# Kolkir/feature-point-cnn

Hardware: AMD Instinct MI355X
Metric: frames/sec (VGA 640x480) SuperPoint fwd+NMS+descriptors (higher is better)
Workload: dtype f32

## Files before the change

### feature-point-cnn_amd/_lib.py

```python
import ctypes
import os
import subprocess

import torch

_DIR = os.path.dirname(os.path.abspath(__file__))
LIB_PATH = os.environ.get("FPC_LIB_PATH") or os.path.join(_DIR, "lib", "libfpc.so")
CSRC = os.path.join(_DIR, "csrc")

SYMBOLS = [
    "fpc_abi_version", "fpc_build_flags", "fpc_strerror", "fpc_last_hip_error", "fpc_default_config", "fpc_create",
    "fpc_destroy", "fpc_load_weights", "fpc_packed_size", "fpc_packed_device_ptr",
    "fpc_export_packed", "fpc_import_packed", "fpc_import_packed_device", "fpc_mark_weights_loaded", "fpc_set_stream", "fpc_upload_stream",
    "fpc_get_stream", "fpc_sync", "fpc_forward", "fpc_detect", "fpc_get_points", "fpc_results",
    "fpc_get_counts", "fpc_get_keypoints", "fpc_set_timing", "fpc_get_timings", "fpc_match", "fpc_first_within",
    "fpc_detect_u8", "fpc_u8_staging", "fpc_homography_adaptation", "fpc_detect_u8_resized",
    "fpc_sample_descriptors", "fpc_plan_hash", "fpc_broadcast_weights", "fpc_read_activation",
    "fpc_pack_layout_revision", "fpc_check_guards", "fpc_stream_report", "fpc_output_range",
    "fpc_match_frames", "fpc_first_within_frames",
    "fpc_default_ransac_params", "fpc_ransac_homography", "fpc_homography_frames",
    "fpc_bank_create", "fpc_bank_destroy", "fpc_bank_get", "fpc_bank_store", "fpc_bank_store_rows", "fpc_bank_clear",
    "fpc_match_bank", "fpc_homography_bank", "fpc_bank_create_ex", "fpc_bank_format",
    "fpc_match_frames_guided", "fpc_match_bank_guided",
    "fpc_cell_order", "fpc_match_frames_guided_cells", "fpc_match_bank_guided_cells",
    "fpc_bank_topk_reserve", "fpc_match_bank_topk", "fpc_homography_bank_topk",
    "fpc_ransac_fundamental", "fpc_fundamental_frames", "fpc_fundamental_bank",
    "fpc_match_frames_guided_epipolar", "fpc_match_bank_guided_epipolar",
]

ABI_VERSION = 4
PACK_LAYOUT_REVISION = 4

PLAN_FLAGS = {
    "no_fused_blocks": 1 << 0, "no_winograd": 1 << 1, "no_winograd_detector": 1 << 2, "no_winograd_layer_in1": 1 << 3,
    "no_xcd_order": 1 << 4, "no_fused_stem_pool": 1 << 5, "split_heads": 1 << 6, "nms_in_line": 1 << 7,
    "no_persistent_grid": 1 << 8, "layer1_tile_8x16": 1 << 9, "winograd_gen1": 1 << 10, "no_latency_tiles": 1 << 11,
    "nms_one_workgroup": 1 << 12, "no_fused_softmax": 1 << 13, "winograd_gen2": 1 << 14, "guard_zones": 1 << 15, "detector_gen1": 1 << 16, "heads_in_line": 1 << 17, "w36_one_wave": 1 << 18, "convt_phases": 1 << 19, "stem_round3": 1 << 20, "conv_round1": 1 << 21,
}


class FpcConfig(ctypes.Structure):
    _fields_ = [("device", ctypes.c_int), ("height", ctypes.c_int), ("width", ctypes.c_int),
                ("max_batch", ctypes.c_int), ("cell", ctypes.c_int), ("nms_dist", ctypes.c_int),
                ("conf_thresh", ctypes.c_float), ("border_remove", ctypes.c_int),
                ("descriptor_enabled", ctypes.c_int), ("max_keypoints", ctypes.c_int),
                ("in_channels", ctypes.c_int), ("dtype", ctypes.c_int), ("arch", ctypes.c_int),
                ("num_streams", ctypes.c_int), ("plan_flags", ctypes.c_uint), ("nms_round_launches", ctypes.c_int),
                ("min_sub_batch", ctypes.c_int)]


class FpcTensor(ctypes.Structure):
    _fields_ = [("name", ctypes.c_char_p), ("data", ctypes.c_void_p), ("ndim", ctypes.c_int),
                ("shape", ctypes.c_int64 * 4)]


class FpcDeviceResults(ctypes.Structure):
    _fields_ = [("count", ctypes.c_void_p), ("n_candidates", ctypes.c_void_p), ("xy", ctypes.c_void_p),
                ("conf", ctypes.c_void_p), ("desc", ctypes.c_void_p), ("capacity", ctypes.c_int),
                ("desc_dim", ctypes.c_int)]


class FpcStreamReport(ctypes.Structure):
    _fields_ = [("n_streams", ctypes.c_int), ("slot", ctypes.c_int * 16), ("queue", ctypes.c_int * 16),
                ("probing", ctypes.c_int), ("hw_queues_found", ctypes.c_int), ("process_probe_rounds", ctypes.c_int),
                ("process_probe_launches", ctypes.c_int), ("process_inconclusive_rounds", ctypes.c_int),
                ("process_probe_ms", ctypes.c_float), ("create_probe_rounds", ctypes.c_int),
                ("create_placement_ms", ctypes.c_float), ("process_registered_streams", ctypes.c_int)]


class FpcRansacParams(ctypes.Structure):
    _fields_ = [("iterations", ctypes.c_int), ("reproj_threshold", ctypes.c_float), ("seed", ctypes.c_uint32),
                ("refits", ctypes.c_int), ("min_inliers", ctypes.c_int)]


BANK_MAX_SLOTS = 1024
BANK_TOPK_MAX = 16


class FpcBankView(ctypes.Structure):
    _fields_ = [("desc", ctypes.c_void_p), ("xy", ctypes.c_void_p), ("count", ctypes.c_void_p), ("slots", ctypes.c_int),
                ("rows", ctypes.c_int), ("desc_dim", ctypes.c_int), ("chunk", ctypes.c_int), ("bytes", ctypes.c_size_t)]


class FpcError(RuntimeError):
    def __init__(self, code, where):
        self.code = code
        l = load()
        msg = l.fpc_strerror(code).decode()
        detail = l.fpc_last_hip_error().decode()
        super().__init__("%s: %s (%d)%s" % (where, msg, code, " -- " + detail if detail else ""))


_lib = None


def build(force=False):
    args = ["make", "-s", "-C", CSRC]
    if force:
        args.append("-B")
    subprocess.check_call(args)
    return LIB_PATH


def load():
    global _lib
    if _lib is not None:
        return _lib
    if not os.path.exists(LIB_PATH):
        raise ImportError("libfpc.so is not built (%s): run `python -c 'import __graft_entry__ as g; g.build()'` "
                          "or `make -C feature-point-cnn_amd/csrc`; there is no CPU fallback" % LIB_PATH)
    l = ctypes.CDLL(LIB_PATH)
    vp, ci = ctypes.c_void_p, ctypes.c_int
    l.fpc_abi_version.restype = ci
    l.fpc_build_flags.restype = ctypes.c_char_p
    l.fpc_strerror.restype = ctypes.c_char_p
    l.fpc_strerror.argtypes = [ci]
    l.fpc_last_hip_error.restype = ctypes.c_char_p
    l.fpc_default_config.argtypes = [ctypes.POINTER(FpcConfig)]
    l.fpc_create.argtypes = [ctypes.POINTER(vp), ctypes.POINTER(FpcConfig)]
    l.fpc_destroy.argtypes = [vp]
    l.fpc_destroy.restype = None
    l.fpc_load_weights.argtypes = [vp, ctypes.POINTER(FpcTensor), ci]
    l.fpc_packed_size.argtypes = [vp]
    l.fpc_packed_size.restype = ctypes.c_size_t
    l.fpc_packed_device_ptr.argtypes = [vp]
    l.fpc_packed_device_ptr.restype = vp
    l.fpc_export_packed.argtypes = [vp, vp, ctypes.c_size_t]
    l.fpc_import_packed.argtypes = [vp, vp, ctypes.c_size_t]
    l.fpc_import_packed_device.argtypes = [vp, vp, ctypes.c_size_t]
    l.fpc_mark_weights_loaded.argtypes = [vp]
    l.fpc_set_stream.argtypes = [vp, vp]
    l.fpc_upload_stream.argtypes = [vp]
    l.fpc_upload_stream.restype = vp
    l.fpc_get_stream.argtypes = [vp]
    l.fpc_get_stream.restype = vp
    l.fpc_sync.argtypes = [vp]
    l.fpc_forward.argtypes = [vp, vp, ci, vp, vp, vp]
    l.fpc_detect.argtypes = [vp, vp, ci]
    l.fpc_get_points.argtypes = [vp, vp, vp, ci]
    l.fpc_detect_u8.argtypes = [vp, vp, ci, ci]
    l.fpc_u8_staging.argtypes = [vp]
    l.fpc_detect_u8_resized.argtypes = [vp, vp, ci, ci, ci, ci]
    l.fpc_homography_adaptation.argtypes = [vp, vp, ci, vp, vp, ci, ci, ci, vp]
    l.fpc_u8_staging.restype = vp
    l.fpc_results.argtypes = [vp, ctypes.POINTER(FpcDeviceResults)]
    l.fpc_get_counts.argtypes = [vp, ci, vp, vp]
    l.fpc_get_keypoints.argtypes = [vp, ci, ci, vp, vp, vp]
    l.fpc_output_range.argtypes = [vp, ci, vp, vp, vp]
    l.fpc_match.argtypes = [vp, vp, ci, vp, ci, ci, ctypes.c_float, vp, vp]
    l.fpc_first_within.argtypes = [vp, vp, ci, vp, ci, ctypes.c_float, vp]
    l.fpc_match_frames.argtypes = [vp, ci, ci, vp, vp, ci, ctypes.c_float, ctypes.c_float, vp, vp]
    l.fpc_first_within_frames.argtypes = [vp, ci, vp, vp, ctypes.c_float, vp]
    rp = ctypes.POINTER(FpcRansacParams)
    l.fpc_default_ransac_params.argtypes = [rp]
    l.fpc_ransac_homography.argtypes = [vp, ci, vp, vp, vp, ci, rp, vp, vp, vp]
    l.fpc_homography_frames.argtypes = [vp, ci, ci, vp, vp, vp, rp, vp, vp, vp]
    l.fpc_bank_create.argtypes = [vp, ci, ci]
    l.fpc_bank_create_ex.argtypes = [vp, ci, ci, ci]
    l.fpc_bank_format.argtypes = [vp, ctypes.POINTER(ci), ctypes.POINTER(vp)]
    l.fpc_bank_destroy.argtypes = [vp]
    l.fpc_bank_get.argtypes = [vp, ctypes.POINTER(FpcBankView)]
    l.fpc_bank_store.argtypes = [vp, ci, ci]
    l.fpc_bank_store_rows.argtypes = [vp, ci, vp, vp, vp]
    l.fpc_bank_clear.argtypes = [vp, ci]
    l.fpc_match_bank.argtypes = [vp, ci, ci, ctypes.c_float, ctypes.c_float, ci, vp, vp, vp, vp]
    l.fpc_homography_bank.argtypes = [vp, ci, vp, vp, rp, vp, vp, vp]
    l.fpc_ransac_fundamental.argtypes = [vp, ci, vp, vp, vp, ci, rp, vp, vp, vp]
    l.fpc_fundamental_frames.argtypes = [vp, ci, ci, vp, vp, vp, rp, vp, vp, vp]
    l.fpc_fundamental_bank.argtypes = [vp, ci, vp, vp, rp, vp, vp, vp]
    l.fpc_match_frames_guided.argtypes = [vp, ci, ci, vp, vp, vp, vp, ctypes.c_float, ci, ctypes.c_float, ctypes.c_float,
                                          vp, vp]
    l.fpc_match_bank_guided.argtypes = [vp, ci, vp, vp, ctypes.c_float, ci, ctypes.c_float, ctypes.c_float, vp, vp]
    l.fpc_cell_order.argtypes = [vp, vp, vp, ci, ci, vp]
    l.fpc_match_frames_guided_cells.argtypes = [vp, ci, ci, vp, vp, vp, vp, ctypes.c_float, ci, ctypes.c_float,
                                                ctypes.c_float, vp, vp, vp]
    l.fpc_match_bank_guided_cells.argtypes = [vp, ci, vp, vp, ctypes.c_float, ci, ctypes.c_float, ctypes.c_float, vp, vp,
                                              vp]
    l.fpc_match_frames_guided_epipolar.argtypes = list(l.fpc_match_frames_guided.argtypes)
    l.fpc_match_bank_guided_epipolar.argtypes = list(l.fpc_match_bank_guided.argtypes)
    l.fpc_bank_topk_reserve.argtypes = [vp, ci, ctypes.POINTER(ctypes.c_size_t)]
    l.fpc_match_bank_topk.argtypes = [vp, ci, ci, ci, ctypes.c_float, ctypes.c_float, ci, vp, vp, vp, vp, vp]
    l.fpc_homography_bank_topk.argtypes = [vp, ci, ci, vp, vp, rp, vp, vp, vp, vp, vp]
    l.fpc_sample_descriptors.argtypes = [vp, vp, vp, ci, vp]
    l.fpc_read_activation.argtypes = [vp, ctypes.c_char_p, ci, ci, vp, ctypes.POINTER(ci), ctypes.POINTER(ci), ctypes.POINTER(ci)]
    l.fpc_plan_hash.argtypes = [vp]
    l.fpc_plan_hash.restype = ctypes.c_uint64
    l.fpc_broadcast_weights.argtypes = [vp, vp, ci]
    l.fpc_pack_layout_revision.restype = ci
    l.fpc_check_guards.argtypes = [vp, ctypes.POINTER(ctypes.c_longlong)]
    l.fpc_stream_report.argtypes = [vp, ctypes.POINTER(FpcStreamReport)]
# ... 21 lines not shown
```

### feature-point-cnn_amd/csrc/fpc_api.hip

```cpp
#include <hip/hip_runtime.h>

#include <dlfcn.h>

#include <algorithm>
#include <cmath>
#include <cstdio>
#include <cstdlib>
#include <cstring>
#include <memory>
#include <mutex>
#include <chrono>
#include <string>
#include <vector>

#include "../../include/fpc.h"
#include "block_mfma.h"
#include "block_bf16.h"
#include "convt_bf16.h"
#include "block_x3.h"
#include "stem_bf16.h"
#include "wblock_mfma.h"
#include "wblock16_mfma.h"
#include "wblock36_mfma.h"
#include "wblock36p_mfma.h"
// ... 268 lines not shown
#undef X
#define X(name, TYT, TXT)                                                                                 \
  {#name, "wblock36_dust_kernel<" #TYT ", " #TXT ">", 3, 16, 2, 64,                                        \
   W36Cfg<1, TYT, TXT, true>::LDS_BYTES, 4, 4 * TYT, 4 * TXT, 256, (const void*)wblock36_dust_kernel<TYT, TXT>, launchw_##name, true},
    FPC_W36D_KINDS(X)
#undef X
#define X(name, TYT, TXT)                                                                                 \
  {#name, "wblock36p_kernel<" #TYT ", " #TXT ", 3>", 3, 16, 2, 64,                                            \
   W36PCfg<TYT, TXT>::LDS_BYTES, 4, 4 * TYT, 4 * TXT, 512, (const void*)wblock36p_kernel<TYT, TXT>, launchw_##name},
    FPC_W36P_KINDS(X)
#undef X
#define X(name, TYT, TXT)                                                                                 \
  {#name, "wblock36p_dust_kernel<" #TYT ", " #TXT ", 3>", 3, 16, 2, 64,                                    \
   W36PCfg<TYT, TXT, true>::LDS_BYTES, 4, 4 * TYT, 4 * TXT, 512, (const void*)wblock36p_dust_kernel<TYT, TXT>, launchw_##name, true},
    FPC_W36PD_KINDS(X)
#undef X
};

static size_t w1_floats(const WKindInfo& k, int nchunk) {
  if (k.gen == 3) return (size_t)k.NCG * ((size_t)nchunk * 36 + (k.NCG == 8 ? W36Cfg<2, 4, 4>::WPAD : W36Cfg<1, 4, 4>::WPAD)) * 256;
  return (size_t)k.NCG * ((size_t)nchunk * 16 + W16Cfg<8>::WPAD) * 256;
}
static double wkind_mfma_flops(const WKindInfo& k, int tiles, int nchunk, int k8_1x1) {
  const double px = (double)k.TH * k.TW, n = k.NBT * 32.0;
  if (k.gen == 3) return 2.0 * tiles * n * (36.0 * (px / 16) * nchunk * k.KC + px * k8_1x1 * 8.0);
  return 2.0 * tiles * n * (16.0 * (px / 4) * nchunk * k.KC + px * k8_1x1 * 8.0);
}
static bool w36_fits(int , int H, int W, int cs_in, int cs_out) {
  return (unsigned long long)H * W * (unsigned long long)std::max(cs_in, cs_out) * sizeof(float) < (unsigned long long)W36_MARKER;
}
static int w36_frames_per_launch(int H, int W, int cs_in, int cs_out) {
  const unsigned long long fb = (unsigned long long)H * W * (unsigned long long)std::max(cs_in, cs_out) * sizeof(float);
  return (int)std::max<unsigned long long>(1, ((unsigned long long)W36_MARKER - 1) / fb);
}
static int w36_conv_part(int cout, int tiles, int cus) {
  if (cout < 128) return 64;
  if (cout == 128) return 128;
  const double t2 = std::ceil((double)tiles * (cout / 128) / cus) * 1.0, t1 = std::ceil((double)tiles * (cout / 64) / cus) * 0.53;
  return t1 < t2 ? 64 : 128;
}
static WKind w36_kind(int cout, int H, int W, bool paired = false) {
  const int t44 = ((H + 15) / 16) * ((W + 15) / 16), t28 = ((H + 7) / 8) * ((W + 31) / 32);
  if (cout == 65 && paired) return t28 < t44 ? WK_W36PD_C65_2x8 : WK_W36PD_C65_4x4;
  if (cout == 65) return t28 < t44 ? WK_W36_C65_2x8 : WK_W36_C65_4x4;
  if (cout == 64 && paired) return t28 < t44 ? WK_W36P_C64_2x8 : WK_W36P_C64_4x4;
  if (cout == 64) return t28 < t44 ? WK_W36_C64_2x8 : WK_W36_C64_4x4;
  return t28 < t44 ? WK_W36_C128_2x8 : WK_W36_C128_4x4;
}

#define FPC_BF16_KINDS(X)                                                                   \
  X(F816_s1_K64_C64, block_bf16_one_kernel, BlockBfCfg, 1, 8, 32, 1, 3, 64, 2, 2, 4, 1, 64) \
  X(F816_s1_K64_C128, block_bf16_kernel, BlockBfCfg, 1, 8, 16, 1, 3, 64, 1, 4, 4, 1, 128)   \
  X(F816_s1_K80_C80, block_bf16_one_kernel, BlockBfCfg, 1, 8, 16, 1, 3, 80, 4, 1, 1, 3, 80) \
  X(F816_s1_K128_C128, block_bf16_one_kernel, BlockBfCfg, 1, 8, 16, 1, 3, 128, 1, 4, 4, 1, 128) \
  X(F816_s1_K128_C80w, block_bf16_one_kernel, BlockBfCfg, 1, 8, 16, 1, 3, 128, 1, 4, 4, 1, 80) \
  X(F620_s2_K64_C128, block_bf16_one_kernel, BlockBfCfg, 1, 6, 20, 2, 3, 64, 2, 2, 2, 2, 128) \
  X(F320_s2_K128_C256, block_bf16_one_kernel, BlockBfCfg, 1, 3, 20, 2, 3, 128, 1, 4, 2, 2, 256) \
  X(F416_s1_K128_C256, block_bf16_two_kernel, BlockBfCfg, 1, 4, 16, 1, 3, 128, 1, 4, 2, 2, 256) \
  X(F816_ct_K64_C128, block_bf16_kernel, BlockBfCfg, 1, 8, 16, 1, 2, 64, 1, 4, 4, 1, 128)   \
  X(F816_ctf_K64_C128, convt_bf16_kernel, ConvTBfCfg, 1, 8, 16, 1, 2, 64, 2, 2, 2, 1, 128)  \
  X(S816_s1_K64_C64, block_x3_kernel, BlockX3Cfg, 3, 8, 16, 1, 3, 64, 2, 2, 2, 1, 64)       \
  X(S620_s2_K16_C128, block_x3_kernel, BlockX3Cfg, 3, 6, 20, 2, 3, 16, 2, 2, 2, 2, 128)     \
  X(S620_s1_K64_C128, block_x3_kernel, BlockX3Cfg, 3, 6, 20, 1, 3, 64, 2, 2, 2, 2, 128)     \
  X(S620_s1_K64_C80, block_x3_kernel, BlockX3Cfg, 3, 6, 20, 1, 3, 64, 4, 1, 1, 3, 80)       \
  X(S620_s1_K16_C80, block_x3_kernel, BlockX3Cfg, 3, 6, 20, 1, 3, 16, 4, 1, 1, 3, 80)       \
  X(S320_s2_K16_C256, block_x3_kernel, BlockX3Cfg, 3, 3, 20, 2, 3, 16, 1, 4, 2, 2, 256)     \
  X(S320_s1_K64_C256, block_x3_kernel, BlockX3Cfg, 3, 3, 20, 1, 3, 64, 1, 4, 2, 2, 256)     \
  X(S620_ct_K64_C128, block_x3_kernel, BlockX3Cfg, 3, 6, 20, 1, 2, 64, 2, 2, 2, 2, 128)     \
  X(S620_1x1_K64_C80, block_x3_kernel, BlockX3Cfg, 3, 6, 20, 1, 1, 64, 4, 1, 1, 3, 80)      \
  X(S320_1x1_K64_C256, block_x3_kernel, BlockX3Cfg, 3, 3, 20, 1, 1, 64, 1, 4, 2, 2, 256)     \
  X(H816_s1_K64_C64, block_h2_kernel, BlockH2Cfg, 2, 8, 16, 1, 3, 64, 2, 2, 2, 1, 64)     \
  X(H620_s2_K16_C128, block_h2_kernel, BlockH2Cfg, 2, 6, 20, 2, 3, 16, 2, 2, 2, 2, 128)     \
  X(H620_s1_K64_C128, block_h2_kernel, BlockH2Cfg, 2, 6, 20, 1, 3, 64, 2, 2, 2, 2, 128)     \
  X(H620_s1_K64_C80, block_h2_kernel, BlockH2Cfg, 2, 6, 20, 1, 3, 64, 4, 1, 1, 3, 80)     \
  X(H620_s1_K16_C80, block_h2_kernel, BlockH2Cfg, 2, 6, 20, 1, 3, 16, 4, 1, 1, 3, 80)     \
  X(H320_s2_K16_C256, block_h2_kernel, BlockH2Cfg, 2, 3, 20, 2, 3, 16, 1, 4, 2, 2, 256)     \
  X(H320_s1_K64_C256, block_h2_kernel, BlockH2Cfg, 2, 3, 20, 1, 3, 64, 1, 4, 2, 2, 256)     \
  X(H620_ct_K64_C128, block_h2_kernel, BlockH2Cfg, 2, 6, 20, 1, 2, 64, 2, 2, 2, 2, 128)     \
  X(H620_1x1_K64_C80, block_h2_kernel, BlockH2Cfg, 2, 6, 20, 1, 1, 64, 4, 1, 1, 3, 80)     \
  X(H320_1x1_K64_C256, block_h2_kernel, BlockH2Cfg, 2, 3, 20, 1, 1, 64, 1, 4, 2, 2, 256)

enum FKind {
#define X(name, ...) FK_##name,
  FPC_BF16_KINDS(X)
#undef X
      FK_COUNT
};

struct FKindInfo {
  const char* name;
  const char* symbol;
  int planes, TH, TW, S, EXT, KC, WM, WN, MB, NB, CMIDP;
  int lds_bytes;
  const void* fn;
  void (*launch)(const BlockBfArgs&, dim3, hipStream_t);
};

#define X(name, KERN, CFG, PL, TH, TW, S, EXT, KC, WM, WN, MB, NB, CMIDP)                                  \
  static void launchf_##name(const BlockBfArgs& a, dim3 grid, hipStream_t st) {                            \
    constexpr int lds = CFG<TH, TW, S, EXT, KC, WM, WN, MB, NB, CMIDP>::LDS_BYTES;                         \
    hipLaunchKernelGGL((KERN<TH, TW, S, EXT, KC, WM, WN, MB, NB, CMIDP>), grid, dim3(WM* WN * 64), lds, st, a); \
  }
FPC_BF16_KINDS(X)
#undef X

static const FKindInfo g_fkinds[FK_COUNT] = {
#define X(name, KERN, CFG, PL, TH, TW, S, EXT, KC, WM, WN, MB, NB, CMIDP)                                   \
  {#name, #KERN "<" #TH ", " #TW ", " #S ", " #EXT ", " #KC ", " #WM ", " #WN ", " #MB ", " #NB ", " #CMIDP ">", \
   PL, TH, TW, S, EXT, KC, WM, WN, MB, NB, CMIDP, CFG<TH, TW, S, EXT, KC, WM, WN, MB, NB, CMIDP>::LDS_BYTES,   \
   (const void*)KERN<TH, TW, S, EXT, KC, WM, WN, MB, NB, CMIDP>, launchf_##name},
    FPC_BF16_KINDS(X)
#undef X
};

enum OpType { OP_STEM, OP_POOL, OP_CONV, OP_BLOCK, OP_WBLOCK, OP_BF16, OP_SOFTMAX, OP_NMS, OP_DESC,
              OP_VCONV0, OP_POOL2, OP_L2NORM };

struct Op {
  OpType type;
  std::string name;
  Kind kind = K_COUNT;
  ConvArgs args{};
  BKind bkind = BK_COUNT;
  BlockArgs bargs{};
  WKind wkind = WK_COUNT;
  WBlockArgs wargs{};
  FKind fkind = FK_COUNT;
  BlockBfArgs fargs{};
  int phase = -1;
  int when = 0;
  bool shadow = false;
  bool wconv = false;
  int n0 = 0;
  bool plain_conv = false;
  bool lean = false;
  int ksize = 0;
  const float* pin = nullptr;
  float* pout = nullptr;
  int pH = 0, pW = 0, pC = 0;
  std::string prefix;
  int cin = 0, cout = 0;
  int grid_y = 1, grid_z = 1;
  double flops_per_frame = 0;
  double mfma_flops_per_frame = 0;
  bool fused_softmax_capable = false;
  double bytes_per_frame = 0;
  bool descriptor_branch = false;
};

struct Timing {
  hipEvent_t start, stop;
  int op;
  int frames;
};

}

using namespace fpc;

struct fpc_ctx {
  fpc_config cfg{};
  int H = 0, W = 0, B = 0, Hc = 0, Wc = 0;
  bool vgg = false;
  int D = 128;
  std::vector<float*> vbuf;
  size_t vconv0_off = 0;
  bool bf16 = false;
  bool split = false;
  bool split_f16 = false;
  int lgcs = 72;
  int cin = 3;
  int cap = 0, sort_cap = 0;
  hipStream_t stream = nullptr;
  bool own_stream = false;
  hipStream_t upload = nullptr;
  bool queue_probe = true;
  int probe_rounds = 0;
  double placement_ms = 0.0;
  std::vector<std::pair<hipStream_t, int>> caller_stream_memo;
  std::vector<hipStream_t> aux;
  std::vector<hipEvent_t> ev_join;
  std::vector<hipStream_t> side;
  std::vector<hipEvent_t> ev_enc, ev_det;
  bool nms_aside = true;
  bool split_heads = false;
  hipEvent_t ev_fork = nullptr;
  int min_sub = 8;
  int num_cus = 256;
  int fkind_blocks_per_cu[64] = {};
  int persist_min_tiles = 1;
  bool xcd_order = true;
  int nms_passes = 2;
  bool fuse_softmax = true;
  bool convt_fused = true;
  bool logits_valid = false;
  bool nms_one_workgroup = false;
  int nms_g = 0;
  bool fuse_stem_pool = true;
  bool conv_lean = true;
  bool stem_lean = true;
  bool stem2 = false;
  bool layer1_t816 = false;
#ifdef FPC_DIAG
  unsigned long long* diag_stamps = nullptr;
  int diag_n = 0;
#endif
  bool winograd_in1 = true;
  bool winograd_det = true;
  int w36_cus = 0;
  bool w36_paired = true;
  bool winograd_det_gen3 = true;
  bool winograd = true;
  bool latency_tiles = true;
  int winograd_gen = 3;
  bool fuse_blocks = true;
  bool weights_loaded = false;
  bool plan_error = false;

  char* slab = nullptr;
  size_t slab_bytes = 0;
  bool guard_zones = false;
  std::vector<std::pair<size_t, size_t>> guards;
  float *stem_out, *x0, *h4, *x1, *x2, *h8, *x3, *cat, *dh, *dproj, *d0, *lg;
  float *h16, *y16a, *y16b, *lo_h, *lo0, *desc_map, *desc_in_nhwc;
  float* prob;
  uint32_t *nmsmap, *cand;
  int32_t *ncand, *count, *xy, *status;
  float* rowmax = nullptr;
  uint32_t* range = nullptr;
  float *conf, *desc_out;
  unsigned long long* sort_scratch;
  int32_t* nms_aux = nullptr;
  unsigned long long *rowbest, *colbest;
  float* mf_norms = nullptr;
  unsigned long long *mf_top2 = nullptr, *mf_colbest = nullptr;
  float4* hf_pairs = nullptr;
  int32_t *hf_row = nullptr, *hf_np = nullptr;
  unsigned long long* hf_best = nullptr;
  int32_t *mgc_perm_q = nullptr, *mgc_perm_t = nullptr;
  int4* mgc_box = nullptr;
  char* bank_slab = nullptr;
  size_t bank_bytes = 0;
  BankArgs bank{};
  int bank_format = FPC_BANK_F32;
  BankBf16Args bank16{};
  std::vector<std::pair<size_t, size_t>> bank_guards;
  char* topk_slab = nullptr;
  BankTopkArgs topk{};
  float4* topk_pairs = nullptr;
  int32_t *topk_row = nullptr, *topk_np = nullptr;
  unsigned long long* topk_best = nullptr;
  std::vector<std::pair<size_t, size_t>> topk_guards;
  int pts_n = 0;
  bool pts_desc = false;

  float* u8stage = nullptr;
  char* ha_ws = nullptr;

  float* blob = nullptr;
  size_t blob_floats = 0;
  uint32_t* bcast_tag = nullptr;
  std::vector<float> host_blob;

  std::vector<Op> ops;
  StemArgs stem{};
  size_t stem_w_off = 0, stem_b_off = 0;
  struct ConvW {
    size_t w_off[4] = {0, 0, 0, 0}, b_off = 0, b2_off = 0;
  };
  std::vector<ConvW> convw;

  bool timing = false;
  int timing_every = 0, timing_calls = 0;
  std::vector<Timing> timings;
  std::vector<hipEvent_t> event_pool;
  size_t events_used = 0;
};

namespace fpc {

static size_t align_up(size_t v, size_t a) { return (v + a - 1) / a * a; }

constexpr size_t GUARD_BYTES = 64 << 10;
constexpr size_t GUARD_TAIL = (size_t)0x80000000u + (4u << 20);
constexpr uint32_t GUARD_PATTERN = 0xA5C3F00Du;

struct Carver {
  size_t off = 0;
  size_t guard = 0;
  std::vector<std::pair<size_t, size_t>>* zones = nullptr;
  template <typename T>
  size_t take(size_t n) {
    const size_t o = off;
    off = align_up(off + n * sizeof(T), 256);
    if (guard) {
      zones->push_back({off, guard});
      off += guard;
    }
    return o;
  }
  void finish() {
    if (guard) {
      zones->push_back({off, GUARD_TAIL});
      off += GUARD_TAIL;
    }
  }
};


__global__ void guard_fill_kernel(uint32_t* p, size_t n, uint32_t v) {
  for (size_t i = (size_t)blockIdx.x * blockDim.x + threadIdx.x; i < n; i += (size_t)gridDim.x * blockDim.x) p[i] = v;
}
__global__ void guard_count_kernel(const uint32_t* p, size_t n, uint32_t v, unsigned long long* bad) {
  unsigned long long mine = 0;
  for (size_t i = (size_t)blockIdx.x * blockDim.x + threadIdx.x; i < n; i += (size_t)gridDim.x * blockDim.x) mine += p[i] != v;
  if (mine) atomicAdd(bad, mine);
}
using GuardZones = std::vector<std::pair<size_t, size_t>>;
static unsigned guard_blocks(size_t words) { return (unsigned)std::min<size_t>(4096, (words + 255) / 256); }

static void fill_zones(fpc_ctx* c, char* base, const GuardZones& zones) {
  for (const auto& z : zones) {
    const size_t n = z.second / 4;
    guard_fill_kernel<<<guard_blocks(n), 256, 0, c->stream>>>(reinterpret_cast<uint32_t*>(base + z.first), n, GUARD_PATTERN);
  }
}
static void count_zones(fpc_ctx* c, const char* base, const GuardZones& zones, unsigned long long* bad) {
  for (const auto& z : zones) {
    const size_t n = z.second / 4;
    guard_count_kernel<<<guard_blocks(n), 256, 0, c->stream>>>(reinterpret_cast<const uint32_t*>(base + z.first), n, GUARD_PATTERN, bad);
  }
}

static int fill_guards(fpc_ctx* c) {
  HIPCHECK(hipDeviceSynchronize());
  fill_zones(c, c->slab, c->guards);
  if (!c->guards.empty()) HIPCHECK(hipStreamSynchronize(c->stream));
  return FPC_OK;
}

static int alloc_side_slab(fpc_ctx* c, const Carver& cv, char** slab) {
  char* p = nullptr;
  HIPCHECK(hipMalloc((void**)&p, cv.off));
  hipError_t e = hipMemset(p, 0, cv.off);
  if (e == hipSuccess) e = hipDeviceSynchronize();
  fill_zones(c, p, *cv.zones);
  if (e == hipSuccess) e = hipStreamSynchronize(c->stream);
  if (e != hipSuccess) hipFree(p);
  HIPCHECK(e);
  *slab = p;
  return FPC_OK;
}


struct ConvSpec {
  std::string name;
  Kind kind;
  int ksize;
  int stride;
  const float* in0;
  int cs0, cin0, cin0_pad, H0, W0;
  const float* in1 = nullptr;
// ... 1548 lines not shown
        srcs.push_back({ci, a.k16_x * 16, 1, [&](int n, int c_, int) { return (double)wp[(size_t)n * ci + c_]; }, &fp.s});
      frag = pack_conv_bf16(srcs, co, nbt, 16, k.planes, &range_bad);
      memcpy(blob.data() + cw.w_off[1], frag.data(), frag.size() * sizeof(float));
      for (int n = 0; n < co; ++n) blob[cw.b2_off + n] = (float)bias[n];
      continue;
    }
    if (op.type == OP_BLOCK) {
      const BKindInfo& k = g_bkinds[op.bkind];
      const BlockArgs& a = op.bargs;
      const fpc_ctx::ConvW& cw = c->convw[i];
      const std::string& p = op.prefix;
      const int ci = op.cin, co = op.cout, nbt = k.WN * k.NB;
      const float* w1 = need(p + ".conv1.weight", {co, ci, 3, 3});
      const float* w2 = need(p + ".conv2.weight", {co, co, 1, 1});
      Fold f1, f2, fp;
      if (!w1 || !w2 || !fold_bn(m, p + ".bn1", co, &f1, missing) || !fold_bn(m, p + ".bn2", co, &f2, missing))
        return FPC_E_MISSING_KEY;
      PackSource s1{ci, a.nchunk * k.KC, 9, [&](int n, int c_, int t) { return (double)w1[((size_t)(n * ci + c_)) * 9 + t]; }, &f1.s};
      std::vector<float> frag = pack_conv({s1}, co, nbt, k.KC);
      memcpy(blob.data() + cw.w_off[0], frag.data(), frag.size() * sizeof(float));
      for (int n = 0; n < co; ++n) blob[cw.b_off + n] = (float)f1.t[n];
      std::vector<PackSource> srcs;
      srcs.push_back({co, a.k8_h * 8, 1, [&](int n, int c_, int) { return (double)w2[(size_t)n * co + c_]; }, &f2.s});
      std::vector<double> bias(f2.t);
      const float* wp = nullptr;
      if (a.k8_x > 0) {
        wp = need(p + ".identity_downsample.0.weight", {co, ci, 1, 1});
        if (!wp || !fold_bn(m, p + ".identity_downsample.1", co, &fp, missing)) return FPC_E_MISSING_KEY;
        srcs.push_back({ci, a.k8_x * 8, 1, [&](int n, int c_, int) { return (double)wp[(size_t)n * ci + c_]; }, &fp.s});
        for (int n = 0; n < co; ++n) bias[n] += fp.t[n];
      }
      frag = pack_conv(srcs, co, nbt, 8);
      memcpy(blob.data() + cw.w_off[1], frag.data(), frag.size() * sizeof(float));
      for (int n = 0; n < co; ++n) blob[cw.b2_off + n] = (float)bias[n];
      continue;
    }
    if (op.type != OP_CONV) continue;
    const KindInfo& k = g_kinds[op.kind];
    const ConvArgs& a = op.args;
    const fpc_ctx::ConvW& cw = c->convw[i];
    const std::string& nm = op.name;
    const size_t dot = nm.find(".conv1+");
    const size_t dot2 = nm.find(".conv2+");
    const int cin0p = a.nchunk0 * k.KC, cin1p = a.nchunk1 * k.KC;
    Fold f, fp;
    std::vector<double> bias(a.nbt * 32, 0.0);
    if (nm == "descriptor.up_sample+bn+relu") {
      const float* w = need("descriptor.up_sample.weight", {256, 128, 3, 3});
      const float* bct = need("descriptor.up_sample.bias", {128});
      if (!w || !bct || !fold_bn(m, "descriptor.bn", 128, &f, missing)) return FPC_E_MISSING_KEY;
      for (int ph = 0; ph < 4; ++ph) {
        const int py = ph >> 1, px = ph & 1;
        std::vector<std::pair<int, int>> taps;
        for (int iy = 0; iy < (py ? 2 : 1); ++iy)
          for (int ix = 0; ix < (px ? 2 : 1); ++ix) taps.push_back({py ? (iy == 0 ? 0 : 2) : 1, px ? (ix == 0 ? 0 : 2) : 1});
        PackSource s{256, cin0p, (int)taps.size(),
                     [&](int n, int ci, int t) { return (double)w[((ci * 128 + n) * 3 + taps[t].first) * 3 + taps[t].second]; },
                     &f.s};
        std::vector<float> frag = pack_conv({s}, 128, a.nbt, k.KC);
        memcpy(blob.data() + cw.w_off[ph], frag.data(), frag.size() * sizeof(float));
      }
      for (int n = 0; n < 128; ++n) bias[n] = (double)bct[n] * f.s[n] + f.t[n];
    } else if (nm == "detector.layer.0.identity_downsample") {
      const float* w = need("detector.layer.0.identity_downsample.0.weight", {65, 128, 1, 1});
      if (!w || !fold_bn(m, "detector.layer.0.identity_downsample.1", 65, &f, missing)) return FPC_E_MISSING_KEY;
      PackSource s{128, cin0p, 1, [&](int n, int ci, int) { return (double)w[n * 128 + ci]; }, &f.s};
      std::vector<float> frag = pack_conv({s}, 65, a.nbt, k.KC);
      memcpy(blob.data() + cw.w_off[0], frag.data(), frag.size() * sizeof(float));
      for (int n = 0; n < 65; ++n) bias[n] = f.t[n];
    } else if (dot != std::string::npos) {
      const std::string p = nm.substr(0, dot);
      auto it = m.find(p + ".conv1.weight");
      if (it == m.end() || it->second.shape.size() != 4 || it->second.shape[2] != 3) {
        if (missing->empty()) *missing = p + ".conv1.weight";
        return FPC_E_MISSING_KEY;
      }
      const int co = (int)it->second.shape[0], ci = (int)it->second.shape[1];
      const float* w = it->second.data;
      if (ci > cin0p || co > a.nbt * 32 || !w) {
        *missing = p + ".conv1.weight";
        return FPC_E_MISSING_KEY;
      }
      if (!fold_bn(m, p + ".bn1", co, &f, missing)) return FPC_E_MISSING_KEY;
      PackSource s{ci, cin0p, 9, [&](int n, int c_, int t) { return (double)w[((size_t)(n * ci + c_)) * 9 + t]; }, &f.s};
      std::vector<float> frag = pack_conv({s}, co, a.nbt, k.KC);
      memcpy(blob.data() + cw.w_off[0], frag.data(), frag.size() * sizeof(float));
      for (int n = 0; n < co; ++n) bias[n] = f.t[n];
    } else if (dot2 != std::string::npos) {
      const std::string p = nm.substr(0, dot2);
      auto it = m.find(p + ".conv2.weight");
      if (it == m.end() || it->second.shape.size() != 4 || !it->second.data) {
        if (missing->empty()) *missing = p + ".conv2.weight";
        return FPC_E_MISSING_KEY;
      }
      const int co = (int)it->second.shape[0];
      const float* w = it->second.data;
      if ((int)it->second.shape[1] != co || co > cin0p || co > a.nbt * 32) {
        *missing = p + ".conv2.weight";
        return FPC_E_MISSING_KEY;
      }
      if (!fold_bn(m, p + ".bn2", co, &f, missing)) return FPC_E_MISSING_KEY;
      std::vector<PackSource> srcs;
      srcs.push_back({co, cin0p, 1, [&, co](int n, int c_, int) { return (double)w[(size_t)n * co + c_]; }, &f.s});
      for (int n = 0; n < co; ++n) bias[n] = f.t[n];
      const float* wp = nullptr;
      int cip = 0;
      if (a.in1) {
        auto ip = m.find(p + ".identity_downsample.0.weight");
        if (ip == m.end() || ip->second.shape.size() != 4 || (int)ip->second.shape[0] != co || !ip->second.data ||
            (int)ip->second.shape[1] > cin1p) {
          if (missing->empty()) *missing = p + ".identity_downsample.0.weight";
          return FPC_E_MISSING_KEY;
        }
        wp = ip->second.data;
        cip = (int)ip->second.shape[1];
        if (!fold_bn(m, p + ".identity_downsample.1", co, &fp, missing)) return FPC_E_MISSING_KEY;
        srcs.push_back({cip, cin1p, 1, [&, cip](int n, int c_, int) { return (double)wp[(size_t)n * cip + c_]; }, &fp.s});
        for (int n = 0; n < co; ++n) bias[n] += fp.t[n];
      }
      std::vector<float> frag = pack_conv(srcs, co, a.nbt, k.KC);
      memcpy(blob.data() + cw.w_off[0], frag.data(), frag.size() * sizeof(float));
    } else {
      *missing = "internal: unknown op " + nm;
      return FPC_E_INVALID;
    }
    for (int n = 0; n < a.nbt * 32; ++n) blob[cw.b_off + n] = (float)bias[n];
  }
  return FPC_OK;
}

static hipEvent_t next_event(fpc_ctx* c) {
  if (c->events_used == c->event_pool.size()) {
    hipEvent_t e;
    hipEventCreate(&e);
    c->event_pool.push_back(e);
  }
  return c->event_pool[c->events_used++];
}

struct Sub {
  int f0, n;
  bool small = false;
  bool fuse_softmax = false;
  hipStream_t st;
  hipStream_t side = nullptr;
  hipEvent_t ev_enc = nullptr, ev_det = nullptr;
};

struct LaunchTimer {
  fpc_ctx* c;
  int op;
  hipStream_t st;
  int frames;
  hipEvent_t s{}, e{};
  LaunchTimer(fpc_ctx* c_, int op_, hipStream_t st_, int frames_) : c(c_), op(op_), st(st_), frames(frames_) {
    if (c->timing) {
      s = next_event(c);
      e = next_event(c);
      hipEventRecord(s, st);
    }
  }
  ~LaunchTimer() {
    if (c->timing) {
      hipEventRecord(e, st);
      c->timings.push_back({s, e, op, frames});
    }
  }
};

static int op_index(const fpc_ctx* c, OpType t) {
  for (size_t i = 0; i < c->ops.size(); ++i)
    if (c->ops[i].type == t) return (int)i;
  return -1;
}

static void run_network(fpc_ctx* c, const float* frames, const Sub& sb0, int which, hipStream_t st) {
  Sub sb = sb0;
  sb.st = st;
  const int H = c->H, W = c->W, n = sb.n, f0 = sb.f0;
  for (size_t i = 0; i < c->ops.size(); ++i) {
    const Op& op = c->ops[i];
    const int br = op.descriptor_branch ? 2 : (op.name.compare(0, 8, "detector") == 0 ? 1 : 0);
    if (br != which) continue;
    if (op.shadow) continue;
    if (op.when == 1 && !sb.small) continue;
    if (op.when == 2 && sb.small) continue;
    switch (op.type) {
      case OP_STEM: {
        if (c->fuse_stem_pool || c->cin == 1 || c->bf16) {
          float* x0 = c->bf16 ? reinterpret_cast<float*>(reinterpret_cast<unsigned short*>(c->x0) + (size_t)f0 * (H / 4) * (W / 4) * 64)
                              : c->x0 + (size_t)f0 * (H / 4) * (W / 4) * 64;
          if (!c->bf16) stem_border_clear_kernel<<<(n * (H / 4) + 7) / 8, 256, 0, sb.st>>>(reinterpret_cast<float4*>(x0), H / 4, W / 4, n * (H / 4));
          LaunchTimer t(c, (int)i, sb.st, n);
          StemPoolArgs a{};
          a.in = frames + (size_t)f0 * c->cin * H * W;
          a.wfrag = c->stem.wfrag;
          a.bias = c->stem.bias;
          a.out = x0;
          a.H = H; a.W = W; a.Ho = H / 2; a.Wo = W / 2; a.Hp = H / 4; a.Wp = W / 4;
          a.tiles_x = c->stem.tiles_x; a.tiles_y = c->stem.tiles_y;
          a.range = c->range + (size_t)f0 * FPC_RANGE_WORDS;
          if (c->split || c->bf16) {
            StemX3Args x{};
            x.in = a.in; x.wfrag = reinterpret_cast<const uint4*>(a.wfrag); x.bias = a.bias; x.out = a.out;
            x.H = H; x.W = W; x.Ho = a.Ho; x.Wo = a.Wo; x.Hp = a.Hp; x.Wp = a.Wp; x.tiles_x = a.tiles_x; x.tiles_y = a.tiles_y;
            x.range_flag = c->split_f16 ? c->status + 1 : nullptr;
#ifdef FPC_DIAG
            x.stamps = nullptr;
            if (const char* e = getenv("FPC_STAMP_OP"))
              if (op.name.find(e) != std::string::npos) {
                if (!c->diag_stamps) hipHostMalloc((void**)&c->diag_stamps, (size_t)65536 * 8 * sizeof(unsigned long long));
                memset(c->diag_stamps, 0, (size_t)65536 * 8 * sizeof(unsigned long long));
                x.stamps = c->diag_stamps;
                c->diag_n = a.tiles_x * a.tiles_y * n;
              }
#endif
            const dim3 grid(a.tiles_x * a.tiles_y * n);
            if (c->split_f16) {
              if (c->cin == 1) hipLaunchKernelGGL((stem_pool_x3_kernel<1, 2>), grid, dim3(256), 0, sb.st, x);
              else hipLaunchKernelGGL((stem_pool_x3_kernel<3, 2>), grid, dim3(256), 0, sb.st, x);
            } else if (c->bf16) {
              x.frames = n;
              x.tiles_x = (x.Wp + SB2_PW - 1) / SB2_PW;
              x.tiles_y = (x.Hp + SB2_PH - 1) / SB2_PH;
              const int T = x.tiles_x * x.tiles_y * n;
              const dim3 pg(std::min((T + 7) / 8 * 8, std::max(8, 2 * c->num_cus / 8 * 8)));
              if (c->cin == 1) hipLaunchKernelGGL(stem_bf16_kernel<1>, pg, dim3(SB2_THREADS), StemB2Cfg<1>::LDS_BYTES, sb.st, x);
              else hipLaunchKernelGGL(stem_bf16_kernel<3>, pg, dim3(SB2_THREADS), StemB2Cfg<3>::LDS_BYTES, sb.st, x);
            } else {
              if (c->cin == 1) hipLaunchKernelGGL((stem_pool_x3_kernel<1, 3>), grid, dim3(256), 0, sb.st, x);
              else hipLaunchKernelGGL((stem_pool_x3_kernel<3, 3>), grid, dim3(256), 0, sb.st, x);
            }
          } else if (c->stem2) {
            if (c->cin == 1) hipLaunchKernelGGL(stem_pool2_kernel<1>, dim3(a.tiles_x * a.tiles_y * n), dim3(256), 0, sb.st, a);
            else hipLaunchKernelGGL(stem_pool2_kernel<3>, dim3(a.tiles_x * a.tiles_y * n), dim3(256), 0, sb.st, a);
          } else if (c->cin == 1)
            hipLaunchKernelGGL(stem_pool_kernel<1>, dim3(a.tiles_x * a.tiles_y * n), dim3(256), 0, sb.st, a);
          else
            hipLaunchKernelGGL(stem_pool_kernel<3>, dim3(a.tiles_x * a.tiles_y * n), dim3(256), 0, sb.st, a);
          break;
        }
        LaunchTimer t(c, (int)i, sb.st, n);
        StemArgs a = c->stem;
        a.in = frames + (size_t)f0 * 3 * H * W;
        a.out = c->stem_out + (size_t)f0 * (H / 2) * (W / 2) * 64;
        hipLaunchKernelGGL(stem_kernel, dim3(a.tiles_x * a.tiles_y * n), dim3(256), 0, sb.st, a);
        break;
      }
      case OP_POOL: {
        if (c->fuse_stem_pool || c->cin == 1 || c->bf16) break;
        LaunchTimer t(c, (int)i, sb.st, n);
        const size_t total = (size_t)n * (H / 4) * (W / 4) * 16;
        hipLaunchKernelGGL(maxpool_kernel, dim3((unsigned)((total + 255) / 256)), dim3(256), 0, sb.st,
                           reinterpret_cast<const float4*>(c->stem_out + (size_t)f0 * (H / 2) * (W / 2) * 64),
                           reinterpret_cast<float4*>(c->x0 + (size_t)f0 * (H / 4) * (W / 4) * 64), n, H / 2, W / 2, H / 4,
                           W / 4);
        break;
      }
      case OP_WBLOCK: {
        LaunchTimer t(c, (int)i, sb.st, n);
        WBlockArgs a = op.wargs;
        a.frame0 = f0;
#ifdef FPC_DIAG
        a.stamps = nullptr;
        if (const char* e = getenv("FPC_STAMP_OP"))
          if (op.name.find(e) != std::string::npos) {
            if (!c->diag_stamps) hipHostMalloc((void**)&c->diag_stamps, (size_t)65536 * 8 * sizeof(unsigned long long));
            memset(c->diag_stamps, 0, (size_t)65536 * 8 * sizeof(unsigned long long));
            a.stamps = c->diag_stamps;
            c->diag_n = a.tiles_x * a.tiles_y * n;
          }
#endif
        a.total = a.tiles_x * a.tiles_y * n;
        a.xcd_order = c->xcd_order ? 1 : 0;
        {
          const unsigned long long xb = (unsigned long long)(f0 + n) * a.H * a.W * a.csx * sizeof(float);
          a.x_bytes = xb > 0xfffffff0ull ? 0xfffffff0u : (unsigned)xb;
        }
        int grid = (c->persist_min_tiles > 0 && a.total >= c->persist_min_tiles * c->num_cus) ? c->num_cus : a.total;
        if (g_wkinds[op.wkind].gen == 3) {
          const int fpl = w36_frames_per_launch(a.H, a.W, a.csx, a.cso);
          const float* x0 = a.x;
          float* o0 = a.out;
          for (int g0 = 0; g0 < n; g0 += fpl) {
            const int gn = std::min(fpl, n - g0);
            a.frame0 = 0;
            a.x = x0 + (size_t)(f0 + g0) * a.H * a.W * a.csx;
            a.out = o0 + (size_t)(f0 + g0) * a.H * a.W * a.cso;
            a.total = a.tiles_x * a.tiles_y * gn;
            a.x_bytes = (unsigned)((unsigned long long)gn * a.H * a.W * a.csx * sizeof(float));
            const int cus_cap = c->w36_cus > 0 ? std::min(c->num_cus, c->w36_cus) : c->num_cus;
            const int cus8 = std::max(1, cus_cap / 8 / std::max(1, op.grid_y)), per_xcd = (a.total + 7) / 8;
            const int rounds = (per_xcd + cus8 - 1) / cus8;
            const int grid3 = 8 * std::min(cus8, (per_xcd + rounds - 1) / rounds);
            g_wkinds[op.wkind].launch(a, dim3(std::min(a.total, grid3), op.grid_y), sb.st);
          }
          break;
        }
        g_wkinds[op.wkind].launch(a, dim3(std::min(a.total, grid), op.grid_y), sb.st);
        break;
      }
      case OP_BLOCK: {
        LaunchTimer t(c, (int)i, sb.st, n);
        BlockArgs a = op.bargs;
        a.frame0 = f0;
#ifdef FPC_DIAG
        a.stamps = nullptr;
        if (const char* e = getenv("FPC_STAMP_OP"))
          if (op.name.find(e) != std::string::npos) {
            if (!c->diag_stamps) hipHostMalloc((void**)&c->diag_stamps, (size_t)65536 * 8 * sizeof(unsigned long long));
            memset(c->diag_stamps, 0, (size_t)65536 * 8 * sizeof(unsigned long long));
            a.stamps = c->diag_stamps;
            c->diag_n = a.tiles_x * a.tiles_y * n;
          }
#endif
        g_bkinds[op.bkind].launch(a, dim3(a.tiles_x * a.tiles_y * n), sb.st);
        break;
      }
      case OP_BF16: {
        LaunchTimer t(c, (int)i, sb.st, n);
        BlockBfArgs a = op.fargs;
        a.frame0 = f0;
        a.range_flag = c->split_f16 ? c->status + 1 : nullptr;
#ifdef FPC_DIAG
        a.stamps = nullptr;
        if (const char* e = getenv("FPC_STAMP_OP"))
          if (op.name.find(e) != std::string::npos) {
            if (!c->diag_stamps) hipHostMalloc((void**)&c->diag_stamps, (size_t)65536 * 8 * sizeof(unsigned long long));
            memset(c->diag_stamps, 0, (size_t)65536 * 8 * sizeof(unsigned long long));
            a.stamps = c->diag_stamps;
            c->diag_n = a.tiles_x * a.tiles_y * n;
          }
#endif
        if (g_fkinds[op.fkind].planes == 1) {
          a.total_tiles = a.tiles_x * a.tiles_y * n;
          if (sb.fuse_softmax && op.fused_softmax_capable) {
            const size_t HW = (size_t)c->H * c->W;
            hipMemsetAsync(c->ncand + f0, 0, sizeof(int32_t) * n, sb.st);
            a.softmax = 1;
            a.thresh = c->cfg.conf_thresh;
            a.nmsmap = c->nmsmap + f0 * HW;
            a.cand = c->cand + f0 * HW;
            a.ncand = c->ncand + f0;
          }
          const int g = std::min((a.total_tiles + 7) / 8 * 8, std::max(8, c->fkind_blocks_per_cu[op.fkind] * c->num_cus / op.grid_y / 8 * 8));
          g_fkinds[op.fkind].launch(a, dim3(g, op.grid_y), sb.st);
        } else {
          g_fkinds[op.fkind].launch(a, dim3(a.tiles_x * a.tiles_y * n), sb.st);
        }
        break;
      }
      case OP_VCONV0: {
        LaunchTimer t(c, (int)i, sb.st, n);
        VggConv0Args a{};
        a.in = frames;
        a.w = c->blob + c->vconv0_off;
        a.out = op.pout;
        a.H = H; a.W = W; a.frame0 = f0;
        hipLaunchKernelGGL(vgg_conv0_kernel, dim3((unsigned)((size_t)n * H * W / 64)), dim3(256), 0, sb.st, a);
        break;
      }
      case OP_POOL2: {
        LaunchTimer t(c, (int)i, sb.st, n);
        const size_t tot = (size_t)n * (op.pH / 2) * (op.pW / 2) * (op.pC / 4);
        hipLaunchKernelGGL(maxpool2_kernel, dim3((unsigned)((tot + 255) / 256)), dim3(256), 0, sb.st,
                           reinterpret_cast<const float4*>(op.pin), reinterpret_cast<float4*>(op.pout), n, op.pH, op.pW,
                           op.pC / 4, f0);
        break;
      }
      case OP_L2NORM: {
        LaunchTimer t(c, (int)i, sb.st, n);
        const size_t npix = (size_t)n * c->Hc * c->Wc;
        hipLaunchKernelGGL(l2norm256_kernel, dim3((unsigned)((npix + 3) / 4)), dim3(256), 0, sb.st,
                           op.pout + (size_t)f0 * c->Hc * c->Wc * 256, npix);
        break;
      }
      case OP_CONV: {
        LaunchTimer t(c, (int)i, sb.st, n);
        ConvArgs a = op.args;
        a.frame0 = f0;
        if (op.lean) lean_kind(op.kind)->launch(a, dim3(a.tiles_x * a.tiles_y * n, op.grid_y, op.grid_z), sb.st);
        else g_kinds[op.kind].launch(a, dim3(a.tiles_x * a.tiles_y * n, op.grid_y, op.grid_z), sb.st);
        break;
      }
      default:
        break;
    }
  }
}

static Sub on(const Sub& sb, hipStream_t st) {
  Sub r = sb;
  r.st = st;
  return r;
}

static void run_softmax(fpc_ctx* c, const Sub& sb, bool dense_map = true) {
  const size_t HW = (size_t)c->H * c->W;
  hipMemsetAsync(c->ncand + sb.f0, 0, sizeof(int32_t) * sb.n, sb.st);
  LaunchTimer t(c, op_index(c, OP_SOFTMAX), sb.st, sb.n);
  const auto kern = c->bf16 ? softmax_d2s_kernel<true> : softmax_d2s_kernel<false>;
  hipLaunchKernelGGL(kern, dim3(sb.n * c->Hc), dim3(256), (size_t)12 * c->W * sizeof(float), sb.st,
                     c->lg + (size_t)sb.f0 * c->Hc * c->Wc * c->lgcs, c->lgcs, sb.n, c->Hc, c->Wc, c->cfg.conf_thresh,
                     dense_map ? c->prob + sb.f0 * HW : nullptr, c->nmsmap + sb.f0 * HW, c->cand + sb.f0 * HW, c->ncand + sb.f0,
                     c->rowmax + (size_t)sb.f0 * c->Hc);
}

static void run_nms(fpc_ctx* c, const Sub& sb) {
  LaunchTimer t(c, op_index(c, OP_NMS), sb.st, sb.n);
  const size_t HW = (size_t)c->H * c->W;
  const int n = sb.n, f0 = sb.f0;
  NmsArgs a{};
  a.nmsmap = c->nmsmap + f0 * HW; a.cand = c->cand + f0 * HW; a.ncand = c->ncand + f0;
  a.sort_scratch = c->sort_scratch + (size_t)f0 * c->sort_cap;
  a.sort_cap = c->sort_cap;
  const bool chunked = !c->nms_one_workgroup;
  a.aux = chunked ? c->nms_aux + (size_t)f0 * NMS_AUX_INTS : nullptr;
  a.H = c->H; a.W = c->W; a.r = c->cfg.nms_dist; a.border = c->cfg.border_remove; a.cap = c->cap;
  a.count = c->count + f0; a.xy = c->xy + (size_t)f0 * c->cap * 2; a.conf = c->conf + (size_t)f0 * c->cap;
  a.status = c->status;
  a.max_rounds = c->H * c->W;
  const int G = c->nms_g > 0 ? c->nms_g : std::max(1, std::min(16, 512 / n));
  for (int pass = 0; pass < c->nms_passes; ++pass) {
    if (c->cfg.nms_dist == 4)
      hipLaunchKernelGGL(nms_rounds_kernel<4>, dim3(G, n), dim3(NMS_ROUNDS_THREADS), 0, sb.st, a);
    else
      hipLaunchKernelGGL(nms_rounds_kernel<0>, dim3(G, n), dim3(NMS_ROUNDS_THREADS), 0, sb.st, a);
  }
  if (chunked) {
    const bool big = HW > 400000;
    const int GC = big ? 8 : 4;
    hipLaunchKernelGGL(nms_finish_kernel, dim3(n), dim3(NMS_FINISH_THREADS), 0, sb.st, a);
    if (big) {
      hipLaunchKernelGGL(nms_chunk_sort_kernel<4096>, dim3(GC, n), dim3(1024), 4096 * sizeof(unsigned long long), sb.st, a);
      hipLaunchKernelGGL(nms_merge_kernel<4096>, dim3(GC, n), dim3(1024), 4096 * sizeof(unsigned long long), sb.st, a);
    } else {
      hipLaunchKernelGGL(nms_chunk_sort_kernel<2048>, dim3(GC, n), dim3(1024), 2048 * sizeof(unsigned long long), sb.st, a);
      hipLaunchKernelGGL(nms_merge_kernel<2048>, dim3(GC, n), dim3(1024), 2048 * sizeof(unsigned long long), sb.st, a);
    }
  }
  hipLaunchKernelGGL(nms_sort_kernel, dim3(n), dim3(1024), chunked ? 0 : NMS_LDS_KEYS * sizeof(unsigned long long), sb.st, a);
}

static void run_desc(fpc_ctx* c, const Sub& sb, const float* dmap_nhwc) {
  LaunchTimer t(c, op_index(c, OP_DESC), sb.st, sb.n);
  const int by_xcd = sb.n >= 8;
  const int G = std::max(8, c->num_cus * 8 / 8 * 8);
  if (c->D == 256)
    hipLaunchKernelGGL(descriptor16_kernel<16>, dim3(G), dim3(256), 0, sb.st,
// ... 97 lines not shown
#else
         ";diag=0"
#endif
         ";ablations=none";
}

const char* fpc_strerror(int code) {
  switch (code) {
    case FPC_OK: return "ok";
    case FPC_E_INVALID: return "invalid argument or unsupported geometry";
    case FPC_E_NO_DEVICE: return "no usable HIP device (this library has no CPU fallback)";
    case FPC_E_HIP: return "HIP runtime error (see fpc_last_hip_error)";
    case FPC_E_NO_WEIGHTS: return "weights not loaded";
    case FPC_E_MISSING_KEY: return "checkpoint entry missing or of the wrong shape (see fpc_last_hip_error)";
    case FPC_E_CAPACITY: return "caller buffer too small";
    case FPC_E_NOT_CONVERGED: return "NMS round limit hit";
    case FPC_E_RANGE: return "value outside fp16's range in FPC_F32_SPLIT_F16 mode (use FPC_F32_SPLIT or FPC_F32)";
    case FPC_E_NONFINITE: return "a frame of the call holds a NaN or Inf pixel (see fpc_last_hip_error for which)";
    default: return "unknown error";
  }
}

const char* fpc_last_hip_error(void) { return g_hip_err.c_str(); }

int fpc_default_config(fpc_config* cfg) {
  if (!cfg) return FPC_E_INVALID;
  memset(cfg, 0, sizeof(*cfg));
  cfg->device = 0;
  cfg->height = 480;
  cfg->width = 640;
  cfg->max_batch = 1;
  cfg->cell = 8;
  cfg->nms_dist = 4;
  cfg->conf_thresh = 0.015f;
  cfg->border_remove = 4;
  cfg->descriptor_enabled = 1;
  cfg->max_keypoints = 0;
  return FPC_OK;
}

enum { SLOT_MAIN = 0, SLOT_AUX = 1, SLOT_SIDE = 100, SLOT_UPLOAD = 200 };

static int prepare_kernels(fpc_ctx* c, const fpc_config* cfg) {
  for (int k = 0; k < K_COUNT; ++k)
    HIPCHECK(hipFuncSetAttribute(g_kinds[k].fn, hipFuncAttributeMaxDynamicSharedMemorySize, g_kinds[k].lds_bytes));
  for (const LeanKindInfo& l : g_lean_kinds) HIPCHECK(hipFuncSetAttribute(l.fn, hipFuncAttributeMaxDynamicSharedMemorySize, l.lds_bytes));
  for (int k = 0; k < WK_COUNT; ++k)
    HIPCHECK(hipFuncSetAttribute(g_wkinds[k].fn, hipFuncAttributeMaxDynamicSharedMemorySize, g_wkinds[k].lds_bytes));
  for (int k = 0; k < BK_COUNT; ++k)
    HIPCHECK(hipFuncSetAttribute(g_bkinds[k].fn, hipFuncAttributeMaxDynamicSharedMemorySize, g_bkinds[k].lds_bytes));
  static_assert(FK_COUNT <= 64, "fpc_ctx::fkind_blocks_per_cu");
  for (int k = 0; k < FK_COUNT; ++k) {
    HIPCHECK(hipFuncSetAttribute(g_fkinds[k].fn, hipFuncAttributeMaxDynamicSharedMemorySize, g_fkinds[k].lds_bytes));
    int nb = 0;
    HIPCHECK(hipOccupancyMaxActiveBlocksPerMultiprocessor(&nb, g_fkinds[k].fn, g_fkinds[k].WM * g_fkinds[k].WN * 64, g_fkinds[k].lds_bytes));
    c->fkind_blocks_per_cu[k] = std::max(1, nb);
#ifdef FPC_DIAG
    hipFuncAttributes fa{};
    hipFuncGetAttributes(&fa, g_fkinds[k].fn);
    fprintf(stderr, "[diag] %s: lds %d B, regs %d, scratch %zu, occupancy %d blocks/CU\n", g_fkinds[k].name, g_fkinds[k].lds_bytes, fa.numRegs, fa.localSizeBytes, nb);
#endif
  }
  HIPCHECK(hipFuncSetAttribute((const void*)softmax_d2s_kernel<false>, hipFuncAttributeMaxDynamicSharedMemorySize,
                               12 * cfg->width * (int)sizeof(float)));
  HIPCHECK(hipFuncSetAttribute((const void*)softmax_d2s_kernel<true>, hipFuncAttributeMaxDynamicSharedMemorySize,
                               12 * cfg->width * (int)sizeof(float)));
  HIPCHECK(hipFuncSetAttribute((const void*)stem_bf16_kernel<1>, hipFuncAttributeMaxDynamicSharedMemorySize, StemB2Cfg<1>::LDS_BYTES));
  HIPCHECK(hipFuncSetAttribute((const void*)stem_bf16_kernel<3>, hipFuncAttributeMaxDynamicSharedMemorySize, StemB2Cfg<3>::LDS_BYTES));
  HIPCHECK(hipFuncSetAttribute((const void*)nms_sort_kernel, hipFuncAttributeMaxDynamicSharedMemorySize,
                               NMS_LDS_KEYS * (int)sizeof(unsigned long long)));
#ifdef FPC_DIAG
  for (int k = 0; k < BK_COUNT; ++k) {
    int nb = -1;
    hipOccupancyMaxActiveBlocksPerMultiprocessor(&nb, g_bkinds[k].fn, g_bkinds[k].WM * g_bkinds[k].WN * 64, g_bkinds[k].lds_bytes);
    hipFuncAttributes fa{};
    hipFuncGetAttributes(&fa, g_bkinds[k].fn);
    fprintf(stderr, "[diag] %s: lds %d B, regs %d, static lds %zu, occupancy %d blocks/CU\n", g_bkinds[k].name, g_bkinds[k].lds_bytes, fa.numRegs, fa.sharedSizeBytes, nb);
  }
  for (int k = 0; k < K_COUNT; ++k) {
    int nb = -1;
    hipOccupancyMaxActiveBlocksPerMultiprocessor(&nb, g_kinds[k].fn, g_kinds[k].threads, g_kinds[k].lds_bytes);
    fprintf(stderr, "[diag] %s: lds %d B, occupancy %d blocks/CU\n", g_kinds[k].name, g_kinds[k].lds_bytes, nb);
  }
#endif
  return FPC_OK;
}

int fpc_create(fpc_ctx** out, const fpc_config* cfg) {
  if (!out || !cfg) return FPC_E_INVALID;
  *out = nullptr;
  const int mult = (cfg->descriptor_enabled && cfg->arch != FPC_ARCH_VGG) ? 16 : 8;
  if (cfg->in_channels != 0 && cfg->in_channels != 1 && cfg->in_channels != 3) return FPC_E_INVALID;
  if (cfg->dtype < FPC_F32 || cfg->dtype > FPC_F32_SPLIT_F16) return FPC_E_INVALID;
  if (cfg->arch != FPC_ARCH_RESNET && cfg->arch != FPC_ARCH_VGG) return FPC_E_INVALID;
  if (cfg->arch == FPC_ARCH_VGG && (cfg->in_channels != 1 || cfg->dtype == FPC_BF16)) return FPC_E_INVALID;
  if (!(cfg->conf_thresh >= 0.f) || !(cfg->conf_thresh <= 3.0e38f)) return FPC_E_INVALID;
  if (cfg->cell != 8 || cfg->height < 16 || cfg->width < 16 || cfg->height % mult || cfg->width % mult ||
      cfg->max_batch < 1 || cfg->nms_dist < 0 || cfg->nms_dist > 64 || cfg->border_remove < 0 ||
      (long long)cfg->height * cfg->width >= (1ll << 30) ||
      (long long)cfg->max_batch * cfg->height * cfg->width >= (1ll << 28) ||
      cfg->width > 3328)
    return FPC_E_INVALID;
  int ndev = 0;
  if (hipGetDeviceCount(&ndev) != hipSuccess || ndev <= 0 || cfg->device < 0 || cfg->device >= ndev) {
    g_hip_err = "hipGetDeviceCount: no device";
    return FPC_E_NO_DEVICE;
  }
  HIPCHECK(hipSetDevice(cfg->device));
  std::unique_ptr<fpc_ctx> c(new fpc_ctx());
  {
    hipDeviceProp_t prop;
    HIPCHECK(hipGetDeviceProperties(&prop, cfg->device));
    c->num_cus = std::max(1, prop.multiProcessorCount);
  }
  c->cfg = *cfg;
  c->H = cfg->height;
  c->W = cfg->width;
  c->B = cfg->max_batch;
  c->Hc = c->H / 8;
  c->Wc = c->W / 8;
  c->cin = cfg->in_channels == 1 ? 1 : 3;
  c->vgg = cfg->arch == FPC_ARCH_VGG;
  c->D = c->vgg ? 256 : 128;
  c->bf16 = cfg->dtype == FPC_BF16;
  c->split = cfg->dtype == FPC_F32_SPLIT || cfg->dtype == FPC_F32_SPLIT_F16;
  c->split_f16 = cfg->dtype == FPC_F32_SPLIT_F16;
  c->lgcs = (c->bf16 || c->split) ? 80 : 72;
  const int r1 = cfg->nms_dist + 1;
  const int worst = ((c->H + r1 - 1) / r1) * ((c->W + r1 - 1) / r1);
  c->cap = cfg->max_keypoints > 0 ? cfg->max_keypoints : worst;
  c->sort_cap = 1;
  while (c->sort_cap < worst) c->sort_cap <<= 1;
  {
    const int prc = prepare_kernels(c.get(), cfg);
    if (prc != FPC_OK) return prc;
  }
  const bool qprobe = qmap::probe_mode() != 0;
  c->queue_probe = qprobe;
  const auto create_t0 = std::chrono::steady_clock::now();
  std::unique_lock<std::mutex> queue_lock(qmap::state().mu);
  const int probe_rounds0 = qmap::state().dev[cfg->device].rounds;
  c->stream = qmap::acquire(cfg->device, c.get(), SLOT_MAIN, true, qprobe, true);
  if (!c->stream) { qmap::release_owner(c.get()); g_hip_err = "hipStreamCreateWithFlags"; return FPC_E_HIP; }
  c->own_stream = true;
  {
    int nsub = cfg->num_streams > 0 ? std::min(8, cfg->num_streams) : (c->split ? 3 : 2);
    const unsigned pf = cfg->plan_flags;
    c->fuse_blocks = !(pf & FPC_PLAN_NO_FUSED_BLOCKS);
    c->guard_zones = (pf & FPC_PLAN_GUARD_ZONES) != 0;
    if (const char* e = getenv("FPC_GUARD_ZONES")) c->guard_zones = atoi(e) != 0;
    c->winograd_det_gen3 = !(pf & FPC_PLAN_DETECTOR_GEN1);
    c->w36_paired = !(pf & FPC_PLAN_W36_ONE_WAVE);
    if (const char* e = getenv("FPC_W36_PAIRED")) c->w36_paired = atoi(e) != 0;
    if (const char* e = getenv("FPC_W36_CUS")) c->w36_cus = std::max(0, atoi(e));
    if (const char* e = getenv("FPC_WINOGRAD_DET_GEN")) c->winograd_det_gen3 = atoi(e) >= 3;
    c->winograd = !(pf & FPC_PLAN_NO_WINOGRAD);
    c->winograd_det = !(pf & FPC_PLAN_NO_WINOGRAD_DETECTOR);
    c->winograd_in1 = !(pf & FPC_PLAN_NO_WINOGRAD_LAYER_IN1);
    c->xcd_order = !(pf & FPC_PLAN_NO_XCD_ORDER);
    c->fuse_stem_pool = !(pf & FPC_PLAN_NO_FUSED_STEM_POOL);
    c->stem_lean = !(pf & FPC_PLAN_STEM_ROUND3);
    c->conv_lean = !(pf & FPC_PLAN_CONV_ROUND1);
    if (const char* e = getenv("FPC_CONV_LEAN")) c->conv_lean = atoi(e) != 0;
    if (const char* e = getenv("FPC_STEM_LEAN")) c->stem_lean = atoi(e) != 0;
    c->split_heads = (pf & FPC_PLAN_SPLIT_HEADS) != 0;
    if (pf & FPC_PLAN_NO_PERSISTENT_GRID) c->persist_min_tiles = 0;
    c->layer1_t816 = (pf & FPC_PLAN_LAYER1_TILE_8x16) != 0;
    c->winograd_gen = (pf & FPC_PLAN_WINOGRAD_GEN1) ? 1 : (pf & FPC_PLAN_WINOGRAD_GEN2) ? 2 : 3;
    if (const char* e = getenv("FPC_WINOGRAD_GEN")) c->winograd_gen = std::min(3, std::max(1, atoi(e)));
    c->latency_tiles = !(pf & FPC_PLAN_NO_LATENCY_TILES);
    if (const char* e = getenv("FPC_LATENCY_TILES")) c->latency_tiles = atoi(e) != 0;
    c->fuse_softmax = !(pf & FPC_PLAN_NO_FUSED_SOFTMAX);
    c->convt_fused = !(pf & FPC_PLAN_CONVT_PHASES);
    if (const char* e = getenv("FPC_CONVT_FUSED")) c->convt_fused = atoi(e) != 0;
    if (const char* e = getenv("FPC_FUSE_SOFTMAX")) c->fuse_softmax = atoi(e) != 0;
    c->nms_one_workgroup = (pf & FPC_PLAN_NMS_ONE_WORKGROUP) != 0;
    if (const char* e = getenv("FPC_NMS_CHUNKED")) c->nms_one_workgroup = atoi(e) == 0;
    if (cfg->min_sub_batch > 0) c->min_sub = cfg->min_sub_batch;
    if (cfg->nms_round_launches > 0) c->nms_passes = std::min(64, cfg->nms_round_launches);
    else if (cfg->nms_round_launches < 0) c->nms_passes = 0;
    if (const char* e = getenv("FPC_STREAMS")) nsub = std::max(1, std::min(8, atoi(e)));
    if (!(pf & FPC_PLAN_HEADS_IN_LINE) && nsub >= 2 && !c->vgg && !c->bf16 && !c->split) c->split_heads = true;
    if (const char* e = getenv("FPC_FUSE")) c->fuse_blocks = atoi(e) != 0;
    if (const char* e = getenv("FPC_WINOGRAD")) c->winograd = atoi(e) != 0;
    if (const char* e = getenv("FPC_XCD_ORDER")) c->xcd_order = atoi(e) != 0;
    if (const char* e = getenv("FPC_MIN_SUB")) c->min_sub = std::max(1, atoi(e));
    if (const char* e = getenv("FPC_PERSIST_MIN")) c->persist_min_tiles = atoi(e);
    if (const char* e = getenv("FPC_WINOGRAD_DET")) c->winograd_det = atoi(e) != 0;
    if (const char* e = getenv("FPC_WINOGRAD_IN1")) c->winograd_in1 = atoi(e) != 0;
    if (const char* e = getenv("FPC_FUSE_STEM")) c->fuse_stem_pool = atoi(e) != 0;
    if (const char* e = getenv("FPC_NMS_PASSES")) c->nms_passes = std::max(0, std::min(64, atoi(e)));
    if (const char* e = getenv("FPC_NMS_G")) c->nms_g = std::max(0, std::min(64, atoi(e)));
    if (getenv("FPC_L1_T816")) c->layer1_t816 = true;
    auto fail = [&](const char* what) {
      g_hip_err = what;
      queue_lock.unlock();
      fpc_destroy(c.release());
      return FPC_E_HIP;
    };
    if (hipEventCreateWithFlags(&c->ev_fork, hipEventDisableTiming) != hipSuccess) return fail("hipEventCreateWithFlags");
    for (int i = 1; i < nsub; ++i) {
      hipStream_t st = qmap::acquire(cfg->device, c.get(), SLOT_AUX + (i - 1), true, qprobe, true);
      hipEvent_t ev;
      if (!st) return fail("hipStreamCreateWithFlags");
      c->aux.push_back(st);
      if (hipEventCreateWithFlags(&ev, hipEventDisableTiming) != hipSuccess) return fail("hipEventCreateWithFlags");
      c->ev_join.push_back(ev);
    }
    if (const char* e = getenv("FPC_SPLIT_HEADS")) c->split_heads = atoi(e) != 0;
    c->nms_aside = !c->split;
    if (pf & FPC_PLAN_NMS_IN_LINE) c->nms_aside = false;
    if (const char* e = getenv("FPC_NMS_ASIDE")) c->nms_aside = atoi(e) != 0;
    if (c->split_heads) c->nms_aside = false;
    const int nside = 2 * nsub <= 4 ? nsub : 1;
    for (int i = 0; i < nsub; ++i) {
      hipStream_t st = nullptr;
      hipEvent_t e1, e2;
      if (i < nside) {
        st = qmap::acquire(cfg->device, c.get(), SLOT_SIDE + i, false, qprobe, true);
        if (!st) return fail("hipStreamCreateWithFlags");
      }
      c->side.push_back(st);
      if (hipEventCreateWithFlags(&e1, hipEventDisableTiming) != hipSuccess) return fail("hipEventCreateWithFlags");
      c->ev_enc.push_back(e1);
      if (hipEventCreateWithFlags(&e2, hipEventDisableTiming) != hipSuccess) return fail("hipEventCreateWithFlags");
      c->ev_det.push_back(e2);
    }
    c->probe_rounds = qmap::state().dev[cfg->device].rounds - probe_rounds0;
    c->placement_ms = std::chrono::duration<double, std::milli>(std::chrono::steady_clock::now() - create_t0).count();
    queue_lock.unlock();
  }
  int rc = FPC_OK;
  if (rc == FPC_OK && getenv("FPC_TEST_FAIL_CREATE")) {
    g_hip_err = "FPC_TEST_FAIL_CREATE is set: fpc_create's failure path was asked for";
    rc = FPC_E_HIP;
  }
  if (rc == FPC_OK) rc = build_plan(c.get());
  if (rc == FPC_OK && c->plan_error) {
    g_hip_err = "no kernel instance for a layer of this dtype / arch combination";
    rc = FPC_E_INVALID;
  }
  if (rc != FPC_OK) {
    fpc_destroy(c.release());
    return rc;
  }
  *out = c.release();
  return FPC_OK;
}

void fpc_destroy(fpc_ctx* c) {
  if (!c) return;
  hipSetDevice(c->cfg.device);
  hipDeviceSynchronize();
  for (auto e : c->event_pool) hipEventDestroy(e);
  for (auto e : c->ev_join) hipEventDestroy(e);
  for (auto e : c->ev_enc) hipEventDestroy(e);
  for (auto e : c->ev_det) hipEventDestroy(e);
  if (c->ev_fork) hipEventDestroy(c->ev_fork);
  {
    std::lock_guard<std::mutex> queue_lock(qmap::state().mu);
    qmap::DeviceQueues& q = qmap::state().dev[c->cfg.device];
    auto give_back = [&](hipStream_t st, int slot) {
      if (!st) return;
      const qmap::Placed* p = qmap::find(c, slot);
      qmap::retire(q, st, p && p->st == st ? p->qclass : qmap::Q_UNKNOWN);
    };
    for (size_t i = 0; i < c->aux.size(); ++i) give_back(c->aux[i], SLOT_AUX + (int)i);
    for (size_t i = 0; i < c->side.size(); ++i) give_back(c->side[i], SLOT_SIDE + (int)i);
    give_back(c->upload, SLOT_UPLOAD);
    if (c->own_stream) give_back(c->stream, SLOT_MAIN);
    qmap::release_owner(c);
  }
  if (c->slab) hipFree(c->slab);
  if (c->bank_slab) hipFree(c->bank_slab);
  if (c->topk_slab) hipFree(c->topk_slab);
  if (c->blob) hipFree(c->blob);
  if (c->u8stage) hipFree(c->u8stage);
  if (c->ha_ws) hipFree(c->ha_ws);
  delete c;
}

int fpc_load_weights(fpc_ctx* c, const fpc_tensor* tensors, int n) {
  if (!c || !tensors || n <= 0) return FPC_E_INVALID;
  TensorMap m;
  for (int i = 0; i < n; ++i) {
    if (!tensors[i].name || tensors[i].ndim < 0 || tensors[i].ndim > 4) return FPC_E_INVALID;
    HostTensor t;
    t.data = tensors[i].data;
    t.shape.assign(tensors[i].shape, tensors[i].shape + tensors[i].ndim);
    m[tensors[i].name] = t;
  }
  std::string missing;
  const int rc = pack_all(c, m, &missing);
  if (rc != FPC_OK) {
    g_hip_err = "checkpoint entry: " + missing;
    return rc;
  }
  HIPCHECK(hipSetDevice(c->cfg.device));
  HIPCHECK(hipMemcpy(c->blob, c->host_blob.data(), c->blob_floats * sizeof(float), hipMemcpyHostToDevice));
  c->weights_loaded = true;
  return FPC_OK;
}

size_t fpc_packed_size(const fpc_ctx* c) { return c ? c->blob_floats * sizeof(float) : 0; }
void* fpc_packed_device_ptr(fpc_ctx* c) { return c ? c->blob : nullptr; }

// ... 1099 lines not shown
  a.cross_check = cross_check != 0;
  bank_as_train(a, c->bank, slot);
  const MatchGuidedArgs g{H, c->xy, c->bank.xy, (double)radius * (double)radius};
  return match_guided_launch(c, half ? GUIDED_BANK_BF16 : strip, a, g, n, max_dist, ratio, match, dist, stats);
}

int fpc_match_frames_guided(fpc_ctx* c, int n, int pairing, const float* key, const int32_t* nkey, const int32_t* key_xy,
                            const float* H, float radius, int cross_check, float max_dist, float ratio, int32_t* match,
                            float* dist) {
  return match_frames_guided(c, GUIDED_PLAIN, n, pairing, key, nkey, key_xy, H, radius, cross_check, max_dist, ratio, match, dist,
                             nullptr);
}

int fpc_match_frames_guided_cells(fpc_ctx* c, int n, int pairing, const float* key, const int32_t* nkey,
                                  const int32_t* key_xy, const float* H, float radius, int cross_check, float max_dist,
                                  float ratio, int32_t* match, float* dist, int32_t* stats) {
  return match_frames_guided(c, GUIDED_CELLS, n, pairing, key, nkey, key_xy, H, radius, cross_check, max_dist, ratio, match, dist,
                             stats);
}

int fpc_match_bank_guided(fpc_ctx* c, int n, const int32_t* slot, const float* H, float radius, int cross_check,
                          float max_dist, float ratio, int32_t* match, float* dist) {
  return match_bank_guided(c, GUIDED_PLAIN, n, slot, H, radius, cross_check, max_dist, ratio, match, dist, nullptr);
}

int fpc_match_bank_guided_cells(fpc_ctx* c, int n, const int32_t* slot, const float* H, float radius, int cross_check,
                                float max_dist, float ratio, int32_t* match, float* dist, int32_t* stats) {
  return match_bank_guided(c, GUIDED_CELLS, n, slot, H, radius, cross_check, max_dist, ratio, match, dist, stats);
}

int fpc_match_frames_guided_epipolar(fpc_ctx* c, int n, int pairing, const float* key, const int32_t* nkey,
                                     const int32_t* key_xy, const float* F, float radius, int cross_check, float max_dist,
                                     float ratio, int32_t* match, float* dist) {
  return match_frames_guided(c, GUIDED_EPIPOLAR, n, pairing, key, nkey, key_xy, F, radius, cross_check, max_dist, ratio, match,
                             dist, nullptr);
}

int fpc_match_bank_guided_epipolar(fpc_ctx* c, int n, const int32_t* slot, const float* F, float radius, int cross_check,
                                   float max_dist, float ratio, int32_t* match, float* dist) {
  return match_bank_guided(c, GUIDED_EPIPOLAR, n, slot, F, radius, cross_check, max_dist, ratio, match, dist, nullptr);
}

int fpc_results(fpc_ctx* c, fpc_device_results* out) {
  if (!c || !out) return FPC_E_INVALID;
  out->count = c->count;
  out->n_candidates = c->ncand;
  out->xy = c->xy;
  out->conf = c->conf;
  out->desc = c->cfg.descriptor_enabled ? c->desc_out : nullptr;
  out->capacity = c->cap;
  out->desc_dim = c->D;
  return FPC_OK;
}

int fpc_get_counts(fpc_ctx* c, int n, int32_t* count, int32_t* ncand) {
  if (!c || n < 1 || n > c->B) return FPC_E_INVALID;
  HIPCHECK(hipSetDevice(c->cfg.device));
  HIPCHECK(hipStreamSynchronize(c->stream));
  int32_t st[2] = {0, 0};
  HIPCHECK(hipMemcpy(st, c->status, sizeof(st), hipMemcpyDeviceToHost));
  if (st[0]) return FPC_E_NOT_CONVERGED;
  if (st[1]) return FPC_E_RANGE;
  if (count) HIPCHECK(hipMemcpy(count, c->count, sizeof(int32_t) * n, hipMemcpyDeviceToHost));
  if (ncand) HIPCHECK(hipMemcpy(ncand, c->ncand, sizeof(int32_t) * n, hipMemcpyDeviceToHost));
  std::vector<uint32_t> rw((size_t)n * FPC_RANGE_WORDS);
  HIPCHECK(hipMemcpy(rw.data(), c->range, rw.size() * sizeof(uint32_t), hipMemcpyDeviceToHost));
  for (int b = 0; b < n; ++b)
    if (rw[(size_t)b * FPC_RANGE_WORDS + RANGE_BAD_INPUT]) {
      g_hip_err = "frame " + std::to_string(b) + " of the last call holds a NaN or Inf pixel";
      return FPC_E_NONFINITE;
    }
  return FPC_OK;
}

int fpc_output_range(fpc_ctx* c, int n, float* max_logit, float* max_desc, int32_t* nonfinite_input) {
  if (!c || n < 1 || n > c->B) return FPC_E_INVALID;
  HIPCHECK(hipSetDevice(c->cfg.device));
  HIPCHECK(hipStreamSynchronize(c->stream));
  std::vector<uint32_t> rw((size_t)n * FPC_RANGE_WORDS);
  HIPCHECK(hipMemcpy(rw.data(), c->range, rw.size() * sizeof(uint32_t), hipMemcpyDeviceToHost));
  std::vector<float> rm((size_t)n * c->Hc);
  if (max_logit) HIPCHECK(hipMemcpy(rm.data(), c->rowmax, rm.size() * sizeof(float), hipMemcpyDeviceToHost));
  for (int b = 0; b < n; ++b) {
    const uint32_t* w = rw.data() + (size_t)b * FPC_RANGE_WORDS;
    float f;
    if (max_logit) {
      f = 0.f;
      for (int i = 0; i < c->Hc; ++i) f = std::max(f, rm[(size_t)b * c->Hc + i]);
      max_logit[b] = f;
    }
    if (max_desc) { memcpy(&f, w + RANGE_MAX_DESC, 4); max_desc[b] = f; }
    if (nonfinite_input) nonfinite_input[b] = (int32_t)w[RANGE_BAD_INPUT];
  }
  return FPC_OK;
}

int fpc_get_keypoints(fpc_ctx* c, int frame, int cap, int32_t* xy, float* conf, float* desc) {
  if (!c || frame < 0 || frame >= c->B || cap < 0) return FPC_E_INVALID;
  HIPCHECK(hipSetDevice(c->cfg.device));
  HIPCHECK(hipStreamSynchronize(c->stream));
  int32_t k = 0;
  HIPCHECK(hipMemcpy(&k, c->count + frame, sizeof(k), hipMemcpyDeviceToHost));
  if (k > cap || k > c->cap) return FPC_E_CAPACITY;
  if (k == 0) return 0;
  if (xy) HIPCHECK(hipMemcpy(xy, c->xy + (size_t)frame * c->cap * 2, sizeof(int32_t) * 2 * k, hipMemcpyDeviceToHost));
  if (conf) HIPCHECK(hipMemcpy(conf, c->conf + (size_t)frame * c->cap, sizeof(float) * k, hipMemcpyDeviceToHost));
  if (desc) {
    if (!c->cfg.descriptor_enabled) return FPC_E_INVALID;
    HIPCHECK(hipMemcpy(desc, c->desc_out + (size_t)frame * c->cap * c->D, sizeof(float) * c->D * k, hipMemcpyDeviceToHost));
  }
  return k;
}

int fpc_set_timing(fpc_ctx* c, int enable) {
  if (!c) return FPC_E_INVALID;
  c->timing_every = enable > 0 ? enable : 0;
  c->timing_calls = 0;
  c->timing = enable != 0;
  c->timings.clear();
  c->events_used = 0;
  return FPC_OK;
}

int fpc_get_timings(fpc_ctx* c, int cap, const char** names, const char** kernels, float* ms, double* flops,
                    double* mfma_flops, double* bytes) {
  if (!c) return FPC_E_INVALID;
  const int n = (int)c->timings.size();
  for (int i = 0; i < n && i < cap; ++i) {
    const Timing& t = c->timings[i];
    float v = 0.f;
    if (hipEventElapsedTime(&v, t.start, t.stop) != hipSuccess) v = -1.f;
    const Op* op = t.op >= 0 ? &c->ops[t.op] : nullptr;
    if (names) names[i] = op ? op->name.c_str() : "?";
    if (kernels) {
      const char* k = "?";
      if (op) switch (op->type) {
          case OP_STEM: k = c->bf16 ? "stem_bf16_kernel" : c->split ? "stem_pool_x3_kernel" : c->stem2 ? "stem_pool2_kernel" : c->fuse_stem_pool ? "stem_pool_kernel" : "stem_kernel"; break;
          case OP_POOL: k = "maxpool_kernel"; break;
          case OP_CONV: k = op->lean ? lean_kind(op->kind)->symbol : g_kinds[op->kind].symbol; break;
          case OP_BLOCK: k = g_bkinds[op->bkind].symbol; break;
          case OP_WBLOCK: k = g_wkinds[op->wkind].symbol; break;
          case OP_BF16: k = g_fkinds[op->fkind].symbol; break;
          case OP_SOFTMAX: k = "softmax_d2s_kernel"; break;
          case OP_NMS: k = c->nms_one_workgroup ? "nms_rounds_kernel+nms_sort_kernel" : "nms_rounds_kernel+nms_finish_kernel+nms_chunk_sort_kernel+nms_merge_kernel"; break;
          case OP_DESC: k = "descriptor16_kernel"; break;
          case OP_VCONV0: k = "vgg_conv0_kernel"; break;
          case OP_POOL2: k = "maxpool2_kernel"; break;
          case OP_L2NORM: k = "l2norm256_kernel"; break;
        }
      kernels[i] = k;
    }
    if (ms) ms[i] = v;
    if (flops) flops[i] = op ? op->flops_per_frame * t.frames : 0.0;
    if (mfma_flops) mfma_flops[i] = op ? op->mfma_flops_per_frame * t.frames : 0.0;
    if (bytes) bytes[i] = op ? op->bytes_per_frame * t.frames : 0.0;
  }
  return n;
}

}
```

### feature-point-cnn_amd/csrc/wblock36_mfma.h

```cpp
#pragma once
#include <type_traits>
#include <utility>

#include "wblock16_mfma.h"

namespace fpc {

template <int... I, class F>
__device__ __forceinline__ void fpc_static_for_impl(std::integer_sequence<int, I...>, F&& f) {
  (f(std::integral_constant<int, I>{}), ...);
}
template <int N, class F>
__device__ __forceinline__ void fpc_static_for(F&& f) {
  fpc_static_for_impl(std::make_integer_sequence<int, N>{}, f);
}

struct W36Dust {
  static constexpr int W2ROW = 0, W2COL = 64, WPCOL = 144, B1 = 400, B2 = 401, UIN64 = 404, UIN = 448, UOUT = 448 + 4 * 36 * 16;
  static constexpr int floats(int nchunk) { return UOUT + nchunk * 36 * 16; }
};

template <int NB_, int TYT_, int TXT_, bool DUST_ = false>
struct W36Cfg {
  static constexpr int NB = NB_, TYT = TYT_, TXT = TXT_;
  static constexpr bool DUST = DUST_;
  static_assert(!DUST || NB == 1, "the dust channel rides on the 64-channel instance");
  static_assert(TYT * TXT == 16 && (TYT == 4 || TYT == 2), "16 Winograd tiles per workgroup tile: 4 x 4 or 2 x 8");
  static_assert(NB == 1 || NB == 2, "a wave owns 16 or 32 output channels");
  static constexpr int NT = 256, NPOS = 36, KC = 16;
  static constexpr int TH = 4 * TYT, TW = 4 * TXT, HH = TH + 2, HW = TW + 2, NHALO = HH * HW;
  static constexpr int N = 64 * NB;
  static constexpr int HROW = 20;
  static constexpr int HIT = (NHALO * 5 + NT - 1) / NT;
  static constexpr int HALO_FLOATS = HIT * NT * 4;
  static constexpr int V_FLOATS = NPOS * 16 * 16;
  static constexpr int OFF_V0 = 0, OFF_H1 = V_FLOATS, OFF_H0 = OFF_H1 + HALO_FLOATS, OFF_V1 = OFF_H0 + HALO_FLOATS;
  static constexpr int RH = N + 8;
  static constexpr int RX = 128 + 8;
  static constexpr int HPX = 128;
  static constexpr int T_FLOATS = HPX * (RH > RX ? RH : RX);
  static constexpr int BASE_FLOATS = (OFF_V1 + V_FLOATS) > (OFF_H0 + T_FLOATS) ? (OFF_V1 + V_FLOATS) : (OFF_H0 + T_FLOATS);
  static constexpr int HIT64 = (NHALO + NT - 1) / NT;
  static constexpr int D_HEAD = BASE_FLOATS, D_COL = D_HEAD + 64, D_UIN = D_HEAD + 448, D_V64 = D_UIN + 2304, D_M64 = D_V64 + 576, D_H64 = D_M64 + 576;
  static constexpr int LDS_FLOATS = DUST ? D_H64 + HIT64 * NT * 4 : BASE_FLOATS;
  static constexpr int LDS_BYTES = LDS_FLOATS * 4;
  static_assert(LDS_BYTES <= 160 * 1024, "LDS");
  static constexpr int STEPS = 18;
  static constexpr int RING = NB == 2 ? 6 : 9;
  static_assert(STEPS % RING == 0, "ring slots must line up across chunks");
  static constexpr int PAG = NB == 2 ? 30 : 36;
  static constexpr int WPAD = 36;
  static constexpr int WPAD2 = 16;
};

template <bool AG0, bool AG1, bool LAST_IN_ASM = false>
__device__ __forceinline__ void fpc_mfma_step(f32x4& c0, f32x4& c1, const f32x4& a0, const f32x4& a1, const f32x4& b0, const f32x4& b1) {
#define FPC_MFMA7                                                                                                      \
  "v_mfma_f32_16x16x4_f32 %0, %2, %10, %0\n\tv_mfma_f32_16x16x4_f32 %1, %6, %14, %1\n\t"                                \
  "v_mfma_f32_16x16x4_f32 %0, %3, %11, %0\n\tv_mfma_f32_16x16x4_f32 %1, %7, %15, %1\n\t"                                \
  "v_mfma_f32_16x16x4_f32 %0, %4, %12, %0\n\tv_mfma_f32_16x16x4_f32 %1, %8, %16, %1\n\t"                                \
  "v_mfma_f32_16x16x4_f32 %0, %5, %13, %0\n\t"
#define FPC_MFMA8 FPC_MFMA7 "v_mfma_f32_16x16x4_f32 %1, %9, %17, %1"
#define FPC_MFMA8_IN                                                                                                   \
  "v"(a0[0]), "v"(a0[1]), "v"(a0[2]), "v"(a0[3]), "v"(a1[0]), "v"(a1[1]), "v"(a1[2]), "v"(a1[3]), "v"(b0[0]), "v"(b0[1]), \
      "v"(b0[2]), "v"(b0[3]), "v"(b1[0]), "v"(b1[1]), "v"(b1[2]), "v"(b1[3])
  if constexpr (LAST_IN_ASM) {
    if constexpr (AG0 && AG1) asm volatile(FPC_MFMA8 : "+a"(c0), "+a"(c1) : FPC_MFMA8_IN);
    else if constexpr (AG0) asm volatile(FPC_MFMA8 : "+a"(c0), "+v"(c1) : FPC_MFMA8_IN);
    else if constexpr (AG1) asm volatile(FPC_MFMA8 : "+v"(c0), "+a"(c1) : FPC_MFMA8_IN);
    else asm volatile(FPC_MFMA8 : "+v"(c0), "+v"(c1) : FPC_MFMA8_IN);
  } else {
    if constexpr (AG0 && AG1) asm volatile(FPC_MFMA7 "s_nop 1" : "+a"(c0), "+a"(c1) : FPC_MFMA8_IN);
    else if constexpr (AG0) asm volatile(FPC_MFMA7 "s_nop 1" : "+a"(c0), "+v"(c1) : FPC_MFMA8_IN);
    else if constexpr (AG1) asm volatile(FPC_MFMA7 "s_nop 1" : "+v"(c0), "+a"(c1) : FPC_MFMA8_IN);
    else asm volatile(FPC_MFMA7 "s_nop 1" : "+v"(c0), "+v"(c1) : FPC_MFMA8_IN);
    c1 = __builtin_amdgcn_mfma_f32_16x16x4f32(a1[3], b1[3], c1, 0, 0, 0);
  }
#undef FPC_MFMA7
#undef FPC_MFMA8
#undef FPC_MFMA8_IN
}

#define W36_MARKER 0x7fffff00

template <bool AG>
__device__ __forceinline__ void fpc_mfma_step16(f32x4& c00, f32x4& c01, f32x4& c10, f32x4& c11, const f32x4& a0, const f32x4& a1,
                                                const f32x4& b00, const f32x4& b01, const f32x4& b10, const f32x4& b11) {
#define FPC_MFMA16                                                                                                      \
  "v_mfma_f32_16x16x4_f32 %0, %4, %12, %0\n\tv_mfma_f32_16x16x4_f32 %1, %4, %16, %1\n\t"                               \
  "v_mfma_f32_16x16x4_f32 %2, %8, %20, %2\n\tv_mfma_f32_16x16x4_f32 %3, %8, %24, %3\n\t"                               \
  "v_mfma_f32_16x16x4_f32 %0, %5, %13, %0\n\tv_mfma_f32_16x16x4_f32 %1, %5, %17, %1\n\t"                               \
  "v_mfma_f32_16x16x4_f32 %2, %9, %21, %2\n\tv_mfma_f32_16x16x4_f32 %3, %9, %25, %3\n\t"                               \
  "v_mfma_f32_16x16x4_f32 %0, %6, %14, %0\n\tv_mfma_f32_16x16x4_f32 %1, %6, %18, %1\n\t"                               \
  "v_mfma_f32_16x16x4_f32 %2, %10, %22, %2\n\tv_mfma_f32_16x16x4_f32 %3, %10, %26, %3\n\t"                             \
  "v_mfma_f32_16x16x4_f32 %0, %7, %15, %0\n\tv_mfma_f32_16x16x4_f32 %1, %7, %19, %1\n\t"                               \
  "v_mfma_f32_16x16x4_f32 %2, %11, %23, %2\n\tv_mfma_f32_16x16x4_f32 %3, %11, %27, %3"
#define FPC_MFMA16_IN                                                                                                   \
  "v"(a0[0]), "v"(a0[1]), "v"(a0[2]), "v"(a0[3]), "v"(a1[0]), "v"(a1[1]), "v"(a1[2]), "v"(a1[3]), "v"(b00[0]), "v"(b00[1]), \
      "v"(b00[2]), "v"(b00[3]), "v"(b01[0]), "v"(b01[1]), "v"(b01[2]), "v"(b01[3]), "v"(b10[0]), "v"(b10[1]), "v"(b10[2]),  \
      "v"(b10[3]), "v"(b11[0]), "v"(b11[1]), "v"(b11[2]), "v"(b11[3])
  if constexpr (AG) asm volatile(FPC_MFMA16 : "+a"(c00), "+a"(c01), "+a"(c10), "+a"(c11) : FPC_MFMA16_IN);
  else asm volatile(FPC_MFMA16 : "+v"(c00), "+v"(c01), "+v"(c10), "+v"(c11) : FPC_MFMA16_IN);
#undef FPC_MFMA16
#undef FPC_MFMA16_IN
}

template <int NB, int TYT, int TXT, bool DUST>
__device__ __forceinline__ void wblock36_body(const WBlockArgs& a) {
  using C = W36Cfg<NB, TYT, TXT, DUST>;
  constexpr int NT = C::NT, TH = C::TH, TW = C::TW, HW = C::HW, HH = C::HH, HROW = C::HROW, HIT = C::HIT;
  constexpr int N = C::N, RH = C::RH, RX = C::RX, RING = C::RING, STEPS = C::STEPS, HPX = C::HPX;
  extern __shared__ __attribute__((aligned(16))) float lds[];
  f32x4* const lds4 = reinterpret_cast<f32x4*>(lds);
  constexpr int TL4 = C::OFF_H0 / 4;

  const int tid = threadIdx.x, lane = tid & 63;
  const unsigned lane16 = (unsigned)lane * 16u;
  const int wave = __builtin_amdgcn_readfirstlane(tid >> 6);
  const int tiles = a.tiles_x * a.tiles_y;
  const int nchunk = a.nchunk;
  const float4* const w1h = a.w1 + (size_t)blockIdx.y * (a.ysplit_floats / 4);
  const float* const b1h = a.b1 + (size_t)blockIdx.y * a.ysplit_floats;

  const bool xcd_order = a.xcd_order && (gridDim.x & 7) == 0;
  const int wg_step = xcd_order ? (int)(gridDim.x >> 3) : (int)gridDim.x;
  const int xchunk = (a.total + 7) >> 3;
  const int wg_first = xcd_order ? (int)(blockIdx.x & 7) * xchunk + (int)(blockIdx.x >> 3) : (int)blockIdx.x;
  const int wg_end = xcd_order ? min(a.total, ((int)(blockIdx.x & 7) + 1) * xchunk) : a.total;
  if (wg_first >= wg_end) return;

  const __amdgpu_buffer_rsrc_t xrsrc = __builtin_amdgcn_make_buffer_rsrc(const_cast<float*>(a.x), 0, (int)a.x_bytes, 0x00020000);
  int okoff[HIT];
  int okoff64[DUST ? C::HIT64 : 1];
  struct TilePos { int b, ty, tx, live; };
  auto tile_pos = [&](int wg) {
    TilePos q;
    q.live = wg < wg_end;
    const int wgc = q.live ? wg : wg_first;
    const int bl = wgc / tiles;
    const int t = wgc - bl * tiles;
    q.b = a.frame0 + bl;
    q.ty = t / a.tiles_x;
    q.tx = t - q.ty * a.tiles_x;
    return q;
  };
  auto halo_base = [&](const TilePos& q) {
    return __builtin_amdgcn_readfirstlane(((q.b * a.H + q.ty * TH) * a.W + q.tx * TW) * a.csx * 4);
  };
  auto halo_tile = [&](const TilePos& q) {
    int tl = tid;
    asm volatile("" : "+v"(tl));
    const int iy0 = q.ty * TH - 1, ix0 = q.tx * TW - 1;
    const int hlim = q.live ? a.H : 0;
#pragma unroll
    for (int i = 0; i < HIT; ++i) {
      const int e = tl + i * NT;
      const int pix = (e * 13108) >> 16, c4 = e - pix * 5;
      const int hy = HW == 18 ? (pix * 3641) >> 16 : (pix * 1928) >> 16;
      const int hx = pix - hy * HW;
      const bool ok = ((unsigned)(iy0 + hy) < (unsigned)hlim) & ((unsigned)(ix0 + hx) < (unsigned)a.W) & (hy < HH) & (c4 < 4);
      const int off = (((hy - 1) * a.W + (hx - 1)) * a.csx + c4 * 4) * 4;
      okoff[i] = ok ? off : W36_MARKER;
    }
    if constexpr (DUST) {
#pragma unroll
      for (int i = 0; i < C::HIT64; ++i) {
        const int pix = tl + i * NT;
        const int hy = HW == 18 ? (pix * 3641) >> 16 : (pix * 1928) >> 16;
        const int hx = pix - hy * HW;
        const bool ok = ((unsigned)(iy0 + hy) < (unsigned)hlim) & ((unsigned)(ix0 + hx) < (unsigned)a.W) & (hy < HH) & (a.dust_in != 0);
        okoff64[i] = ok ? (((hy - 1) * a.W + (hx - 1)) * a.csx + 64) * 4 : W36_MARKER;
      }
    }
  };
  auto load_halo = [&](int base, int hoff) {
#pragma unroll
    for (int i = 0; i < HIT; ++i) {
      int voff;
      asm("v_add_i32 %0, %1, %2 clamp" : "=v"(voff) : "v"(okoff[i]), "s"(base));
      __builtin_amdgcn_raw_ptr_buffer_load_lds(xrsrc, (__attribute__((address_space(3))) void*)(lds + hoff + (i * NT + wave * 64) * 4), 16, voff, 0, 0, 0);
    }
  };
  auto load_halo64 = [&](int base) {
    if constexpr (DUST) {
#pragma unroll
      for (int i = 0; i < C::HIT64; ++i) {
        int voff;
        asm("v_add_i32 %0, %1, %2 clamp" : "=v"(voff) : "v"(okoff64[i]), "s"(base));
        __builtin_amdgcn_raw_ptr_buffer_load_lds(xrsrc, (__attribute__((address_space(3))) void*)(lds + C::D_H64 + (i * NT + wave * 64) * 4), 16, voff, 0, 0, 0);
      }
    }
  };
  const int wt_t = tid >> 4, ch_t = tid & 15;
  const int m_t = ((wt_t & 7) >> 1) * 4 + (wt_t >> 3) * 2 + (wt_t & 1);
  const int trd = ((4 * (wt_t / TXT)) * HW + 4 * (wt_t % TXT)) * HROW + ch_t;
  const int twr = m_t * 16 + ((((ch_t >> 2) ^ (2 * ((m_t >> 3) & 1))) << 2) | (ch_t & 3));
  typedef float f32x2 __attribute__((ext_vector_type(2)));
  f32x2 tp[6][3];
  auto t_read = [&](int rd, int i, int j) { tp[i][j >> 1][j & 1] = lds[rd + (i * HW + j) * HROW]; };
  auto bt6 = [&](f32x2& x0, f32x2& x1, f32x2& x2, f32x2& x3, f32x2& x4, f32x2& x5) {
    const f32x2 k4 = {4.f, 4.f}, km4 = {-4.f, -4.f}, k5 = {-5.f, -5.f}, k2 = {2.f, 2.f}, km2 = {-2.f, -2.f};
    const f32x2 p = __builtin_elementwise_fma(km4, x2, x4), q = __builtin_elementwise_fma(km4, x1, x3);
    const f32x2 r = x4 - x2, s = x3 - x1;
    const f32x2 y0 = __builtin_elementwise_fma(k4, x0, __builtin_elementwise_fma(k5, x2, x4));
    const f32x2 y5 = __builtin_elementwise_fma(k4, x1, __builtin_elementwise_fma(k5, x3, x5));
    x0 = y0;
    x1 = p + q;
    x2 = p - q;
    x3 = __builtin_elementwise_fma(k2, s, r);
    x4 = __builtin_elementwise_fma(km2, s, r);
    x5 = y5;
  };
  auto t_burst = [&]() {
#pragma unroll
    for (int jj = 0; jj < 3; ++jj) bt6(tp[0][jj], tp[1][jj], tp[2][jj], tp[3][jj], tp[4][jj], tp[5][jj]);
#pragma unroll
    for (int ii = 0; ii < 3; ++ii)
#pragma unroll
      for (int jj = 0; jj < 3; ++jj) {
        const f32x2 ra = tp[2 * ii][jj], rb = tp[2 * ii + 1][jj];
        tp[2 * ii][jj] = __builtin_shufflevector(ra, rb, 0, 2);
        tp[2 * ii + 1][jj] = __builtin_shufflevector(ra, rb, 1, 3);
      }
#pragma unroll
    for (int ii = 0; ii < 3; ++ii) bt6(tp[2 * ii][0], tp[2 * ii + 1][0], tp[2 * ii][1], tp[2 * ii + 1][1], tp[2 * ii][2], tp[2 * ii + 1][2]);
  };
  auto t_write = [&](int wr, int i, int j) { lds[wr + (i * 6 + j) * 256] = tp[2 * (i >> 1) + (j & 1)][j >> 1][i & 1]; };
  auto transform_all = [&](int hoff, int voff) {
#pragma unroll
    for (int i = 0; i < 6; ++i)
#pragma unroll
      for (int j = 0; j < 6; ++j) t_read(trd + hoff, i, j);
    t_burst();
#pragma unroll
    for (int i = 0; i < 6; ++i)
#pragma unroll
      for (int j = 0; j < 6; ++j) t_write(twr + voff, i, j);
  };

  const int aoff4 = (lane & 15) * 4 + ((lane >> 4) ^ (2 * ((lane & 15) >> 3)));
  const unsigned gstride = ((unsigned)nchunk * 36u + (unsigned)C::WPAD) * 1024u;
  const __amdgpu_buffer_rsrc_t wrsrc = __builtin_amdgcn_make_buffer_rsrc(const_cast<float4*>(w1h), 0, (int)(4u * (unsigned)NB * gstride), 0x00020000);
  const unsigned wlane = (unsigned)(wave * NB) * gstride + lane16;
  const int gs_s = __builtin_amdgcn_readfirstlane((int)gstride);
  struct BF { f32x4 v[2][NB]; };
  auto ldb = [&](int s) {
    BF r;
#pragma unroll
    for (int q = 0; q < 2; ++q)
#pragma unroll
      for (int nb = 0; nb < NB; ++nb)
        r.v[q][nb] = __builtin_bit_cast(f32x4, __builtin_amdgcn_raw_buffer_load_b128(wrsrc, (int)wlane, (2 * s + q) * 1024 + nb * gs_s, 0));
    return r;
  };

  [[maybe_unused]] int d_va = 0, d_ua = 0;
  [[maybe_unused]] const __amdgpu_buffer_rsrc_t drsrc =
      DUST ? __builtin_amdgcn_make_buffer_rsrc(const_cast<float*>(a.dust + W36Dust::UOUT), 0, nchunk * 36 * 16 * 4, 0x00020000) : xrsrc;
  [[maybe_unused]] f32x4 du[9];
  [[maybe_unused]] float dacc[9];
  if constexpr (DUST) {
    d_va = wave * 64 + lane;
    d_ua = wave * 64 + 16 * ((lane & 3) ^ (2 * (lane >> 5)));
    for (int i = tid; i < 448 / 4; i += NT) lds4[C::D_HEAD / 4 + i] = reinterpret_cast<const f32x4*>(a.dust)[i];
    for (int i = tid; i < 2304 / 4; i += NT) lds4[C::D_UIN / 4 + i] = reinterpret_cast<const f32x4*>(a.dust + W36Dust::UIN)[i];
  }

  TilePos pos_cur = tile_pos(wg_first);
  int base_cur = halo_base(pos_cur);
  halo_tile(pos_cur);
  load_halo64(base_cur);
  load_halo(base_cur, C::OFF_H0);
  load_halo(base_cur + 64, C::OFF_H1);
  asm volatile("s_waitcnt vmcnt(%0)" ::"n"(HIT) : "memory");
  FPC_LDS_BARRIER();
  transform_all(C::OFF_H0, C::OFF_V0);
  FPC_LDS_BARRIER();

  constexpr int C4 = N / 4, EIT = HPX * C4 / NT, PPI = NT / C4;
  constexpr int CPR = TW / PPI;
  const __amdgpu_buffer_rsrc_t orsrc = __builtin_amdgcn_make_buffer_rsrc(a.out + blockIdx.y * N, 0, W36_MARKER, 0x00020000);

  const int g2s = __builtin_amdgcn_readfirstlane(((a.k8_h + a.k8_x) / 2 + C::WPAD2) * 64);
  const __amdgpu_buffer_rsrc_t w2rsrc = __builtin_amdgcn_make_buffer_rsrc(const_cast<float4*>(a.w2), 0, a.conv_only ? 0 : 4 * NB * g2s * 16, 0x00020000);
  const unsigned w2lane = (unsigned)(wave * NB * g2s) * 16u + lane16;

  const int wg_stamp = wg_first + 2 * wg_step < wg_end ? wg_first + 2 * wg_step : wg_first;
  for (int wg = wg_first; wg < wg_end; wg += wg_step) {
    const int b = pos_cur.b, ty = pos_cur.ty, tx = pos_cur.tx;
    const TilePos pos_next = tile_pos(wg + wg_step);
    const int base_next = halo_base(pos_next);
    if (wg == wg_stamp) { FPC_STAMP(0) FPC_RSTAMP(6) }

    f32x4 acc[36][NB];
    {
      float zf = 0.f;
      asm volatile("" : "+v"(zf));
#pragma unroll
      for (int p = 0; p < 36; ++p)
#pragma unroll
        for (int nb = 0; nb < NB; ++nb) acc[p][nb] = f32x4{zf, zf, zf, zf};
    }

    BF bq[RING];
#pragma unroll
    for (int i = 0; i < RING - 1; ++i) bq[i] = ldb(i);
    if constexpr (DUST) {
      float zf = 0.f;
      asm volatile("" : "+v"(zf));
#pragma unroll
      for (int i = 0; i < 9; ++i) dacc[i] = zf;
    }

    auto chunk_body = [&](auto PAR, const int c) {
      constexpr int par = decltype(PAR)::value;
      constexpr int VB_OFF = par ? C::OFF_V1 : C::OFF_V0, VN_OFF = par ? C::OFF_V0 : C::OFF_V1;
      constexpr int HS_OFF = par ? C::OFF_H1 : C::OFF_H0;
      constexpr int HN_OFF = par ? C::OFF_H0 : C::OFF_H1;
      const int c3 = c + 2;
      const bool nxt = c3 >= nchunk;
      const int l_base = (nxt ? base_next : base_cur) + (nxt ? c3 - nchunk : c3) * 64;
      int ao = aoff4 + VB_OFF / 4, trd_c = trd + HN_OFF, twr_c = twr + VN_OFF;
      asm volatile("" : "+v"(ao), "+v"(trd_c), "+v"(twr_c));
      [[maybe_unused]] int dva = d_va + VB_OFF / 4;
      [[maybe_unused]] f32x4 dv[3];
      if constexpr (DUST) asm volatile("" : "+v"(dva));
      constexpr int AQ = 2;
      f32x4 ac[2][AQ];
#pragma unroll
      for (int q = 0; q < AQ; ++q) ac[0][q] = lds4[ao + q * 64];
#ifdef FPC_DIAG_STEPS
      unsigned long long tq[11] = {0, 0, 0, 0, 0, 0, 0, 0, 0, 0, 0};
#define FPC_TQ(i) asm volatile("s_memtime %0" : "=s"(tq[i]));
#else
#define FPC_TQ(i)
#endif
      fpc_static_for<STEPS>([&](auto S) __attribute__((always_inline)) {
        constexpr int s = decltype(S)::value;
        if constexpr (s % 2 == 0) { FPC_TQ(s / 2) }
        bq[(s + RING - 1) % RING] = ldb(c * STEPS + s + RING - 1);
        if (s + 1 < STEPS) {
#pragma unroll
          for (int q = 0; q < AQ; ++q) ac[(s + 1) & 1][q] = lds4[ao + ((s + 1) * AQ + q) * 64];
        }
        constexpr int SPS = 36 / STEPS;
#pragma unroll
        for (int u = 0; u < SPS; ++u) {
          const int slot = s * SPS + u;
          if (slot == 1) {
            if (c3 == nchunk) halo_tile(pos_next);
            load_halo(l_base, HS_OFF);
          } else if (slot >= 2 && slot < 14) {
#pragma unroll
            for (int k = 0; k < 3; ++k) { const int e = (slot - 2) * 3 + k; t_read(trd_c, e / 6, e % 6); }
          } else if (slot == 14) {
            t_burst();
          } else if (slot >= 15 && slot < 33) {
#pragma unroll
            for (int k = 0; k < 2; ++k) { const int e = (slot - 15) * 2 + k; t_write(twr_c, e / 6, e % 6); }
          }
          if constexpr (DUST) {
            auto dread = [&](int i0) {
#pragma unroll
              for (int k = 0; k < 3; ++k) dv[k] = lds4[dva + (i0 + k) * 256];
            };
            auto dfma = [&](int i0) {
#pragma unroll
              for (int k = 0; k < 3; ++k)
#pragma unroll
                for (int e = 0; e < 4; ++e) dacc[i0 + k] = __builtin_fmaf(dv[k][e], du[i0 + k][e], dacc[i0 + k]);
            };
            if (slot == 3) {
#pragma unroll
              for (int i = 0; i < 9; ++i)
                du[i] = __builtin_bit_cast(f32x4, __builtin_amdgcn_raw_buffer_load_b128(drsrc, d_ua + i * 256, c * (36 * 16 * 4), 0));
            } else if (slot == 23) {
              dread(0);
            } else if (slot == 25) {
              dfma(0);
              dread(3);
            } else if (slot == 27) {
              dfma(3);
              dread(6);
            } else if (slot == 29) {
              dfma(6);
            }
          }
        }
        __builtin_amdgcn_sched_barrier(0);
        {
          const BF& bv = bq[s % RING];
          constexpr int p0 = 2 * s, p1 = 2 * s + 1;
          if constexpr (NB == 2)
            fpc_mfma_step16<(p0 < C::PAG)>(acc[p0][0], acc[p0][1], acc[p1][0], acc[p1][1], ac[s & 1][0], ac[s & 1][1], bv.v[0][0], bv.v[0][1],
                                           bv.v[1][0], bv.v[1][NB - 1]);
          else
            fpc_mfma_step<true, true>(acc[p0][0], acc[p1][0], ac[s & 1][0], ac[s & 1][1], bv.v[0][0], bv.v[1][0]);
        }
        __builtin_amdgcn_sched_barrier(0);
      });
      FPC_TQ(9)
      asm volatile("s_waitcnt vmcnt(%0)" ::"n"(2 * NB * (RING - 1)) : "memory");
      FPC_LDS_BARRIER();
      FPC_TQ(10)
#ifdef FPC_DIAG_STEPS
      if (a.stamps && wg == wg_stamp && c == 2 && (threadIdx.x & 63) == 0) {
        asm volatile("s_waitcnt lgkmcnt(0)" ::: "memory");
        unsigned long long* q = a.stamps + 1024 * 8 + ((size_t)blockIdx.x * 4 + (threadIdx.x >> 6)) * 16;
        for (int i = 0; i < 11; ++i) q[i] = tq[i];
      }
#endif
    };
    __builtin_amdgcn_s_waitcnt(0x0F70);
    {
      int c = 0;
      do {
        chunk_body(std::integral_constant<int, 0>{}, c);
        chunk_body(std::integral_constant<int, 1>{}, c + 1);
        c += 2;
      } while (c < nchunk);
    }
    if (wg == wg_stamp) { FPC_STAMP(1) }
    asm volatile("s_nop 15\n\ts_nop 7" ::: "memory");

    if constexpr (DUST) {
      int tid_d = tid;
      asm volatile("" : "+v"(tid_d));
      const int lane_d = tid_d & 63;
      if (a.dust_in) {
        if (tid_d < 16) {
          const int rd = C::D_H64 + ((4 * (tid_d / TXT)) * HW + 4 * (tid_d % TXT)) * 4;
#pragma unroll
          for (int i = 0; i < 6; ++i)
#pragma unroll
            for (int j = 0; j < 6; ++j) tp[i][j >> 1][j & 1] = lds[rd + (i * HW + j) * 4];
          t_burst();
          const int mrow = ((tid_d & 7) >> 1) * 4 + (tid_d >> 3) * 2 + (tid_d & 1);
#pragma unroll
          for (int i = 0; i < 6; ++i)
#pragma unroll
            for (int j = 0; j < 6; ++j) lds[C::D_V64 + (i * 6 + j) * 16 + mrow] = tp[2 * (i >> 1) + (j & 1)][j >> 1][i & 1];
        }
        FPC_LDS_BARRIER();
        {
          const int va = C::D_V64 + (lane_d & 15), ub = C::D_UIN + wave * 576 + (lane_d & 15);
          float av[36], bv[36];
#pragma unroll
          for (int p = 0; p < 36; ++p) {
            av[p] = lds[va + p * 16];
            bv[p] = lds[ub + p * 16];
          }
          __builtin_amdgcn_sched_barrier(0);
#pragma unroll
          for (int p = 0; p < 36; ++p) {
            const float x = lane_d < 16 ? av[p] : 0.f;
            acc[p][0] = __builtin_amdgcn_mfma_f32_16x16x4f32(x, bv[p], acc[p][0], 0, 0, 0);
          }
        }
      }
      {
        const int m_d = lane_d >> 2;
#pragma unroll
        for (int i = 0; i < 9; ++i) {
          float v = dacc[i];
          v += __shfl_xor(v, 1);
          v += __shfl_xor(v, 2);
          const int pos = wave + 4 * i;
          if (a.dust_in) v = __builtin_fmaf(lds[C::D_V64 + pos * 16 + m_d], lds[C::D_HEAD + W36Dust::UIN64 + pos], v);
          if ((lane_d & 3) == 0) lds[C::D_M64 + pos * 16 + m_d] = v;
        }
      }
      FPC_LDS_BARRIER();
      load_halo64(base_next);
      if (tid_d < 16) {
        float mm[36];
#pragma unroll
        for (int p = 0; p < 36; ++p) mm[p] = lds[C::D_M64 + p * 16 + tid_d];
        const float bias1 = lds[C::D_HEAD + W36Dust::B1];
        float tt[4][6];
#pragma unroll
        for (int j = 0; j < 6; ++j) {
          const float m0 = mm[0 * 6 + j], m1 = mm[1 * 6 + j], m2 = mm[2 * 6 + j], m3 = mm[3 * 6 + j], m4 = mm[4 * 6 + j], m5 = mm[5 * 6 + j];
          const float s12 = m1 + m2, d12 = m1 - m2, s34 = m3 + m4, d34 = m3 - m4;
          tt[0][j] = m0 + s12 + s34;
          tt[1][j] = __builtin_fmaf(2.f, d34, d12);
          tt[2][j] = __builtin_fmaf(4.f, s34, s12);
          tt[3][j] = __builtin_fmaf(8.f, d34, d12) + m5;
        }
        const int T = 8 * ((tid_d >> 1) & 1) + 2 * (tid_d >> 2) + (tid_d & 1), th = T & 7;
        const int hb = C::OFF_H0 + ((4 * (th / TXT)) * TW + 4 * (th % TXT)) * RH + 64;
#pragma unroll
        for (int i = 0; i < 4; ++i) {
          const float m0 = tt[i][0], m1 = tt[i][1], m2 = tt[i][2], m3 = tt[i][3], m4 = tt[i][4], m5 = tt[i][5];
          const float s12 = m1 + m2, d12 = m1 - m2, s34 = m3 + m4, d34 = m3 - m4;
          float yv[4];
          yv[0] = m0 + s12 + s34 + bias1;
          yv[1] = __builtin_fmaf(2.f, d34, d12) + bias1;
          yv[2] = __builtin_fmaf(4.f, s34, s12) + bias1;
          yv[3] = __builtin_fmaf(8.f, d34, d12) + m5 + bias1;
#pragma unroll
          for (int jj = 0; jj < 4; ++jj) {
            const float v = yv[jj] > 0.f ? yv[jj] : 0.f;
            lds[T < 8 ? hb + (i * TW + jj) * RH : C::D_V64 + tid_d * 16 + i * 4 + jj] = v;
          }
        }
      }
    }

    int tid_t = tid;
    asm volatile("" : "+v"(tid_t));
    const int lane_t = tid_t & 63, n16 = lane_t & 15, kq = lane_t >> 4;
    const bool proj = a.k8_x > 0;
    float yh1[NB][2][16];
    int hw_base[2];
#pragma unroll
    for (int rr = 0; rr < 2; ++rr) {
      const int th = 2 * kq + rr;
      hw_base[rr] = C::OFF_H0 + ((4 * (th / TXT)) * TW + 4 * (th % TXT)) * RH + 16 * (wave * NB) + n16;
    }
#pragma unroll
    for (int nb = 0; nb < NB; ++nb) {
      const float bias1 = b1h[16 * (wave * NB + nb) + n16];
      if constexpr (NB == 1) {
#pragma unroll
      for (int rp = 0; rp < 2; ++rp) {
        __builtin_amdgcn_sched_barrier(0);
        f32x2 tt[4][6];
#pragma unroll
        for (int j = 0; j < 6; ++j) {
          auto pr = [&](int pos) { return f32x2{acc[pos][nb][2 * rp], acc[pos][nb][2 * rp + 1]}; };
          const f32x2 m0 = pr(0 * 6 + j), m1 = pr(1 * 6 + j), m2 = pr(2 * 6 + j), m3 = pr(3 * 6 + j), m4 = pr(4 * 6 + j), m5 = pr(5 * 6 + j);
          const f32x2 s12 = m1 + m2, d12 = m1 - m2, s34 = m3 + m4, d34 = m3 - m4;
          tt[0][j] = m0 + s12 + s34;
          tt[1][j] = __builtin_elementwise_fma(f32x2{2.f, 2.f}, d34, d12);
          tt[2][j] = __builtin_elementwise_fma(f32x2{4.f, 4.f}, s34, s12);
          tt[3][j] = __builtin_elementwise_fma(f32x2{8.f, 8.f}, d34, d12) + m5;
        }
        const f32x2 bias2 = {bias1, bias1}, zero2 = {0.f, 0.f};
#pragma unroll
        for (int i = 0; i < 4; ++i) {
          const f32x2 m0 = tt[i][0], m1 = tt[i][1], m2 = tt[i][2], m3 = tt[i][3], m4 = tt[i][4], m5 = tt[i][5];
          const f32x2 s12 = m1 + m2, d12 = m1 - m2, s34 = m3 + m4, d34 = m3 - m4;
          f32x2 yv[4];
          yv[0] = m0 + s12 + s34 + bias2;
          yv[1] = __builtin_elementwise_fma(f32x2{2.f, 2.f}, d34, d12) + bias2;
          yv[2] = __builtin_elementwise_fma(f32x2{4.f, 4.f}, s34, s12) + bias2;
          yv[3] = __builtin_elementwise_fma(f32x2{8.f, 8.f}, d34, d12) + m5 + bias2;
#pragma unroll
          for (int jj = 0; jj < 4; ++jj) {
            const f32x2 v = __builtin_elementwise_max(yv[jj], zero2);
#pragma unroll
            for (int e = 0; e < 2; ++e) {
              if (rp == 0) lds[hw_base[e] + 16 * nb + (i * TW + jj) * RH] = v[e];
              else yh1[nb][e][i * 4 + jj] = v[e];
            }
          }
        }
      }
      } else {
#pragma unroll
      for (int r = 0; r < 4; ++r) {
        __builtin_amdgcn_sched_barrier(0);
        float tt[4][6];
#pragma unroll
        for (int j = 0; j < 6; ++j) {
          const float m0 = acc[0 * 6 + j][nb][r], m1 = acc[1 * 6 + j][nb][r], m2 = acc[2 * 6 + j][nb][r];
          const float m3 = acc[3 * 6 + j][nb][r], m4 = acc[4 * 6 + j][nb][r], m5 = acc[5 * 6 + j][nb][r];
          const float s12 = m1 + m2, d12 = m1 - m2, s34 = m3 + m4, d34 = m3 - m4;
          tt[0][j] = m0 + s12 + s34;
          tt[1][j] = __builtin_fmaf(2.f, d34, d12);
          tt[2][j] = __builtin_fmaf(4.f, s34, s12);
          tt[3][j] = __builtin_fmaf(8.f, d34, d12) + m5;
        }
#pragma unroll
        for (int i = 0; i < 4; ++i) {
          const float m0 = tt[i][0], m1 = tt[i][1], m2 = tt[i][2], m3 = tt[i][3], m4 = tt[i][4], m5 = tt[i][5];
          const float s12 = m1 + m2, d12 = m1 - m2, s34 = m3 + m4, d34 = m3 - m4;
          float yv[4];
          yv[0] = m0 + s12 + s34 + bias1;
          yv[1] = __builtin_fmaf(2.f, d34, d12) + bias1;
          yv[2] = __builtin_fmaf(4.f, s34, s12) + bias1;
          yv[3] = __builtin_fmaf(8.f, d34, d12) + m5 + bias1;
#pragma unroll
          for (int jj = 0; jj < 4; ++jj) {
            const float v = yv[jj] > 0.f ? yv[jj] : 0.f;
            if (r < 2) lds[hw_base[r & 1] + 16 * nb + (i * TW + jj) * RH] = v;
            else yh1[nb][r - 2][i * 4 + jj] = v;
          }
        }
      }
      }
    }
    __builtin_amdgcn_sched_barrier(0);

    const int m0 = tid_t / C4, c4t = tid_t - m0 * C4;
    const int opart = (m0 * a.cso + c4t * 4) * 4;
    int ocol[CPR];
#pragma unroll
    for (int k = 0; k < CPR; ++k) ocol[k] = (tx * TW + m0 + k * PPI < a.W) ? opart + k * PPI * a.cso * 4 : W36_MARKER;

#pragma unroll
    for (int half = 0; half < 2; ++half) {
      const int y0 = ty * TH + half * (TH / 2), x0 = tx * TW;
      const int rows_valid = min(TH / 2, a.H - y0);
      const int xbase = __builtin_amdgcn_readfirstlane(((b * a.H + y0) * a.W + x0) * a.csx * 4);
      const int obase = __builtin_amdgcn_readfirstlane(((b * a.H + y0) * a.W + x0) * a.cso * 4);
      if (half == 1) {
#pragma unroll
        for (int nb = 0; nb < NB; ++nb)
#pragma unroll
          for (int rr = 0; rr < 2; ++rr)
#pragma unroll
            for (int i = 0; i < 4; ++i)
#pragma unroll
              for (int jj = 0; jj < 4; ++jj) lds[hw_base[rr] + 16 * nb + (i * TW + jj) * RH] = yh1[nb][rr][i * 4 + jj];
        if constexpr (DUST) {
          const int T = 8 * ((tid_t >> 1) & 1) + 2 * (tid_t >> 2) + (tid_t & 1), th = T & 7;
          if (tid_t < 16 && T >= 8) {
            const int hb = C::OFF_H0 + ((4 * (th / TXT)) * TW + 4 * (th % TXT)) * RH + 64;
#pragma unroll
            for (int i = 0; i < 4; ++i)
#pragma unroll
              for (int jj = 0; jj < 4; ++jj) lds[hb + (i * TW + jj) * RH] = lds[C::D_V64 + tid_t * 16 + i * 4 + jj];
          }
        }
      }
      FPC_LDS_BARRIER();
      if (wg == wg_stamp && half == 0) { FPC_STAMP(2) }
      [[maybe_unused]] float dpart[8];
      [[maybe_unused]] float dw2r = 0.f;
      [[maybe_unused]] float dhv[8][4];
      [[maybe_unused]] const int dq = lane_t & 15, dpxl = lane_t >> 4;
      [[maybe_unused]] float dx64 = 0.f;
      if constexpr (DUST) {
        if (!proj) {
          const int px = 32 * wave + 4 * (dq >> 1) + dpxl;
          dx64 = __builtin_bit_cast(float, __builtin_amdgcn_raw_buffer_load_b32(xrsrc, (((px / TW) * a.W + px % TW) * a.csx + 64) * 4, xbase, 0));
        }
        const f32x4 wq = lds4[C::D_COL / 4 + dq];
        const float w64 = dq == 0 ? lds[C::D_COL + 64] : 0.f;
#pragma unroll
        for (int it = 0; it < 8; ++it) {
          const int px = 32 * wave + 4 * it + dpxl;
          const f32x4 hq = lds4[TL4 + px * (RH / 4) + dq];
          const float h64 = lds[C::OFF_H0 + px * RH + 64];
          float v = h64 * w64;
#pragma unroll
          for (int e = 0; e < 4; ++e) v = __builtin_fmaf(hq[e], wq[e], v);
          dpart[it] = v;
        }
        dw2r = lds[C::D_HEAD + W36Dust::W2ROW + 16 * wave + (lane_t & 15)];
#pragma unroll
        for (int mb = 0; mb < 8; ++mb)
#pragma unroll
          for (int r = 0; r < 4; ++r) dhv[mb][r] = lds[C::OFF_H0 + (16 * mb + 4 * (lane_t >> 4) + r) * RH + 64];
      }
      int erd = TL4 + m0 * (RH / 4) + c4t;
      asm volatile("" : "+v"(erd));
      auto store_out = [&]() {
#pragma unroll
        for (int i = 0; i < EIT; ++i) {
          if (i / CPR < rows_valid) {
            f32x4 v = lds4[erd + i * PPI * (RH / 4)];
            if (!a.conv_only) {
              v.x = v.x > 0.f ? v.x : 0.f;
              v.y = v.y > 0.f ? v.y : 0.f;
              v.z = v.z > 0.f ? v.z : 0.f;
              v.w = v.w > 0.f ? v.w : 0.f;
            }
            int voff;
            const int so = obase + (i / CPR) * a.W * a.cso * 4;
            asm("v_add_i32 %0, %1, %2 clamp" : "=v"(voff) : "v"(ocol[i % CPR]), "s"(so));
            __builtin_amdgcn_raw_buffer_store_b128(__builtin_bit_cast(__attribute__((__vector_size__(4 * sizeof(unsigned)))) unsigned, v), orsrc, voff, 0, 0);
          }
        }
      };

      if (a.conv_only) {
        store_out();
        FPC_LDS_BARRIER();
        continue;
      }

      f32x4 acc2[8][NB];
      auto ldb2 = [&](int s, int nb) {
        return __builtin_bit_cast(f32x4, __builtin_amdgcn_raw_buffer_load_b128(w2rsrc, (int)w2lane, (nb * g2s + s * 64) * 16, 0));
      };
      constexpr int KH = N / 16;
      constexpr int NBLK = NB == 2 ? 8 : 4, APB = NB == 2 ? 1 : 2;
      auto gemm_over = [&](int row_pitch4, int ksteps, int s_first) {
        int ar = TL4 + n16 * row_pitch4 + kq;
        asm volatile("" : "+v"(ar));
        f32x4 cb[4][NB];
#pragma unroll
        for (int i = 0; i < 3; ++i)
#pragma unroll
          for (int nb = 0; nb < NB; ++nb) cb[i][nb] = ldb2(s_first + i, nb);
        f32x4 af[2][APB];
#pragma unroll
        for (int q = 0; q < APB; ++q) af[0][q] = lds4[ar + q * 16 * row_pitch4];
        for (int g = 0; g < ksteps; g += 4) {
#pragma unroll
          for (int u = 0; u < 4; ++u) {
#pragma unroll
            for (int nb = 0; nb < NB; ++nb) cb[(u + 3) & 3][nb] = ldb2(s_first + g + u + 3, nb);
            fpc_static_for<NBLK>([&](auto B_) __attribute__((always_inline)) {
              constexpr int blk = decltype(B_)::value;
              if (blk + 1 < NBLK) {
#pragma unroll
                for (int q = 0; q < APB; ++q) af[(blk + 1) & 1][q] = lds4[ar + (g + u) * 4 + ((blk + 1) * APB + q) * 16 * row_pitch4];
              } else {
#pragma unroll
                for (int q = 0; q < APB; ++q) af[(blk + 1) & 1][q] = lds4[ar + (g + u + 1) * 4 + q * 16 * row_pitch4];
              }
              __builtin_amdgcn_sched_barrier(0);
              if constexpr (NB == 2) fpc_mfma_step<true, true, true>(acc2[blk][0], acc2[blk][1], af[blk & 1][0], af[blk & 1][0], cb[u][0], cb[u][NB - 1]);
              else fpc_mfma_step<true, true>(acc2[2 * blk][0], acc2[2 * blk + 1][0], af[blk & 1][0], af[blk & 1][APB - 1], cb[u][0], cb[u][0]);
              __builtin_amdgcn_sched_barrier(0);
            });
          }
        }
      };
      if (proj) {
        constexpr int XIT = HPX * 32 / NT;
        f32x4 xst[XIT];
        auto load_x = [&](int pass) {
          const int kx4 = min(32, a.k8_x * 2 - pass * 32);
          const int xp = ((tid_t >> 5) * a.csx + ((tid_t & 31) < kx4 ? pass * 128 + (tid_t & 31) * 4 : 0)) * 4;
#pragma unroll
          for (int i = 0; i < XIT; ++i) {
            constexpr int XCPR = TW / 8;
            const int so = xbase + ((i / XCPR) * a.W + (i % XCPR) * 8) * a.csx * 4;
            xst[i] = __builtin_bit_cast(f32x4, __builtin_amdgcn_raw_buffer_load_b128(xrsrc, xp + so, 0, 0));
          }
        };
        load_x(0);
        {
          float zf = 0.f;
          asm volatile("" : "+v"(zf));
#pragma unroll
          for (int mb = 0; mb < 8; ++mb)
#pragma unroll
            for (int nb = 0; nb < NB; ++nb) acc2[mb][nb] = f32x4{zf, zf, zf, zf};
          if constexpr (DUST) {
#pragma unroll
            for (int mb = 0; mb < 8; ++mb)
#pragma unroll
              for (int r = 0; r < 4; ++r) acc2[mb][0][r] = dhv[mb][r] * dw2r;
          }
        }
        gemm_over(RH / 4, KH, 0);
        if (wg == wg_stamp && half == 0) { FPC_STAMP(3) }
        const int npass = (a.k8_x + 15) >> 4;
        for (int pass = 0; pass < npass; ++pass) {
          FPC_LDS_BARRIER();
          {
            int xw = TL4 + (tid_t >> 5) * (RX / 4) + (tid_t & 31);
            asm volatile("" : "+v"(xw));
#pragma unroll
            for (int i = 0; i < XIT; ++i) lds4[xw + i * 8 * (RX / 4)] = xst[i];
          }
          FPC_LDS_BARRIER();
          if (pass + 1 < npass) load_x(pass + 1);
          if constexpr (DUST) {
            const f32x4 wa = lds4[C::D_COL / 4 + 20 + pass * 32 + dq], wb = lds4[C::D_COL / 4 + 20 + pass * 32 + 16 + dq];
#pragma unroll
            for (int it = 0; it < 8; ++it) {
              const int px = 32 * wave + 4 * it + dpxl;
              const f32x4 xa = lds4[TL4 + px * (RX / 4) + dq], xb = lds4[TL4 + px * (RX / 4) + 16 + dq];
              float v = dpart[it];
#pragma unroll
              for (int e = 0; e < 4; ++e) v = __builtin_fmaf(xb[e], wb[e], __builtin_fmaf(xa[e], wa[e], v));
              dpart[it] = v;
            }
          }
          const int steps = min(8, a.k8_x / 2 - pass * 8);
          gemm_over(RX / 4, steps, KH + pass * 8);
        }
      } else {
        int xl = (4 * kq * a.csx + 16 * (wave * NB) + n16) * 4;
        asm volatile("" : "+v"(xl));
#pragma unroll
        for (int mb = 0; mb < 8; ++mb)
#pragma unroll
          for (int r = 0; r < 4; ++r) {
            constexpr int BPR = TW / 16;
            const int so = xbase + ((mb / BPR) * a.W + (mb % BPR) * 16 + r) * a.csx * 4;
#pragma unroll
            for (int nb = 0; nb < NB; ++nb)
              acc2[mb][nb][r] = __builtin_bit_cast(float, __builtin_amdgcn_raw_buffer_load_b32(xrsrc, xl + so + 64 * nb, 0, 0));
          }
        if constexpr (DUST) {
#pragma unroll
          for (int mb = 0; mb < 8; ++mb)
#pragma unroll
            for (int r = 0; r < 4; ++r) acc2[mb][0][r] = __builtin_fmaf(dhv[mb][r], dw2r, acc2[mb][0][r]);
        }
        gemm_over(RH / 4, KH, 0);
        if (wg == wg_stamp && half == 0) { FPC_STAMP(3) }
      }

      if (wg == wg_stamp && half == 0) { FPC_STAMP(4) }
      asm volatile("s_nop 15\n\ts_nop 7" ::: "memory");
      FPC_LDS_BARRIER();
      {
        int ew = C::OFF_H0 + (4 * kq) * RH + 16 * (wave * NB) + n16;
        asm volatile("" : "+v"(ew));
#pragma unroll
        for (int nb = 0; nb < NB; ++nb) {
          const float bias = a.b2[16 * (wave * NB + nb) + n16];
#pragma unroll
          for (int mb = 0; mb < 8; ++mb)
#pragma unroll
            for (int r = 0; r < 4; ++r) lds[ew + 16 * nb + (16 * mb + r) * RH] = acc2[mb][nb][r] + bias;
        }
      }
      FPC_LDS_BARRIER();
      store_out();
      if constexpr (DUST) {
        const bool b3 = (dq & 8) != 0, b2 = (dq & 4) != 0, b1 = (dq & 2) != 0;
        float r1[4], r2[2];
#pragma unroll
        for (int k = 0; k < 4; ++k) r1[k] = (b3 ? dpart[4 + k] : dpart[k]) + __shfl_xor(b3 ? dpart[k] : dpart[4 + k], 8);
#pragma unroll
        for (int k = 0; k < 2; ++k) r2[k] = (b2 ? r1[2 + k] : r1[k]) + __shfl_xor(b2 ? r1[k] : r1[2 + k], 4);
        float tot = (b1 ? r2[1] : r2[0]) + __shfl_xor(b1 ? r2[0] : r2[1], 2);
        tot += __shfl_xor(tot, 1);
        const int dpx = 32 * wave + 4 * (dq >> 1) + dpxl, dhf = dq & 1, drow = dpx / TW, dcol = dpx % TW;
        tot += dx64 + lds[C::D_HEAD + W36Dust::B2];
        tot = tot > 0.f ? tot : 0.f;
        const bool ok = (drow < rows_valid) & (x0 + dcol < a.W);
        const int doff = ok ? ((drow * a.W + dcol) * a.cso + 64 + 4 * dhf) * 4 : W36_MARKER;
        int voff;
        asm("v_add_i32 %0, %1, %2 clamp" : "=v"(voff) : "v"(doff), "s"(obase));
        const f32x4 v = {dhf ? 0.f : tot, 0.f, 0.f, 0.f};
        __builtin_amdgcn_raw_buffer_store_b128(__builtin_bit_cast(__attribute__((__vector_size__(4 * sizeof(unsigned)))) unsigned, v), orsrc, voff, 0, 0);
      }
      if (wg == wg_stamp && half == 0) { FPC_STAMP(5) FPC_RSTAMP(7) }
      FPC_LDS_BARRIER();
    }
    pos_cur = pos_next;
    base_cur = base_next;
  }
}

template <int NB, int TYT, int TXT>
__global__ __launch_bounds__(256, 1) void wblock36_kernel(const WBlockArgs a) {
  wblock36_body<NB, TYT, TXT, false>(a);
}

template <int TYT, int TXT>
__global__ __launch_bounds__(256, 1) void wblock36_dust_kernel(const WBlockArgs a) {
  wblock36_body<1, TYT, TXT, true>(a);
}

}
```

### feature-point-cnn_amd/csrc/wblock36p_mfma.h

```cpp
#pragma once
#include "wblock36_mfma.h"

namespace fpc {

template <int TYT_, int TXT_, bool DUST_ = false>
struct W36PCfg {
  static constexpr int TYT = TYT_, TXT = TXT_;
  static constexpr bool DUST = DUST_;
  static_assert(TYT * TXT == 16 && (TYT == 4 || TYT == 2), "16 Winograd tiles per workgroup tile: 4 x 4 or 2 x 8");
  static constexpr int NT = 512, NTH = 256, NPOS = 36, KC = 16, N = 64;
  static constexpr int TH = 4 * TYT, TW = 4 * TXT, HH = TH + 2, HW = TW + 2, NHALO = HH * HW;
  static constexpr int HROW = 20;
  static constexpr int HIT = (NHALO * 5 + NTH - 1) / NTH;
  static constexpr int HALO_FLOATS = HIT * NTH * 4;
  static constexpr int V_FLOATS = NPOS * 16 * 16;
  static constexpr int OFF_V0 = 0, OFF_H1 = V_FLOATS, OFF_H0 = OFF_H1 + HALO_FLOATS, OFF_V1 = OFF_H0 + HALO_FLOATS;
  static constexpr int RH = N + 8;
  static constexpr int PX = TH * TW;
  static constexpr int T_FLOATS = PX * RH;
  static constexpr int BASE_FLOATS = (OFF_V1 + V_FLOATS) > (OFF_H0 + T_FLOATS) ? (OFF_V1 + V_FLOATS) : (OFF_H0 + T_FLOATS);
  static constexpr int HIT64 = (NHALO + NTH - 1) / NTH;
  static constexpr int D_HEAD = BASE_FLOATS, D_COL = D_HEAD + 64, D_UIN = D_HEAD + 448, D_V64 = D_UIN + 2304, D_M64 = D_V64 + 576, D_H64 = D_M64 + 576;
  static constexpr int LDS_FLOATS = DUST ? D_H64 + HIT64 * NTH * 4 : BASE_FLOATS;
  static constexpr int LDS_BYTES = LDS_FLOATS * 4;
  static_assert(LDS_BYTES <= 160 * 1024, "LDS");
  static constexpr int STEPS = 9;
  static constexpr int WPAD = W36Cfg<1, TYT, TXT>::WPAD, WPAD2 = W36Cfg<1, TYT, TXT>::WPAD2;
  static_assert(WPAD >= 36, "a wave prefetches up to one chunk past its stream's end");
};

template <int TYT, int TXT, int RING, bool DUST>
__device__ __forceinline__ void wblock36p_body(const WBlockArgs& a) {
  using C = W36PCfg<TYT, TXT, DUST>;
  constexpr int TH = C::TH, TW = C::TW, HW = C::HW, HH = C::HH, HROW = C::HROW, HIT = C::HIT, NTH = C::NTH;
  constexpr int N = C::N, RH = C::RH, STEPS = C::STEPS, PX = C::PX;
  static_assert(STEPS % RING == 0 && RING >= 2, "ring slots must line up across chunks");
  extern __shared__ __attribute__((aligned(16))) float lds[];
  f32x4* const lds4 = reinterpret_cast<f32x4*>(lds);
  constexpr int TL4 = C::OFF_H0 / 4;

  const int tid = threadIdx.x, lane = tid & 63;
  const unsigned lane16 = (unsigned)lane * 16u;
  const int wave = __builtin_amdgcn_readfirstlane(tid >> 6);
  const int grp = wave & 3;
  const int hs = wave >> 2;
  const int tiles = a.tiles_x * a.tiles_y;
  const int nchunk = a.nchunk;
  const float4* const w1h = a.w1 + (size_t)blockIdx.y * (a.ysplit_floats / 4);
  const float* const b1h = a.b1 + (size_t)blockIdx.y * a.ysplit_floats;

  const bool xcd_order = a.xcd_order && (gridDim.x & 7) == 0;
  const int wg_step = xcd_order ? (int)(gridDim.x >> 3) : (int)gridDim.x;
  const int xchunk = (a.total + 7) >> 3;
  const int wg_first = xcd_order ? (int)(blockIdx.x & 7) * xchunk + (int)(blockIdx.x >> 3) : (int)blockIdx.x;
  const int wg_end = xcd_order ? min(a.total, ((int)(blockIdx.x & 7) + 1) * xchunk) : a.total;
  if (wg_first >= wg_end) return;

  const __amdgpu_buffer_rsrc_t xrsrc = __builtin_amdgcn_make_buffer_rsrc(const_cast<float*>(a.x), 0, (int)a.x_bytes, 0x00020000);
  struct TilePos { int b, ty, tx, live; };
  auto tile_pos = [&](int wg) {
    TilePos q;
    q.live = wg < wg_end;
    const int wgc = q.live ? wg : wg_first;
    const int bl = wgc / tiles;
    const int t = wgc - bl * tiles;
    q.b = a.frame0 + bl;
    q.ty = t / a.tiles_x;
    q.tx = t - q.ty * a.tiles_x;
    return q;
  };
  auto halo_base = [&](const TilePos& q) {
    return __builtin_amdgcn_readfirstlane(((q.b * a.H + q.ty * TH) * a.W + q.tx * TW) * a.csx * 4);
  };
  constexpr bool KEEP_HYX = !DUST;
  auto slot_hyx = [&](int tl, int i) {
    const int e = tl + i * NTH;
    const int pix = (e * 13108) >> 16, c4 = e - pix * 5;
    const int hy = HW == 18 ? (pix * 3641) >> 16 : (pix * 1928) >> 16;
    const int hx = pix - hy * HW;
    const bool slot_ok = (hy < HH) & (c4 < 4);
    return slot_ok ? (hy << 16) | (c4 << 8) | hx : 0x7fff0000;
  };
  int okoff[HIT];
  [[maybe_unused]] int hyx[KEEP_HYX ? HIT : 1];
  if (hs == 1) {
    const int tl = tid & (NTH - 1);
#pragma unroll
    for (int i = 0; i < HIT; ++i) {
      if constexpr (KEEP_HYX) hyx[i] = slot_hyx(tl, i);
      okoff[i] = W36_MARKER;
    }
  }
  [[maybe_unused]] int okoff64[C::HIT64];
  auto slot_hyx64 = [&](int tl, int i) {
    const int pix = tl + i * NTH;
    const int hy = HW == 18 ? (pix * 3641) >> 16 : (pix * 1928) >> 16;
    const int hx = pix - hy * HW;
    return (hy < HH && a.dust_in) ? (hy << 16) | hx : 0x7fff0000;
  };
  if constexpr (DUST) {
    if (hs == 1) {
#pragma unroll
      for (int i = 0; i < C::HIT64; ++i) okoff64[i] = W36_MARKER;
    }
  }
  auto halo_tile = [&](const TilePos& q) {
    const int iy0 = q.ty * TH - 1, ix0 = q.tx * TW - 1;
    const int hlim = q.live ? a.H : 0;
    int tlq = tid & (NTH - 1);
    asm volatile("" : "+v"(tlq));
#pragma unroll
    for (int i = 0; i < HIT; ++i) {
      int hv = KEEP_HYX ? hyx[KEEP_HYX ? i : 0] : slot_hyx(tlq, i);
      asm volatile("" : "+v"(hv));
      const int hy = hv >> 16, hx = hv & 0xff, c4 = (hv >> 8) & 0xff;
      const bool ok = ((unsigned)(iy0 + hy) < (unsigned)hlim) & ((unsigned)(ix0 + hx) < (unsigned)a.W);
      okoff[i] = ok ? (((hy - 1) * a.W + (hx - 1)) * a.csx + c4 * 4) * 4 : W36_MARKER;
    }
    if constexpr (DUST) {
#pragma unroll
      for (int i = 0; i < C::HIT64; ++i) {
        int hv = slot_hyx64(tlq, i);
        asm volatile("" : "+v"(hv));
        const int hy = hv >> 16, hx = hv & 0xffff;
        const bool ok = ((unsigned)(iy0 + hy) < (unsigned)hlim) & ((unsigned)(ix0 + hx) < (unsigned)a.W);
        okoff64[i] = ok ? (((hy - 1) * a.W + (hx - 1)) * a.csx + 64) * 4 : W36_MARKER;
      }
    }
  };
  auto load_halo64 = [&](int base) {
    if constexpr (DUST) {
#pragma unroll
      for (int i = 0; i < C::HIT64; ++i) {
        int voff;
        asm("v_add_i32 %0, %1, %2 clamp" : "=v"(voff) : "v"(okoff64[i]), "s"(base));
        __builtin_amdgcn_raw_ptr_buffer_load_lds(xrsrc, (__attribute__((address_space(3))) void*)(lds + C::D_H64 + (i * NTH + grp * 64) * 4), 16, voff, 0, 0, 0);
      }
    }
  };
  auto load_halo = [&](int base, int hoff_f) {
#pragma unroll
    for (int i = 0; i < HIT; ++i) {
      int voff;
      asm("v_add_i32 %0, %1, %2 clamp" : "=v"(voff) : "v"(okoff[i]), "s"(base));
      __builtin_amdgcn_raw_ptr_buffer_load_lds(xrsrc, (__attribute__((address_space(3))) void*)(lds + hoff_f + (i * NTH + grp * 64) * 4), 16, voff, 0, 0, 0);
    }
  };
  const int tq = tid & (NTH - 1);
  const int wt_t = tq >> 4, ch_t = tq & 15;
  const int m_t = ((wt_t & 7) >> 1) * 4 + (wt_t >> 3) * 2 + (wt_t & 1);
  const int trd = ((4 * (wt_t / TXT)) * HW + 4 * (wt_t % TXT)) * HROW + ch_t;
  const int twr = m_t * 16 + ((((ch_t >> 2) ^ (2 * ((m_t >> 3) & 1))) << 2) | (ch_t & 3));
  typedef float f32x2 __attribute__((ext_vector_type(2)));
  f32x2 tp[6][3];
  auto t_read = [&](int rd, int i, int j) { tp[i][j >> 1][j & 1] = lds[rd + (i * HW + j) * HROW]; };
  auto bt6 = [&](f32x2& x0, f32x2& x1, f32x2& x2, f32x2& x3, f32x2& x4, f32x2& x5) {
    const f32x2 k4 = {4.f, 4.f}, km4 = {-4.f, -4.f}, k5 = {-5.f, -5.f}, k2 = {2.f, 2.f}, km2 = {-2.f, -2.f};
    const f32x2 p = __builtin_elementwise_fma(km4, x2, x4), q = __builtin_elementwise_fma(km4, x1, x3);
    const f32x2 r = x4 - x2, s = x3 - x1;
    const f32x2 y0 = __builtin_elementwise_fma(k4, x0, __builtin_elementwise_fma(k5, x2, x4));
    const f32x2 y5 = __builtin_elementwise_fma(k4, x1, __builtin_elementwise_fma(k5, x3, x5));
    x0 = y0;
    x1 = p + q;
    x2 = p - q;
    x3 = __builtin_elementwise_fma(k2, s, r);
    x4 = __builtin_elementwise_fma(km2, s, r);
    x5 = y5;
  };
  auto t_burst = [&]() {
#pragma unroll
    for (int jj = 0; jj < 3; ++jj) bt6(tp[0][jj], tp[1][jj], tp[2][jj], tp[3][jj], tp[4][jj], tp[5][jj]);
#pragma unroll
    for (int ii = 0; ii < 3; ++ii)
#pragma unroll
      for (int jj = 0; jj < 3; ++jj) {
        const f32x2 ra = tp[2 * ii][jj], rb = tp[2 * ii + 1][jj];
        tp[2 * ii][jj] = __builtin_shufflevector(ra, rb, 0, 2);
        tp[2 * ii + 1][jj] = __builtin_shufflevector(ra, rb, 1, 3);
      }
#pragma unroll
    for (int ii = 0; ii < 3; ++ii) bt6(tp[2 * ii][0], tp[2 * ii + 1][0], tp[2 * ii][1], tp[2 * ii + 1][1], tp[2 * ii][2], tp[2 * ii + 1][2]);
  };
  auto t_write = [&](int wr, int i, int j) { lds[wr + (i * 6 + j) * 256] = tp[2 * (i >> 1) + (j & 1)][j >> 1][i & 1]; };

  const int aoff4 = (lane & 15) * 4 + ((lane >> 4) ^ (2 * ((lane & 15) >> 3))) + hs * 18 * 64;
  const unsigned gstride = ((unsigned)nchunk * 36u + (unsigned)C::WPAD) * 1024u;
  const __amdgpu_buffer_rsrc_t wrsrc = __builtin_amdgcn_make_buffer_rsrc(const_cast<float4*>(w1h), 0, (int)(4u * gstride), 0x00020000);
  const unsigned wlane = (unsigned)grp * gstride + (unsigned)hs * (18u * 1024u) + lane16;
  struct BF { f32x4 v[2]; };
  auto ldb = [&](int cc, int s) {
    BF r;
#pragma unroll
    for (int q = 0; q < 2; ++q)
      r.v[q] = __builtin_bit_cast(f32x4, __builtin_amdgcn_raw_buffer_load_b128(wrsrc, (int)wlane, cc * (36 * 1024) + (2 * s + q) * 1024, 0));
    return r;
  };

  [[maybe_unused]] int d_va = 0, d_ua = 0;
  [[maybe_unused]] const __amdgpu_buffer_rsrc_t drsrc =
      DUST ? __builtin_amdgcn_make_buffer_rsrc(const_cast<float*>(a.dust + W36Dust::UOUT), 0, nchunk * 36 * 16 * 4, 0x00020000) : xrsrc;
  [[maybe_unused]] f32x4 du[6];
  [[maybe_unused]] float dacc[9];
  if constexpr (DUST) {
    d_va = grp * 64 + lane;
    d_ua = grp * 64 + 16 * ((lane & 3) ^ (2 * (lane >> 5)));
    for (int i = tid; i < 448 / 4; i += C::NT) lds4[C::D_HEAD / 4 + i] = reinterpret_cast<const f32x4*>(a.dust)[i];
    for (int i = tid; i < 2304 / 4; i += C::NT) lds4[C::D_UIN / 4 + i] = reinterpret_cast<const f32x4*>(a.dust + W36Dust::UIN)[i];
  }

  TilePos pos_cur = tile_pos(wg_first);
  int base_cur = halo_base(pos_cur);
  if (hs == 1) {
    halo_tile(pos_cur);
    load_halo64(base_cur);
    load_halo(base_cur, C::OFF_H0);
    load_halo(base_cur + 64, C::OFF_H1);
    asm volatile("s_waitcnt vmcnt(%0)" ::"n"(HIT) : "memory");
  }
  FPC_LDS_BARRIER();
  if (hs == 0) {
#pragma unroll
    for (int i = 0; i < 6; ++i)
#pragma unroll
      for (int j = 0; j < 6; ++j) t_read(trd + C::OFF_H0, i, j);
    t_burst();
#pragma unroll
    for (int i = 0; i < 6; ++i)
#pragma unroll
      for (int j = 0; j < 6; ++j) t_write(twr + C::OFF_V0, i, j);
  }
  FPC_LDS_BARRIER();

  constexpr int C4 = N / 4, EIT = PX * C4 / C::NT, PPI = C::NT / C4;
  constexpr int RPI = PPI / TW > 0 ? PPI / TW : 1;
  const __amdgpu_buffer_rsrc_t orsrc = __builtin_amdgcn_make_buffer_rsrc(a.out + blockIdx.y * N, 0, W36_MARKER, 0x00020000);
  const int g2s = __builtin_amdgcn_readfirstlane(((a.k8_h + a.k8_x) / 2 + C::WPAD2) * 64);
  const __amdgpu_buffer_rsrc_t w2rsrc = __builtin_amdgcn_make_buffer_rsrc(const_cast<float4*>(a.w2), 0, a.conv_only ? 0 : 4 * g2s * 16, 0x00020000);
  const unsigned w2lane = (unsigned)(grp * g2s) * 16u + lane16;

  const int wg_stamp = wg_first + 2 * wg_step < wg_end ? wg_first + 2 * wg_step : wg_first;
  for (int wg = wg_first; wg < wg_end; wg += wg_step) {
    const int b = pos_cur.b, ty = pos_cur.ty, tx = pos_cur.tx;
    const TilePos pos_next = tile_pos(wg + wg_step);
    const int base_next = halo_base(pos_next);
    if (wg == wg_stamp) { FPC_STAMP(0) FPC_RSTAMP(6) }

    f32x4 acc[18];
    {
      float zf = 0.f;
      asm volatile("" : "+v"(zf));
#pragma unroll
      for (int p = 0; p < 18; ++p) acc[p] = f32x4{zf, zf, zf, zf};
    }
    if constexpr (DUST) {
      float zf = 0.f;
      asm volatile("" : "+v"(zf));
#pragma unroll
      for (int i = 0; i < 9; ++i) dacc[i] = zf;
    }
    BF bq[RING];
#pragma unroll
    for (int i = 0; i < RING - 1; ++i) bq[i] = ldb(0, i);

    auto chunk_body = [&](auto ROLE, auto PAR, const int c) {
      constexpr int role = decltype(ROLE)::value, par = decltype(PAR)::value;
      constexpr int VB_OFF = par ? C::OFF_V1 : C::OFF_V0, VN_OFF = par ? C::OFF_V0 : C::OFF_V1;
      constexpr int HS_OFF = par ? C::OFF_H1 : C::OFF_H0;
      constexpr int HN_OFF = par ? C::OFF_H0 : C::OFF_H1;
      const int c3 = c + 2;
      const bool nxt = c3 >= nchunk;
      const int l_base = (nxt ? base_next : base_cur) + (nxt ? c3 - nchunk : c3) * 64;
      int ao = aoff4 + VB_OFF / 4, trd_c = trd + HN_OFF, twr_c = twr + VN_OFF;
      asm volatile("" : "+v"(ao), "+v"(trd_c), "+v"(twr_c));
      [[maybe_unused]] int dva = d_va + VB_OFF / 4;
      [[maybe_unused]] f32x4 dv[3];
      if constexpr (DUST) asm volatile("" : "+v"(dva));
      f32x4 ac[2][2];
#pragma unroll
      for (int q = 0; q < 2; ++q) ac[0][q] = lds4[ao + q * 64];
      fpc_static_for<STEPS>([&](auto S) __attribute__((always_inline)) {
        constexpr int s = decltype(S)::value;
        {
          constexpr int t = s + RING - 1;
          if constexpr (t < STEPS) bq[t % RING] = ldb(c, t);
          else bq[t % RING] = ldb(c + 1, t - STEPS);
        }
        if (s + 1 < STEPS) {
#pragma unroll
          for (int q = 0; q < 2; ++q) ac[(s + 1) & 1][q] = lds4[ao + ((s + 1) * 2 + q) * 64];
        }
        constexpr int SPS = 4;
#pragma unroll
        for (int u = 0; u < SPS; ++u) {
          const int slot = s * SPS + u;
          if constexpr (role == 1) {
            if (slot == 1) {
              if (c3 == nchunk) halo_tile(pos_next);
              load_halo(l_base, HS_OFF);
            }
            if constexpr (DUST) {
              auto dread = [&](int i0) {
#pragma unroll
                for (int k = 0; k < 3; ++k) dv[k] = lds4[dva + (i0 + k) * 256];
              };
              auto dfma = [&](int i0) {
#pragma unroll
                for (int k = 0; k < 3; ++k)
#pragma unroll
                  for (int e = 0; e < 4; ++e) dacc[i0 + k] = __builtin_fmaf(dv[k][e], du[(i0 / 3 % 2) * 3 + k][e], dacc[i0 + k]);
              };
              auto dload = [&](int i0) {
#pragma unroll
                for (int k = 0; k < 3; ++k)
                  du[(i0 / 3 % 2) * 3 + k] = __builtin_bit_cast(f32x4, __builtin_amdgcn_raw_buffer_load_b128(drsrc, d_ua + (i0 + k) * 256, c * (36 * 16 * 4), 0));
              };
              if (slot == 3) dload(0);
              else if (slot == 11) dread(0);
              else if (slot == 13) { dfma(0); dload(3); }
              else if (slot == 21) dread(3);
              else if (slot == 23) { dfma(3); dload(6); }
              else if (slot == 31) dread(6);
              else if (slot == 33) dfma(6);
            }
          } else {
            if (slot >= 2 && slot < 14) {
#pragma unroll
              for (int k = 0; k < 3; ++k) { const int e = (slot - 2) * 3 + k; t_read(trd_c, e / 6, e % 6); }
            } else if (slot == 14) {
              t_burst();
            } else if (slot >= 15 && slot < 33) {
#pragma unroll
              for (int k = 0; k < 2; ++k) { const int e = (slot - 15) * 2 + k; t_write(twr_c, e / 6, e % 6); }
            }
          }
        }
        __builtin_amdgcn_sched_barrier(0);
        fpc_mfma_step<false, false>(acc[2 * s], acc[2 * s + 1], ac[s & 1][0], ac[s & 1][1], bq[s % RING].v[0], bq[s % RING].v[1]);
        __builtin_amdgcn_sched_barrier(0);
      });
      asm volatile("s_waitcnt vmcnt(%0)" ::"n"(2 * (STEPS - 1)) : "memory");
      FPC_LDS_BARRIER();
    };
    __builtin_amdgcn_s_waitcnt(0x0F70);
    if (hs == 0) {
      int c = 0;
      do {
        chunk_body(std::integral_constant<int, 0>{}, std::integral_constant<int, 0>{}, c);
        chunk_body(std::integral_constant<int, 0>{}, std::integral_constant<int, 1>{}, c + 1);
        c += 2;
      } while (c < nchunk);
    } else {
      int c = 0;
      do {
        chunk_body(std::integral_constant<int, 1>{}, std::integral_constant<int, 0>{}, c);
        chunk_body(std::integral_constant<int, 1>{}, std::integral_constant<int, 1>{}, c + 1);
        c += 2;
      } while (c < nchunk);
    }
    if (wg == wg_stamp) { FPC_STAMP(1) }
    asm volatile("s_nop 15\n\ts_nop 7" ::: "memory");

    int tid_t = tid;
    asm volatile("" : "+v"(tid_t));
    const int lane_t = tid_t & 63, n16 = lane_t & 15, kq = lane_t >> 4;
    const bool proj = a.k8_x > 0;
    if constexpr (DUST) {
      if (a.dust_in) {
        if (tid_t < 16) {
          const int rd = C::D_H64 + ((4 * (tid_t / TXT)) * HW + 4 * (tid_t % TXT)) * 4;
#pragma unroll
          for (int i = 0; i < 6; ++i)
#pragma unroll
            for (int j = 0; j < 6; ++j) tp[i][j >> 1][j & 1] = lds[rd + (i * HW + j) * 4];
          t_burst();
          const int mrow = ((tid_t & 7) >> 1) * 4 + (tid_t >> 3) * 2 + (tid_t & 1);
#pragma unroll
          for (int i = 0; i < 6; ++i)
#pragma unroll
            for (int j = 0; j < 6; ++j) lds[C::D_V64 + (i * 6 + j) * 16 + mrow] = tp[2 * (i >> 1) + (j & 1)][j >> 1][i & 1];
        }
        FPC_LDS_BARRIER();
        {
          const int va = C::D_V64 + hs * 18 * 16 + (lane_t & 15), ub = C::D_UIN + grp * 576 + hs * 18 * 16 + (lane_t & 15);
          float av[18], bv[18];
#pragma unroll
          for (int p = 0; p < 18; ++p) {
            av[p] = lds[va + p * 16];
            bv[p] = lds[ub + p * 16];
          }
          __builtin_amdgcn_sched_barrier(0);
#pragma unroll
          for (int p = 0; p < 18; ++p) {
            const float x = lane_t < 16 ? av[p] : 0.f;
            acc[p] = __builtin_amdgcn_mfma_f32_16x16x4f32(x, bv[p], acc[p], 0, 0, 0);
          }
        }
      }
      if (hs == 1) {
        const int m_d = lane_t >> 2;
#pragma unroll
        for (int i = 0; i < 9; ++i) {
          float v = dacc[i];
          v += __shfl_xor(v, 1);
          v += __shfl_xor(v, 2);
          const int pos = grp + 4 * i;
          if (a.dust_in) v = __builtin_fmaf(lds[C::D_V64 + pos * 16 + m_d], lds[C::D_HEAD + W36Dust::UIN64 + pos], v);
          if ((lane_t & 3) == 0) lds[C::D_M64 + pos * 16 + m_d] = v;
        }
      }
      FPC_LDS_BARRIER();
      if (hs == 1) load_halo64(base_next);
    }

    int hw_base[4];
#pragma unroll
    for (int r = 0; r < 4; ++r) {
      const int T = 8 * (r >> 1) + 2 * kq + (r & 1);
      hw_base[r] = C::OFF_H0 + ((4 * (T / TXT)) * TW + 4 * (T % TXT)) * RH + 16 * grp + n16;
    }
    auto out_transform = [&](auto ROLE) __attribute__((always_inline)) {
      constexpr int role = decltype(ROLE)::value;
      auto partial = [&](int rp, f32x2 (&yv)[4][4]) {
        f32x2 tt[4][6];
#pragma unroll
        for (int j = 0; j < 6; ++j) {
          auto pr = [&](int pos) { return f32x2{acc[pos][2 * rp], acc[pos][2 * rp + 1]}; };
          const f32x2 ma = pr(0 * 6 + j), mb = pr(1 * 6 + j), mc = pr(2 * 6 + j);
          if constexpr (role == 0) {
            const f32x2 s12 = mb + mc, d12 = mb - mc;
            tt[0][j] = ma + s12;
            tt[1][j] = d12;
            tt[2][j] = s12;
            tt[3][j] = d12;
          } else {
            const f32x2 s34 = ma + mb, d34 = ma - mb;
            tt[0][j] = s34;
            tt[1][j] = f32x2{2.f, 2.f} * d34;
            tt[2][j] = f32x2{4.f, 4.f} * s34;
            tt[3][j] = __builtin_elementwise_fma(f32x2{8.f, 8.f}, d34, mc);
          }
        }
#pragma unroll
        for (int i = 0; i < 4; ++i) {
          const f32x2 m0 = tt[i][0], m1 = tt[i][1], m2 = tt[i][2], m3 = tt[i][3], m4 = tt[i][4], m5 = tt[i][5];
          const f32x2 s12 = m1 + m2, d12 = m1 - m2, s34 = m3 + m4, d34 = m3 - m4;
          yv[i][0] = m0 + s12 + s34;
          yv[i][1] = __builtin_elementwise_fma(f32x2{2.f, 2.f}, d34, d12);
          yv[i][2] = __builtin_elementwise_fma(f32x2{4.f, 4.f}, s34, s12);
          yv[i][3] = __builtin_elementwise_fma(f32x2{8.f, 8.f}, d34, d12) + m5;
        }
      };
      {
        f32x2 yv[4][4];
        partial(1 - role, yv);
#pragma unroll
        for (int e = 0; e < 2; ++e)
#pragma unroll
          for (int i = 0; i < 4; ++i) lds4[TL4 + (e * 4 + i) * C::NT + tid_t] = f32x4{yv[i][0][e], yv[i][1][e], yv[i][2][e], yv[i][3][e]};
      }
      FPC_LDS_BARRIER();
      {
        f32x4 other[2][4];
#pragma unroll
        for (int e = 0; e < 2; ++e)
#pragma unroll
          for (int i = 0; i < 4; ++i) other[e][i] = lds4[TL4 + (e * 4 + i) * C::NT + (tid_t ^ NTH)];
        f32x2 yv[4][4];
        partial(role, yv);
        const float bias1 = b1h[16 * grp + n16];
        float hv[2][16];
#pragma unroll
        for (int i = 0; i < 4; ++i)
#pragma unroll
          for (int jj = 0; jj < 4; ++jj)
#pragma unroll
            for (int e = 0; e < 2; ++e) {
              const float v = (yv[i][jj][e] + other[e][i][jj]) + bias1;
              hv[e][i * 4 + jj] = v > 0.f ? v : 0.f;
            }
        FPC_LDS_BARRIER();
#pragma unroll
        for (int e = 0; e < 2; ++e)
#pragma unroll
          for (int i = 0; i < 4; ++i)
#pragma unroll
            for (int jj = 0; jj < 4; ++jj) lds[hw_base[2 * role + e] + (i * TW + jj) * RH] = hv[e][i * 4 + jj];
        if constexpr (DUST && role == 0) {
          if (tid_t < 16) {
            float mm[36];
#pragma unroll
            for (int p = 0; p < 36; ++p) mm[p] = lds[C::D_M64 + p * 16 + tid_t];
            const float bias64 = lds[C::D_HEAD + W36Dust::B1];
            float tt[4][6];
#pragma unroll
            for (int j = 0; j < 6; ++j) {
              const float m0 = mm[0 * 6 + j], m1 = mm[1 * 6 + j], m2 = mm[2 * 6 + j], m3 = mm[3 * 6 + j], m4 = mm[4 * 6 + j], m5 = mm[5 * 6 + j];
              const float s12 = m1 + m2, d12 = m1 - m2, s34 = m3 + m4, d34 = m3 - m4;
              tt[0][j] = m0 + s12 + s34;
              tt[1][j] = __builtin_fmaf(2.f, d34, d12);
              tt[2][j] = __builtin_fmaf(4.f, s34, s12);
              tt[3][j] = __builtin_fmaf(8.f, d34, d12) + m5;
            }
            const int T = 8 * ((tid_t >> 1) & 1) + 2 * (tid_t >> 2) + (tid_t & 1);
            const int hb = C::OFF_H0 + ((4 * (T / TXT)) * TW + 4 * (T % TXT)) * RH + 64;
#pragma unroll
            for (int i = 0; i < 4; ++i) {
              const float m0 = tt[i][0], m1 = tt[i][1], m2 = tt[i][2], m3 = tt[i][3], m4 = tt[i][4], m5 = tt[i][5];
              const float s12 = m1 + m2, d12 = m1 - m2, s34 = m3 + m4, d34 = m3 - m4;
              float yv64[4];
              yv64[0] = m0 + s12 + s34 + bias64;
              yv64[1] = __builtin_fmaf(2.f, d34, d12) + bias64;
              yv64[2] = __builtin_fmaf(4.f, s34, s12) + bias64;
              yv64[3] = __builtin_fmaf(8.f, d34, d12) + m5 + bias64;
#pragma unroll
              for (int jj = 0; jj < 4; ++jj) lds[hb + (i * TW + jj) * RH] = yv64[jj] > 0.f ? yv64[jj] : 0.f;
            }
          }
        }
      }
      FPC_LDS_BARRIER();
    };
    if (hs == 0) out_transform(std::integral_constant<int, 0>{});
    else out_transform(std::integral_constant<int, 1>{});
    if (wg == wg_stamp) { FPC_STAMP(2) }

    const int y0 = ty * TH, x0 = tx * TW;
    const int rows_valid = min(TH, a.H - y0);
    const int xbase = __builtin_amdgcn_readfirstlane(((b * a.H + y0) * a.W + x0) * a.csx * 4);
    const int obase = __builtin_amdgcn_readfirstlane(((b * a.H + y0) * a.W + x0) * a.cso * 4);
    const int m0 = tid_t / C4, c4t = tid_t - m0 * C4;
    const int rsub = __builtin_amdgcn_readfirstlane(m0 / TW), pcol = m0 % TW;
    const int ocol = (x0 + pcol < a.W) ? (pcol * a.cso + c4t * 4) * 4 : W36_MARKER;
    int erd = TL4 + m0 * (RH / 4) + c4t;
    asm volatile("" : "+v"(erd));
    auto store_out = [&]() {
#pragma unroll
      for (int i = 0; i < EIT; ++i) {
        const int prow = i * RPI + rsub;
        if (prow < rows_valid) {
          f32x4 v = lds4[erd + i * PPI * (RH / 4)];
          if (!a.conv_only) {
            v.x = v.x > 0.f ? v.x : 0.f;
            v.y = v.y > 0.f ? v.y : 0.f;
            v.z = v.z > 0.f ? v.z : 0.f;
            v.w = v.w > 0.f ? v.w : 0.f;
          }
          int voff;
          const int so = obase + prow * a.W * a.cso * 4;
          asm("v_add_i32 %0, %1, %2 clamp" : "=v"(voff) : "v"(ocol), "s"(so));
          __builtin_amdgcn_raw_buffer_store_b128(__builtin_bit_cast(__attribute__((__vector_size__(4 * sizeof(unsigned)))) unsigned, v), orsrc, voff, 0, 0);
        }
      }
    };

    if (a.conv_only) {
      store_out();
      FPC_LDS_BARRIER();
    } else {
      f32x4 acc2[8];
      const int pb = hs;
      [[maybe_unused]] float dpart[8];
      [[maybe_unused]] float dw2r = 0.f;
      [[maybe_unused]] float dhv[8][4];
      [[maybe_unused]] const int dq = lane_t & 15, dpxl = lane_t >> 4;
// ... 186 lines not shown
```

### feature-point-cnn_amd/csrc/wblock_mfma.h

```cpp
#pragma once
#include "block_mfma.h"

namespace fpc {

struct WBlockArgs {
  const float* x;
  int csx, nchunk;
  int H, W;
  const float4* w1;
  const float* b1;
  const float4* w2;
  const float* b2;
  int k8_h, k8_x;
  float* out;
  int cso, tiles_x, tiles_y, frame0;
  int total;
  int xcd_order;
  int ysplit_floats;
  unsigned x_bytes;
  int conv_only;
  const float* dust;
  int dust_in;
#ifdef FPC_DIAG
  unsigned long long* stamps;
#endif
};

template <int KC, int NBT, int CMID_>
struct WBlockCfg {
  static constexpr int TH = 8, TW = 16, NT = 512;
  static constexpr int HW = TW + 2, HH = TH + 2;
  static constexpr int ROW4 = KC / 4 + 1;
  static constexpr int CMID = CMID_;
  static constexpr int ROWH4 = CMID / 4 + 1;
  static constexpr int HALO_BYTES = HH * HW * ROW4 * 16;
  static constexpr int V_BYTES = 16 * 32 * ROW4 * 16;
  static constexpr int M_BYTES = 16 * 32 * 36 * 4;
  static constexpr int H_BYTES = 128 * ROWH4 * 16;
  static constexpr int LDS_BYTES = (HALO_BYTES + V_BYTES) > (M_BYTES + H_BYTES) ? (HALO_BYTES + V_BYTES) : (M_BYTES + H_BYTES);
  static constexpr int GN = NBT >= 4 ? 2 : 1;
  static constexpr int GX = 8 / GN;
  static constexpr int PX = 16 / GX;
  static constexpr int NBW = NBT / GN;
};

__device__ __forceinline__ float4 fpc_ldg_su(const float4* ubase, unsigned lane_bytes) {
  typedef const char __attribute__((address_space(1))) * gptr;
  typedef float f4v __attribute__((ext_vector_type(4)));
  gptr b = (gptr) reinterpret_cast<const char*>(ubase);
  asm("" : "+s"(b));
  const f4v v = *reinterpret_cast<const f4v __attribute__((address_space(1)))*>(b + lane_bytes);
  return make_float4(v.x, v.y, v.z, v.w);
}

template <int KC, int NBT, int CMID_>
__global__ __launch_bounds__(512, 2) void wblock_mfma_kernel(const WBlockArgs a) {
  using C = WBlockCfg<KC, NBT, CMID_>;
  constexpr int NT = C::NT, TH = C::TH, TW = C::TW, HW = C::HW, HH = C::HH, ROW4 = C::ROW4, K8 = KC / 8, KC4 = KC / 4;
  constexpr int NV = HH * HW * KC4, ITER = (NV + NT - 1) / NT, ROWH4 = C::ROWH4, CMID = C::CMID;
  constexpr int GN = C::GN, PX = C::PX, NBW = C::NBW;
  extern __shared__ float4 lds4[];
  float4* halo4 = lds4;
  float4* v4 = lds4 + C::HALO_BYTES / 16;

  const int tid = threadIdx.x, lane = tid & 63;
  const unsigned lane16 = (unsigned)lane * 16u;
  const int wave = __builtin_amdgcn_readfirstlane(tid >> 6);
  const int gx = wave / GN, gn = wave % GN;
  const int half = lane >> 5, l31 = lane & 31;
  const int tiles = a.tiles_x * a.tiles_y;
  FPC_STAMP(0)

  float4 stage[ITER];
  auto load_chunk = [&](int wg, int chunk) {
    const int bl = wg / tiles;
    const int bb = a.frame0 + bl;
    const int t = wg - bl * tiles;
    const int tyy = t / a.tiles_x, txx = t - tyy * a.tiles_x;
    const int iy0 = tyy * TH - 1, ix0 = txx * TW - 1;
#pragma unroll
    for (int i = 0; i < ITER; ++i) {
      const int e = tid + i * NT;
      const int pix = e / KC4, c4 = e - pix * KC4;
      const int hy = pix / HW, hx = pix - hy * HW;
      const int iy = iy0 + hy, ix = ix0 + hx;
      const bool ok = (NV % NT == 0 || e < NV) && iy >= 0 && iy < a.H && ix >= 0 && ix < a.W;
      const size_t off = ok ? ((size_t)(bb * a.H + iy) * a.W + ix) * a.csx + chunk * KC + c4 * 4 : 0;
      float4 v = *reinterpret_cast<const float4*>(a.x + off);
      if (!ok) v = make_float4(0.f, 0.f, 0.f, 0.f);
      stage[i] = v;
    }
  };
  auto store_chunk = [&]() {
#pragma unroll
    for (int i = 0; i < ITER; ++i) {
      const int e = tid + i * NT;
      const int pix = e / KC4, c4 = e - pix * KC4;
      if (NV % NT == 0 || e < NV) halo4[pix * ROW4 + c4] = stage[i];
    }
  };

  constexpr int STEPS = PX * K8;
  constexpr int stepstride = NBT * 64;
  constexpr bool PIN = NBT != 3;
  const float4* wbase = a.w1 + (size_t)(gx * PX * K8 * NBT + gn * NBW) * 64 + (PIN ? 0 : lane);
  auto ldw = [&](const float4* pw) { return PIN ? fpc_ldg_su(pw, lane16) : *pw; };
  auto wptr = [&](int s) {
    const int chunk = s / STEPS, ls = s - chunk * STEPS;
    return wbase + (size_t)(chunk * 16 * K8 + ls) * stepstride;
  };

  const bool xcd_order = a.xcd_order && (gridDim.x & 7) == 0;
  const int wg_step = xcd_order ? (int)(gridDim.x >> 3) : (int)gridDim.x;
  const int xchunk = (a.total + 7) >> 3;
  const int wg_first = xcd_order ? (int)(blockIdx.x & 7) * xchunk + (int)(blockIdx.x >> 3) : (int)blockIdx.x;
  const int wg_end = xcd_order ? min(a.total, ((int)(blockIdx.x & 7) + 1) * xchunk) : a.total;
  if (wg_first < wg_end) load_chunk(wg_first, 0);
  const int wg_stamp = wg_first + 2 * wg_step < wg_end ? wg_first + 2 * wg_step : wg_first;
  for (int wg = wg_first; wg < wg_end; wg += wg_step) {
  const int bl = wg / tiles;
  const int b = a.frame0 + bl;
  const int t = wg - bl * tiles;
  const int ty = t / a.tiles_x, tx = t - ty * a.tiles_x;
  if (wg == wg_stamp && wg != wg_first) { FPC_STAMP(0) }
  int tid_t = tid;
  asm volatile("" : "+v"(tid_t));

  f32x16 acc[PX][NBW];
#pragma unroll
  for (int p = 0; p < PX; ++p)
#pragma unroll
    for (int nb = 0; nb < NBW; ++nb)
#pragma unroll
      for (int r = 0; r < 16; ++r) acc[p][nb][r] = 0.f;

  float4 b0[NBW], b1[NBW];
  {
    const float4* p0 = wptr(0);
    const float4* p1 = wptr(1);
#pragma unroll
    for (int nb = 0; nb < NBW; ++nb) {
      b0[nb] = ldw(p0 + nb * 64);
      b1[nb] = ldw(p1 + nb * 64);
    }
  }
  int gs = 0;
  for (int chunk = 0; chunk < a.nchunk; ++chunk) {
    FPC_LDS_BARRIER();
    store_chunk();
    FPC_LDS_BARRIER();
    if (chunk == 0 && wg == wg_stamp) { FPC_STAMP(6) }
    if (chunk + 1 < a.nchunk) load_chunk(wg, chunk + 1);
    else if (wg + wg_step < wg_end) load_chunk(wg + wg_step, 0);
    {
      const float2* halo2 = reinterpret_cast<const float2*>(halo4);
      float2* v2 = reinterpret_cast<float2*>(v4);
      for (int item = tid_t; item < 32 * (KC / 2); item += NT) {
        const int c2 = item % (KC / 2), wt = item / (KC / 2);
        const int ty2 = wt >> 3, tx2 = wt & 7;
        const int base = ((2 * ty2) * HW + 2 * tx2) * (ROW4 * 2) + c2;
        float2 d[4][4];
#pragma unroll
        for (int i = 0; i < 4; ++i)
#pragma unroll
          for (int j = 0; j < 4; ++j) d[i][j] = halo2[base + (i * HW + j) * (ROW4 * 2)];
        float2 r[4][4];
#pragma unroll
        for (int j = 0; j < 4; ++j) {
          r[0][j] = make_float2(d[0][j].x - d[2][j].x, d[0][j].y - d[2][j].y);
          r[1][j] = make_float2(d[1][j].x + d[2][j].x, d[1][j].y + d[2][j].y);
          r[2][j] = make_float2(d[2][j].x - d[1][j].x, d[2][j].y - d[1][j].y);
          r[3][j] = make_float2(d[1][j].x - d[3][j].x, d[1][j].y - d[3][j].y);
        }
#pragma unroll
        for (int i = 0; i < 4; ++i) {
// ... 270 lines not shown
```

### include/fpc.h

```cpp
#ifndef FPC_H
#define FPC_H

#include <stddef.h>
#include <stdint.h>

#ifdef __cplusplus
extern "C" {
#endif

#define FPC_ABI_VERSION 4
#define FPC_PACK_LAYOUT_REVISION 4

enum {
  FPC_OK = 0,
  FPC_E_INVALID = -1,
  FPC_E_NO_DEVICE = -2,
  FPC_E_HIP = -3,
  FPC_E_NO_WEIGHTS = -4,
  FPC_E_MISSING_KEY = -5,
  FPC_E_CAPACITY = -6,
  FPC_E_NOT_CONVERGED = -7,
  FPC_E_RANGE = -8,
  FPC_E_NONFINITE = -9
};


enum { FPC_F32 = 0, FPC_BF16 = 1, FPC_F32_SPLIT = 2, FPC_F32_SPLIT_F16 = 3 };
enum { FPC_ARCH_RESNET = 0, FPC_ARCH_VGG = 1 };

typedef struct fpc_config {
  int device;
  int height, width;
  int max_batch;
  int cell;
  int nms_dist;
  float conf_thresh;
  int border_remove;
  int descriptor_enabled;
  int max_keypoints;
  int in_channels;
  int dtype;
  int arch;
  int num_streams;
  unsigned plan_flags;
  int nms_round_launches;
  int min_sub_batch;
} fpc_config;

enum {
  FPC_PLAN_NO_FUSED_BLOCKS = 1 << 0,
  FPC_PLAN_NO_WINOGRAD = 1 << 1,
  FPC_PLAN_NO_WINOGRAD_DETECTOR = 1 << 2,
  FPC_PLAN_NO_WINOGRAD_LAYER_IN1 = 1 << 3,
  FPC_PLAN_NO_XCD_ORDER = 1 << 4,
  FPC_PLAN_NO_FUSED_STEM_POOL = 1 << 5,
  FPC_PLAN_SPLIT_HEADS = 1 << 6,
  FPC_PLAN_NMS_IN_LINE = 1 << 7,
  FPC_PLAN_NO_PERSISTENT_GRID = 1 << 8,
  FPC_PLAN_LAYER1_TILE_8x16 = 1 << 9,
  FPC_PLAN_WINOGRAD_GEN1 = 1 << 10,
  FPC_PLAN_NO_LATENCY_TILES = 1 << 11,
  FPC_PLAN_NMS_ONE_WORKGROUP = 1 << 12,
  FPC_PLAN_NO_FUSED_SOFTMAX = 1 << 13,
  FPC_PLAN_WINOGRAD_GEN2 = 1 << 14,
  FPC_PLAN_HEADS_IN_LINE = 1 << 17,
  FPC_PLAN_DETECTOR_GEN1 = 1 << 16,
  FPC_PLAN_W36_ONE_WAVE = 1 << 18,
  FPC_PLAN_STEM_ROUND3 = 1 << 20,
  FPC_PLAN_CONV_ROUND1 = 1 << 21,
  FPC_PLAN_CONVT_PHASES = 1 << 19,
  FPC_PLAN_GUARD_ZONES = 1 << 15
};

typedef struct fpc_tensor {
  const char* name;
  const float* data;
  int ndim;
  int64_t shape[4];
} fpc_tensor;

typedef struct fpc_device_results {
  const int32_t* count;
  const int32_t* n_candidates;
  const int32_t* xy;
  const float* conf;
  const float* desc;
  int capacity;
  int desc_dim;
} fpc_device_results;

typedef struct fpc_ctx fpc_ctx;

int fpc_abi_version(void);
const char* fpc_build_flags(void);
const char* fpc_strerror(int code);
const char* fpc_last_hip_error(void);

int fpc_default_config(fpc_config* cfg);

int fpc_create(fpc_ctx** out, const fpc_config* cfg);
void fpc_destroy(fpc_ctx* ctx);

int fpc_load_weights(fpc_ctx* ctx, const fpc_tensor* tensors, int n);

size_t fpc_packed_size(const fpc_ctx* ctx);
void* fpc_packed_device_ptr(fpc_ctx* ctx);
int fpc_export_packed(fpc_ctx* ctx, void* host_dst, size_t cap);
int fpc_import_packed(fpc_ctx* ctx, const void* host_src, size_t n);
int fpc_import_packed_device(fpc_ctx* ctx, const void* dev_src, size_t n);
int fpc_mark_weights_loaded(fpc_ctx* ctx);
uint64_t fpc_plan_hash(const fpc_ctx* ctx);
int fpc_pack_layout_revision(void);

int fpc_check_guards(fpc_ctx* ctx, long long* bad_words);

int fpc_broadcast_weights(fpc_ctx* ctx, void* nccl_comm, int root);

int fpc_set_stream(fpc_ctx* ctx, void* hip_stream);
void* fpc_get_stream(fpc_ctx* ctx);
void* fpc_upload_stream(fpc_ctx* ctx);
typedef struct fpc_stream_report_t {
  int n_streams;
  int slot[16], queue[16];
  int probing;
  int hw_queues_found;
  int process_probe_rounds, process_probe_launches, process_inconclusive_rounds;
  float process_probe_ms;
  int create_probe_rounds;
  float create_placement_ms;
  int process_registered_streams;
} fpc_stream_report_t;
int fpc_stream_report(fpc_ctx* ctx, fpc_stream_report_t* out);
int fpc_sync(fpc_ctx* ctx);

int fpc_forward(fpc_ctx* ctx, const float* frames_dev, int n, float* prob_map_dev,
                float* desc_dev, float* logits_dev);

int fpc_read_activation(fpc_ctx* ctx, const char* name, int frame0, int n, float* out_dev, int* channels, int* height,
                        int* width);

int fpc_detect(fpc_ctx* ctx, const float* frames_dev, int n);

enum { FPC_U8_GRAY = 0, FPC_U8_RGB_HWC = 1, FPC_U8_BGR_HWC = 2, FPC_U8_BGR_HWC_GRAY = 3 };
int fpc_detect_u8(fpc_ctx* ctx, const uint8_t* frames_dev, int n, int layout);
int fpc_detect_u8_resized(fpc_ctx* ctx, const uint8_t* frames_dev, int n, int src_h, int src_w, int layout);
const float* fpc_u8_staging(fpc_ctx* ctx);

int fpc_homography_adaptation(fpc_ctx* ctx, const float* frames_dev, int n, const float* homographies_host,
                              const float* inverses_host, int num, int erosion_radius, int aggregation,
                              float* prob_out_dev);

int fpc_get_points(fpc_ctx* ctx, const float* prob_map_dev, const float* desc_nchw_dev, int n);

int fpc_sample_descriptors(fpc_ctx* ctx, const float* desc_nchw_dev, const double* xy_dev, int k, float* out_dev);

int fpc_match(fpc_ctx* ctx, const float* q_dev, int nq, const float* t_dev, int nt, int cross_check,
              float max_dist, int32_t* match_dev, float* dist_dev);
int fpc_first_within(fpc_ctx* ctx, const float* key_dev, int nk, const float* cur_dev, int nc,
                     float tolerance, int32_t* first_dev);

enum { FPC_PAIR_KEY = 0, FPC_PAIR_PREVIOUS = 1 };
int fpc_match_frames(fpc_ctx* ctx, int n, int pairing, const float* key_dev, const int32_t* nkey_dev,
                     int cross_check, float max_dist, float ratio, int32_t* match_dev, float* dist_dev);
int fpc_first_within_frames(fpc_ctx* ctx, int n, const float* key_dev, const int32_t* nkey_dev,
                            float tolerance, int32_t* first_dev);

typedef struct fpc_ransac_params {
  int      iterations;
  float    reproj_threshold;
  uint32_t seed;
  int      refits;
  int      min_inliers;
} fpc_ransac_params;
int fpc_default_ransac_params(fpc_ransac_params* params);
int fpc_ransac_homography(fpc_ctx* ctx, int n, const float* src_xy_dev, const float* dst_xy_dev, const int32_t* npairs_dev,
                          int stride, const fpc_ransac_params* params, float* H_dev, int32_t* ninliers_dev,
                          uint8_t* inlier_dev);
int fpc_homography_frames(fpc_ctx* ctx, int n, int pairing, const int32_t* key_xy_dev, const int32_t* nkey_dev,
                          const int32_t* match_dev, const fpc_ransac_params* params, float* H_dev, int32_t* ninliers_dev,
                          uint8_t* inlier_dev);

#define FPC_BANK_MAX_SLOTS 1024
typedef struct fpc_bank_view {
  const float*   desc;
  const int32_t* xy;
  const int32_t* count;
  int slots, rows, desc_dim;
  int chunk;
  size_t bytes;
} fpc_bank_view;
int fpc_bank_create(fpc_ctx* ctx, int slots, int rows);
int fpc_bank_destroy(fpc_ctx* ctx);
int fpc_bank_get(fpc_ctx* ctx, fpc_bank_view* out);
int fpc_bank_store(fpc_ctx* ctx, int frame, int slot);
int fpc_bank_store_rows(fpc_ctx* ctx, int slot, const float* desc_dev, const int32_t* xy_dev, const int32_t* n_dev);
int fpc_bank_clear(fpc_ctx* ctx, int slot);
int fpc_match_bank(fpc_ctx* ctx, int n, int cross_check, float max_dist, float ratio, int min_score, int32_t* score_dev,
                   int32_t* best_dev, int32_t* match_dev, float* dist_dev);
int fpc_homography_bank(fpc_ctx* ctx, int n, const int32_t* slot_dev, const int32_t* match_dev,
                        const fpc_ransac_params* params, float* H_dev, int32_t* ninliers_dev, uint8_t* inlier_dev);

int fpc_ransac_fundamental(fpc_ctx* ctx, int n, const float* src_xy_dev, const float* dst_xy_dev, const int32_t* npairs_dev,
                           int stride, const fpc_ransac_params* params, float* F_dev, int32_t* ninliers_dev,
                           uint8_t* inlier_dev);
int fpc_fundamental_frames(fpc_ctx* ctx, int n, int pairing, const int32_t* key_xy_dev, const int32_t* nkey_dev,
                           const int32_t* match_dev, const fpc_ransac_params* params, float* F_dev, int32_t* ninliers_dev,
                           uint8_t* inlier_dev);
int fpc_fundamental_bank(fpc_ctx* ctx, int n, const int32_t* slot_dev, const int32_t* match_dev,
                         const fpc_ransac_params* params, float* F_dev, int32_t* ninliers_dev, uint8_t* inlier_dev);

#define FPC_BANK_F32  0
#define FPC_BANK_BF16 1
int fpc_bank_create_ex(fpc_ctx* ctx, int slots, int rows, int format);
int fpc_bank_format(fpc_ctx* ctx, int* format, const void** desc);

int fpc_match_frames_guided(fpc_ctx* ctx, int n, int pairing, const float* key_dev, const int32_t* nkey_dev,
                            const int32_t* key_xy_dev, const float* H_dev, float radius, int cross_check, float max_dist,
                            float ratio, int32_t* match_dev, float* dist_dev);
int fpc_match_bank_guided(fpc_ctx* ctx, int n, const int32_t* slot_dev, const float* H_dev, float radius, int cross_check,
                          float max_dist, float ratio, int32_t* match_dev, float* dist_dev);

int fpc_cell_order(fpc_ctx* ctx, const int32_t* xy_dev, const int32_t* n_dev, int sets, int stride, int32_t* perm_dev);
// ... 36 lines not shown
```

Baseline: 12050.

## Stack frames vertically in w36 Winograd blocks to remove partial-tile waste

When the frame height is not a multiple of the 16-row Winograd tile, batched frames are launched as one tall stacked image. Tiles that straddle a frame boundary insert a zero halo row at the seam, so each frame keeps its own padding. This reduces the idle partial tiles at the bottom of each frame. The cost is extra index logic in the halo loaders, a seam word stored in LDS, and per-tile shifted read offsets. The MFMA FLOP accounting is rescaled to match the tiles actually run.

```diff
diff --git a/feature-point-cnn_amd/_lib.py b/feature-point-cnn_amd/_lib.py
--- a/feature-point-cnn_amd/_lib.py
+++ b/feature-point-cnn_amd/_lib.py
@@ -36,6 +36,7 @@
     "no_xcd_order": 1 << 4, "no_fused_stem_pool": 1 << 5, "split_heads": 1 << 6, "nms_in_line": 1 << 7,
     "no_persistent_grid": 1 << 8, "layer1_tile_8x16": 1 << 9, "winograd_gen1": 1 << 10, "no_latency_tiles": 1 << 11,
     "nms_one_workgroup": 1 << 12, "no_fused_softmax": 1 << 13, "winograd_gen2": 1 << 14, "guard_zones": 1 << 15, "detector_gen1": 1 << 16, "heads_in_line": 1 << 17, "w36_one_wave": 1 << 18, "convt_phases": 1 << 19, "stem_round3": 1 << 20, "conv_round1": 1 << 21,
+    "no_stacked_tiles": 1 << 22,
 }
 
 
diff --git a/feature-point-cnn_amd/csrc/fpc_api.hip b/feature-point-cnn_amd/csrc/fpc_api.hip
--- a/feature-point-cnn_amd/csrc/fpc_api.hip
+++ b/feature-point-cnn_amd/csrc/fpc_api.hip
@@ -444,6 +444,7 @@
   hipEvent_t start, stop;
   int op;
   int frames;
+  double mfma_scale;
 };
 
 }
@@ -500,6 +501,7 @@
   bool winograd_in1 = true;
   bool winograd_det = true;
   int w36_cus = 0;
+  bool w36_stacked = true;
   bool w36_paired = true;
   bool winograd_det_gen3 = true;
   bool winograd = true;
@@ -2354,6 +2356,7 @@
   int op;
   hipStream_t st;
   int frames;
+  double mfma_scale = 1.0;
   hipEvent_t s{}, e{};
   LaunchTimer(fpc_ctx* c_, int op_, hipStream_t st_, int frames_) : c(c_), op(op_), st(st_), frames(frames_) {
     if (c->timing) {
@@ -2365,7 +2368,7 @@
   ~LaunchTimer() {
     if (c->timing) {
       hipEventRecord(e, st);
-      c->timings.push_back({s, e, op, frames});
+      c->timings.push_back({s, e, op, frames, mfma_scale});
     }
   }
 };
@@ -2484,19 +2487,28 @@
           const int fpl = w36_frames_per_launch(a.H, a.W, a.csx, a.cso);
           const float* x0 = a.x;
           float* o0 = a.out;
+          const int H1 = a.H, tiles_y1 = a.tiles_y, TH = g_wkinds[op.wkind].TH;
+          const bool stackable = c->w36_stacked && TH == 16 && H1 % TH != 0 && H1 % 4 == 0 && H1 >= 20;
+          long long tiles_run = 0;
           for (int g0 = 0; g0 < n; g0 += fpl) {
             const int gn = std::min(fpl, n - g0);
+            const bool stacked = stackable && gn > 1;
             a.frame0 = 0;
-            a.x = x0 + (size_t)(f0 + g0) * a.H * a.W * a.csx;
-            a.out = o0 + (size_t)(f0 + g0) * a.H * a.W * a.cso;
-            a.total = a.tiles_x * a.tiles_y * gn;
-            a.x_bytes = (unsigned)((unsigned long long)gn * a.H * a.W * a.csx * sizeof(float));
+            a.x = x0 + (size_t)(f0 + g0) * H1 * a.W * a.csx;
+            a.out = o0 + (size_t)(f0 + g0) * H1 * a.W * a.cso;
+            a.H = stacked ? gn * H1 : H1;
+            a.frame_rows = stacked ? H1 : 0;
+            a.tiles_y = stacked ? (gn * H1 + TH - 1) / TH : tiles_y1;
+            a.total = a.tiles_x * a.tiles_y * (stacked ? 1 : gn);
+            tiles_run += a.total;
+            a.x_bytes = (unsigned)((unsigned long long)gn * H1 * a.W * a.csx * sizeof(float));
             const int cus_cap = c->w36_cus > 0 ? std::min(c->num_cus, c->w36_cus) : c->num_cus;
             const int cus8 = std::max(1, cus_cap / 8 / std::max(1, op.grid_y)), per_xcd = (a.total + 7) / 8;
             const int rounds = (per_xcd + cus8 - 1) / cus8;
             const int grid3 = 8 * std::min(cus8, (per_xcd + rounds - 1) / rounds);
             g_wkinds[op.wkind].launch(a, dim3(std::min(a.total, grid3), op.grid_y), sb.st);
           }
+          t.mfma_scale = (double)tiles_run / ((double)a.tiles_x * tiles_y1 * n);
           break;
         }
         g_wkinds[op.wkind].launch(a, dim3(std::min(a.total, grid), op.grid_y), sb.st);
@@ -2900,6 +2912,8 @@
     c->winograd_det_gen3 = !(pf & FPC_PLAN_DETECTOR_GEN1);
     c->w36_paired = !(pf & FPC_PLAN_W36_ONE_WAVE);
     if (const char* e = getenv("FPC_W36_PAIRED")) c->w36_paired = atoi(e) != 0;
+    c->w36_stacked = !(pf & FPC_PLAN_NO_STACKED_TILES);
+    if (const char* e = getenv("FPC_STACKED_TILES")) c->w36_stacked = atoi(e) != 0;
     if (const char* e = getenv("FPC_W36_CUS")) c->w36_cus = std::max(0, atoi(e));
     if (const char* e = getenv("FPC_WINOGRAD_DET_GEN")) c->winograd_det_gen3 = atoi(e) >= 3;
     c->winograd = !(pf & FPC_PLAN_NO_WINOGRAD);
@@ -4305,7 +4319,7 @@
     }
     if (ms) ms[i] = v;
     if (flops) flops[i] = op ? op->flops_per_frame * t.frames : 0.0;
-    if (mfma_flops) mfma_flops[i] = op ? op->mfma_flops_per_frame * t.frames : 0.0;
+    if (mfma_flops) mfma_flops[i] = op ? op->mfma_flops_per_frame * t.frames * t.mfma_scale : 0.0;
     if (bytes) bytes[i] = op ? op->bytes_per_frame * t.frames : 0.0;
   }
   return n;
diff --git a/feature-point-cnn_amd/csrc/w36_seam.h b/feature-point-cnn_amd/csrc/w36_seam.h
--- /dev/null
+++ b/feature-point-cnn_amd/csrc/w36_seam.h
@@ -0,0 +1,33 @@
+#pragma once
+
+#define FPC_SEAM_FN __host__ __device__ inline
+
+namespace fpc {
+
+constexpr int W36_SEAM_NONE = 0xff;
+constexpr int W36_SEAM_ZERO = -0x40000000;
+
+FPC_SEAM_FN int w36_seam(int y0, int frame_rows, int th) {
+  if (frame_rows <= 0) return W36_SEAM_NONE;
+  const int r = (y0 + frame_rows - 1) / frame_rows * frame_rows - y0;
+  if (r > th) return W36_SEAM_NONE;
+  if (r == 0) return 0;
+  return r < th ? (r + 1) | (1 << 8) : th + 1;
+}
+FPC_SEAM_FN int w36_seam_zero_row(int seam) { return seam & 0xff; }
+FPC_SEAM_FN int w36_seam_inserted(int seam) { return seam >> 8; }
+FPC_SEAM_FN int w36_seam_rows(int seam, int th) { return th + 2 + w36_seam_inserted(seam); }
+FPC_SEAM_FN int w36_seam_tile_row(int seam, int hy) {
+  const int z = w36_seam_zero_row(seam);
+  if (hy == z) return W36_SEAM_ZERO;
+  return hy - 1 - (w36_seam_inserted(seam) && hy > z ? 1 : 0);
+}
+FPC_SEAM_FN int w36_seam_patch_shift(int seam, int wr) {
+  return w36_seam_inserted(seam) && 4 * wr + 1 >= w36_seam_zero_row(seam) ? 1 : 0;
+}
+FPC_SEAM_FN int w36_seam_source_row(int y0, int frame_rows, int th, int hy) {
+  const int t = w36_seam_tile_row(w36_seam(y0, frame_rows, th), hy);
+  return t == W36_SEAM_ZERO ? W36_SEAM_ZERO : y0 + t;
+}
+
+}
diff --git a/feature-point-cnn_amd/csrc/wblock36_mfma.h b/feature-point-cnn_amd/csrc/wblock36_mfma.h
--- a/feature-point-cnn_amd/csrc/wblock36_mfma.h
+++ b/feature-point-cnn_amd/csrc/wblock36_mfma.h
@@ -2,6 +2,7 @@
 #include <type_traits>
 #include <utility>
 
+#include "w36_seam.h"
 #include "wblock16_mfma.h"
 
 namespace fpc {
@@ -42,6 +43,7 @@
   static constexpr int BASE_FLOATS = (OFF_V1 + V_FLOATS) > (OFF_H0 + T_FLOATS) ? (OFF_V1 + V_FLOATS) : (OFF_H0 + T_FLOATS);
   static constexpr int HIT64 = (NHALO + NT - 1) / NT;
   static constexpr int D_HEAD = BASE_FLOATS, D_COL = D_HEAD + 64, D_UIN = D_HEAD + 448, D_V64 = D_UIN + 2304, D_M64 = D_V64 + 576, D_H64 = D_M64 + 576;
+  static constexpr int D_SEAM = D_HEAD + 402;
   static constexpr int LDS_FLOATS = DUST ? D_H64 + HIT64 * NT * 4 : BASE_FLOATS;
   static constexpr int LDS_BYTES = LDS_FLOATS * 4;
   static_assert(LDS_BYTES <= 160 * 1024, "LDS");
@@ -110,6 +112,8 @@
   using C = W36Cfg<NB, TYT, TXT, DUST>;
   constexpr int NT = C::NT, TH = C::TH, TW = C::TW, HW = C::HW, HH = C::HH, HROW = C::HROW, HIT = C::HIT;
   constexpr int N = C::N, RH = C::RH, RX = C::RX, RING = C::RING, STEPS = C::STEPS, HPX = C::HPX;
+  constexpr bool SEAM = TYT == 4;
+  static_assert(!SEAM || ((HH + 1) * HW * 5 <= HIT * NT && (HH + 1) * HW <= (DUST ? C::HIT64 : 2) * NT), "an inserted halo row must fit the requests");
   extern __shared__ __attribute__((aligned(16))) float lds[];
   f32x4* const lds4 = reinterpret_cast<f32x4*>(lds);
   constexpr int TL4 = C::OFF_H0 / 4;
@@ -135,13 +139,14 @@
   struct TilePos { int b, ty, tx, live; };
   auto tile_pos = [&](int wg) {
     TilePos q;
-    q.live = wg < wg_end;
-    const int wgc = q.live ? wg : wg_first;
+    const bool live = wg < wg_end;
+    const int wgc = live ? wg : wg_first;
     const int bl = wgc / tiles;
     const int t = wgc - bl * tiles;
     q.b = a.frame0 + bl;
     q.ty = t / a.tiles_x;
     q.tx = t - q.ty * a.tiles_x;
+    q.live = (int)live | (SEAM ? w36_seam(q.ty * TH, a.frame_rows, TH) : W36_SEAM_NONE) << 1;
     return q;
   };
   auto halo_base = [&](const TilePos& q) {
@@ -151,25 +156,56 @@
     int tl = tid;
     asm volatile("" : "+v"(tl));
     const int iy0 = q.ty * TH - 1, ix0 = q.tx * TW - 1;
-    const int hlim = q.live ? a.H : 0;
-#pragma unroll
-    for (int i = 0; i < HIT; ++i) {
-      const int e = tl + i * NT;
-      const int pix = (e * 13108) >> 16, c4 = e - pix * 5;
-      const int hy = HW == 18 ? (pix * 3641) >> 16 : (pix * 1928) >> 16;
-      const int hx = pix - hy * HW;
-      const bool ok = ((unsigned)(iy0 + hy) < (unsigned)hlim) & ((unsigned)(ix0 + hx) < (unsigned)a.W) & (hy < HH) & (c4 < 4);
-      const int off = (((hy - 1) * a.W + (hx - 1)) * a.csx + c4 * 4) * 4;
-      okoff[i] = ok ? off : W36_MARKER;
-    }
-    if constexpr (DUST) {
-#pragma unroll
-      for (int i = 0; i < C::HIT64; ++i) {
-        const int pix = tl + i * NT;
+    const int hlim = (q.live & 1) ? a.H : 0;
+    if constexpr (!SEAM) {
+#pragma unroll
+      for (int i = 0; i < HIT; ++i) {
+        const int e = tl + i * NT;
+        const int pix = (e * 13108) >> 16, c4 = e - pix * 5;
         const int hy = HW == 18 ? (pix * 3641) >> 16 : (pix * 1928) >> 16;
         const int hx = pix - hy * HW;
-        const bool ok = ((unsigned)(iy0 + hy) < (unsigned)hlim) & ((unsigned)(ix0 + hx) < (unsigned)a.W) & (hy < HH) & (a.dust_in != 0);
-        okoff64[i] = ok ? (((hy - 1) * a.W + (hx - 1)) * a.csx + 64) * 4 : W36_MARKER;
+        const bool ok = ((unsigned)(iy0 + hy) < (unsigned)hlim) & ((unsigned)(ix0 + hx) < (unsigned)a.W) & (hy < HH) & (c4 < 4);
+        const int off = (((hy - 1) * a.W + (hx - 1)) * a.csx + c4 * 4) * 4;
+        okoff[i] = ok ? off : W36_MARKER;
+      }
+      if constexpr (DUST) {
+#pragma unroll
+        for (int i = 0; i < C::HIT64; ++i) {
+          const int pix = tl + i * NT;
+          const int hy = HW == 18 ? (pix * 3641) >> 16 : (pix * 1928) >> 16;
+          const int hx = pix - hy * HW;
+          const bool ok = ((unsigned)(iy0 + hy) < (unsigned)hlim) & ((unsigned)(ix0 + hx) < (unsigned)a.W) & (hy < HH) & (a.dust_in != 0);
+          okoff64[i] = ok ? (((hy - 1) * a.W + (hx - 1)) * a.csx + 64) * 4 : W36_MARKER;
+        }
+      }
+    } else {
+      const int zrow = w36_seam_zero_row(q.live >> 1), ins = w36_seam_inserted(q.live >> 1), hrows = HH + ins;
+      auto slot_row = [&](int hy, int& sy) {
+        sy = hy - (((zrow - hy) >> 31) & ins);
+        const int dz = hy - zrow, iy = iy0 + sy;
+        return iy | (hlim - 1 - iy) | ~((dz | -dz) >> 31) | (hrows - 1 - hy);
+      };
+      const int wlim = a.W - 1;
+#pragma unroll
+      for (int i = 0; i < HIT; ++i) {
+        const int e = tl + i * NT;
+        const int pix = (e * 13108) >> 16, c4 = e - pix * 5;
+        const int hy = (pix * 3641) >> 16, hx = pix - hy * HW;
+        int sy;
+        const int ix = ix0 + hx, bad = slot_row(hy, sy) | ix | (wlim - ix) | (3 - c4);
+        const int off = (((sy - 1) * a.W + (hx - 1)) * a.csx + c4 * 4) * 4;
+        okoff[i] = bad < 0 ? W36_MARKER : off;
+      }
+      if constexpr (DUST) {
+        const int nodust = a.dust_in ? 0 : -1;
+#pragma unroll
+        for (int i = 0; i < C::HIT64; ++i) {
+          const int pix = tl + i * NT;
+          const int hy = (pix * 3641) >> 16, hx = pix - hy * HW;
+          int sy;
+          const int ix = ix0 + hx, bad = slot_row(hy, sy) | ix | (wlim - ix) | nodust;
+          okoff64[i] = bad < 0 ? W36_MARKER : (((sy - 1) * a.W + (hx - 1)) * a.csx + 64) * 4;
+        }
       }
     }
   };
@@ -193,7 +229,13 @@
   };
   const int wt_t = tid >> 4, ch_t = tid & 15;
   const int m_t = ((wt_t & 7) >> 1) * 4 + (wt_t >> 3) * 2 + (wt_t & 1);
-  const int trd = ((4 * (wt_t / TXT)) * HW + 4 * (wt_t % TXT)) * HROW + ch_t;
+  int trd = ((4 * (wt_t / TXT)) * HW + 4 * (wt_t % TXT)) * HROW + ch_t;
+  auto trd_tile = [&](const TilePos& q) {
+    int tl = tid;
+    asm volatile("" : "+v"(tl));
+    const int wt = tl >> 4, wr = wt / TXT;
+    return ((4 * wr + w36_seam_patch_shift(q.live >> 1, wr)) * HW + 4 * (wt % TXT)) * HROW + (tl & 15);
+  };
   const int twr = m_t * 16 + ((((ch_t >> 2) ^ (2 * ((m_t >> 3) & 1))) << 2) | (ch_t & 3));
   typedef float f32x2 __attribute__((ext_vector_type(2)));
   f32x2 tp[6][3];
@@ -269,6 +311,7 @@
   TilePos pos_cur = tile_pos(wg_first);
   int base_cur = halo_base(pos_cur);
   halo_tile(pos_cur);
+  if constexpr (SEAM) trd = trd_tile(pos_cur);
   load_halo64(base_cur);
   load_halo(base_cur, C::OFF_H0);
   load_halo(base_cur + 64, C::OFF_H1);
@@ -276,6 +319,9 @@
   FPC_LDS_BARRIER();
   transform_all(C::OFF_H0, C::OFF_V0);
   FPC_LDS_BARRIER();
+  if constexpr (DUST && SEAM) {
+    if (tid == 0) lds[C::D_SEAM] = __int_as_float(pos_cur.live >> 1);
+  }
 
   constexpr int C4 = N / 4, EIT = HPX * C4 / NT, PPI = NT / C4;
   constexpr int CPR = TW / PPI;
@@ -320,6 +366,9 @@
       const int c3 = c + 2;
       const bool nxt = c3 >= nchunk;
       const int l_base = (nxt ? base_next : base_cur) + (nxt ? c3 - nchunk : c3) * 64;
+      if constexpr (SEAM && par == 1) {
+        if (c + 1 == nchunk) trd = trd_tile(pos_next);
+      }
       int ao = aoff4 + VB_OFF / 4, trd_c = trd + HN_OFF, twr_c = twr + VN_OFF;
       asm volatile("" : "+v"(ao), "+v"(trd_c), "+v"(twr_c));
       [[maybe_unused]] int dva = d_va + VB_OFF / 4;
@@ -429,7 +478,8 @@
       const int lane_d = tid_d & 63;
       if (a.dust_in) {
         if (tid_d < 16) {
-          const int rd = C::D_H64 + ((4 * (tid_d / TXT)) * HW + 4 * (tid_d % TXT)) * 4;
+          const int wr_d = tid_d / TXT;
+          const int rd = C::D_H64 + ((4 * wr_d + (SEAM ? w36_seam_patch_shift(__float_as_int(lds[C::D_SEAM]), wr_d) : 0)) * HW + 4 * (tid_d % TXT)) * 4;
 #pragma unroll
           for (int i = 0; i < 6; ++i)
 #pragma unroll
@@ -472,6 +522,9 @@
       }
       FPC_LDS_BARRIER();
       load_halo64(base_next);
+      if constexpr (SEAM) {
+        if (tid_d == 0) lds[C::D_SEAM] = __int_as_float(pos_next.live >> 1);
+      }
       if (tid_d < 16) {
         float mm[36];
 #pragma unroll
@@ -599,6 +652,8 @@
 #pragma unroll
     for (int k = 0; k < CPR; ++k) ocol[k] = (tx * TW + m0 + k * PPI < a.W) ? opart + k * PPI * a.cso * 4 : W36_MARKER;
 
+    int tW = a.W, tcso = a.cso, tcsx = a.csx;
+    asm volatile("" : "+s"(tW), "+s"(tcso), "+s"(tcsx));
 #pragma unroll
     for (int half = 0; half < 2; ++half) {
       const int y0 = ty * TH + half * (TH / 2), x0 = tx * TW;
@@ -669,7 +724,7 @@
               v.w = v.w > 0.f ? v.w : 0.f;
             }
             int voff;
-            const int so = obase + (i / CPR) * a.W * a.cso * 4;
+            const int so = obase + (i / CPR) * tW * tcso * 4;
             asm("v_add_i32 %0, %1, %2 clamp" : "=v"(voff) : "v"(ocol[i % CPR]), "s"(so));
             __builtin_amdgcn_raw_buffer_store_b128(__builtin_bit_cast(__attribute__((__vector_size__(4 * sizeof(unsigned)))) unsigned, v), orsrc, voff, 0, 0);
           }
@@ -730,7 +785,7 @@
 #pragma unroll
           for (int i = 0; i < XIT; ++i) {
             constexpr int XCPR = TW / 8;
-            const int so = xbase + ((i / XCPR) * a.W + (i % XCPR) * 8) * a.csx * 4;
+            const int so = xbase + ((i / XCPR) * tW + (i % XCPR) * 8) * tcsx * 4;
             xst[i] = __builtin_bit_cast(f32x4, __builtin_amdgcn_raw_buffer_load_b128(xrsrc, xp + so, 0, 0));
           }
         };
@@ -785,7 +840,7 @@
 #pragma unroll
           for (int r = 0; r < 4; ++r) {
             constexpr int BPR = TW / 16;
-            const int so = xbase + ((mb / BPR) * a.W + (mb % BPR) * 16 + r) * a.csx * 4;
+            const int so = xbase + ((mb / BPR) * tW + (mb % BPR) * 16 + r) * tcsx * 4;
 #pragma unroll
             for (int nb = 0; nb < NB; ++nb)
               acc2[mb][nb][r] = __builtin_bit_cast(float, __builtin_amdgcn_raw_buffer_load_b32(xrsrc, xl + so + 64 * nb, 0, 0));
diff --git a/feature-point-cnn_amd/csrc/wblock36p_mfma.h b/feature-point-cnn_amd/csrc/wblock36p_mfma.h
--- a/feature-point-cnn_amd/csrc/wblock36p_mfma.h
+++ b/feature-point-cnn_amd/csrc/wblock36p_mfma.h
@@ -21,6 +21,7 @@
   static constexpr int BASE_FLOATS = (OFF_V1 + V_FLOATS) > (OFF_H0 + T_FLOATS) ? (OFF_V1 + V_FLOATS) : (OFF_H0 + T_FLOATS);
   static constexpr int HIT64 = (NHALO + NTH - 1) / NTH;
   static constexpr int D_HEAD = BASE_FLOATS, D_COL = D_HEAD + 64, D_UIN = D_HEAD + 448, D_V64 = D_UIN + 2304, D_M64 = D_V64 + 576, D_H64 = D_M64 + 576;
+  static constexpr int D_SEAM = D_HEAD + 402;
   static constexpr int LDS_FLOATS = DUST ? D_H64 + HIT64 * NTH * 4 : BASE_FLOATS;
   static constexpr int LDS_BYTES = LDS_FLOATS * 4;
   static_assert(LDS_BYTES <= 160 * 1024, "LDS");
@@ -35,6 +36,9 @@
   constexpr int TH = C::TH, TW = C::TW, HW = C::HW, HH = C::HH, HROW = C::HROW, HIT = C::HIT, NTH = C::NTH;
   constexpr int N = C::N, RH = C::RH, STEPS = C::STEPS, PX = C::PX;
   static_assert(STEPS % RING == 0 && RING >= 2, "ring slots must line up across chunks");
+  constexpr bool SEAM = TYT == 4;
+  constexpr int HSLOT = SEAM ? HH + 1 : HH;
+  static_assert(HSLOT * HW * 5 <= HIT * NTH && HSLOT * HW <= C::HIT64 * NTH, "an inserted halo row must fit the requests");
   extern __shared__ __attribute__((aligned(16))) float lds[];
   f32x4* const lds4 = reinterpret_cast<f32x4*>(lds);
   constexpr int TL4 = C::OFF_H0 / 4;
@@ -60,13 +64,14 @@
   struct TilePos { int b, ty, tx, live; };
   auto tile_pos = [&](int wg) {
     TilePos q;
-    q.live = wg < wg_end;
-    const int wgc = q.live ? wg : wg_first;
+    const bool live = wg < wg_end;
+    const int wgc = live ? wg : wg_first;
     const int bl = wgc / tiles;
     const int t = wgc - bl * tiles;
     q.b = a.frame0 + bl;
     q.ty = t / a.tiles_x;
     q.tx = t - q.ty * a.tiles_x;
+    q.live = (int)live | (SEAM ? w36_seam(q.ty * TH, a.frame_rows, TH) : W36_SEAM_NONE) << 1;
     return q;
   };
   auto halo_base = [&](const TilePos& q) {
@@ -78,7 +83,7 @@
     const int pix = (e * 13108) >> 16, c4 = e - pix * 5;
     const int hy = HW == 18 ? (pix * 3641) >> 16 : (pix * 1928) >> 16;
     const int hx = pix - hy * HW;
-    const bool slot_ok = (hy < HH) & (c4 < 4);
+    const bool slot_ok = (hy < HSLOT) & (c4 < 4);
     return slot_ok ? (hy << 16) | (c4 << 8) | hx : 0x7fff0000;
   };
   int okoff[HIT];
@@ -96,7 +101,7 @@
     const int pix = tl + i * NTH;
     const int hy = HW == 18 ? (pix * 3641) >> 16 : (pix * 1928) >> 16;
     const int hx = pix - hy * HW;
-    return (hy < HH && a.dust_in) ? (hy << 16) | hx : 0x7fff0000;
+    return (hy < HSLOT && a.dust_in) ? (hy << 16) | hx : 0x7fff0000;
   };
   if constexpr (DUST) {
     if (hs == 1) {
@@ -106,25 +111,74 @@
   }
   auto halo_tile = [&](const TilePos& q) {
     const int iy0 = q.ty * TH - 1, ix0 = q.tx * TW - 1;
-    const int hlim = q.live ? a.H : 0;
+    const int hlim = (q.live & 1) ? a.H : 0;
     int tlq = tid & (NTH - 1);
     asm volatile("" : "+v"(tlq));
-#pragma unroll
-    for (int i = 0; i < HIT; ++i) {
-      int hv = KEEP_HYX ? hyx[KEEP_HYX ? i : 0] : slot_hyx(tlq, i);
-      asm volatile("" : "+v"(hv));
-      const int hy = hv >> 16, hx = hv & 0xff, c4 = (hv >> 8) & 0xff;
-      const bool ok = ((unsigned)(iy0 + hy) < (unsigned)hlim) & ((unsigned)(ix0 + hx) < (unsigned)a.W);
-      okoff[i] = ok ? (((hy - 1) * a.W + (hx - 1)) * a.csx + c4 * 4) * 4 : W36_MARKER;
-    }
-    if constexpr (DUST) {
-#pragma unroll
-      for (int i = 0; i < C::HIT64; ++i) {
-        int hv = slot_hyx64(tlq, i);
+    if constexpr (!SEAM) {
+#pragma unroll
+      for (int i = 0; i < HIT; ++i) {
+        int hv = KEEP_HYX ? hyx[KEEP_HYX ? i : 0] : slot_hyx(tlq, i);
         asm volatile("" : "+v"(hv));
-        const int hy = hv >> 16, hx = hv & 0xffff;
+        const int hy = hv >> 16, hx = hv & 0xff, c4 = (hv >> 8) & 0xff;
         const bool ok = ((unsigned)(iy0 + hy) < (unsigned)hlim) & ((unsigned)(ix0 + hx) < (unsigned)a.W);
-        okoff64[i] = ok ? (((hy - 1) * a.W + (hx - 1)) * a.csx + 64) * 4 : W36_MARKER;
+        okoff[i] = ok ? (((hy - 1) * a.W + (hx - 1)) * a.csx + c4 * 4) * 4 : W36_MARKER;
+      }
+      if constexpr (DUST) {
+#pragma unroll
+        for (int i = 0; i < C::HIT64; ++i) {
+          int hv = slot_hyx64(tlq, i);
+          asm volatile("" : "+v"(hv));
+          const int hy = hv >> 16, hx = hv & 0xffff;
+          const bool ok = ((unsigned)(iy0 + hy) < (unsigned)hlim) & ((unsigned)(ix0 + hx) < (unsigned)a.W);
+          okoff64[i] = ok ? (((hy - 1) * a.W + (hx - 1)) * a.csx + 64) * 4 : W36_MARKER;
+        }
+      }
+    } else {
+      const int zrow = w36_seam_zero_row(q.live >> 1), ins = w36_seam_inserted(q.live >> 1), hrows = HH + ins;
+      auto seam_row = [&](int hy, int& sy) {
+        sy = hy - (((zrow - hy) >> 31) & ins);
+        const int dz = hy - zrow;
+        return (iy0 + sy) | ~((dz | -dz) >> 31);
+      };
+      if constexpr (!DUST) {
+        auto slot_row = [&](int hy, int& sy) {
+          sy = hy - (((zrow - hy) >> 31) & ins);
+          const int dz = hy - zrow, iy = iy0 + sy;
+          return iy | (hlim - 1 - iy) | ~((dz | -dz) >> 31) | (hrows - 1 - hy);
+        };
+        const int wlim = a.W - 1;
+#pragma unroll
+        for (int i = 0; i < HIT; ++i) {
+          int hv = hyx[KEEP_HYX ? i : 0];
+          asm volatile("" : "+v"(hv));
+          const int hy = hv >> 16, hx = hv & 0xff, c4 = (hv >> 8) & 0xff;
+          int sy;
+          const int ix = ix0 + hx, bad = slot_row(hy, sy) | ix | (wlim - ix);
+          okoff[i] = bad < 0 ? W36_MARKER : (((sy - 1) * a.W + (hx - 1)) * a.csx + c4 * 4) * 4;
+        }
+      } else {
+#pragma unroll
+        for (int i = 0; i < HIT; ++i) {
+          int hv = slot_hyx(tlq, i);
+          asm volatile("" : "+v"(hv));
+          const int hy = hv >> 16, hx = hv & 0xff, c4 = (hv >> 8) & 0xff;
+          int sy;
+          const int iy = seam_row(hy, sy);
+          const bool rows_ok = (i * NTH + NTH - 1) / 5 / HW < HH ? true : hy < hrows;
+          const bool ok = ((unsigned)iy < (unsigned)hlim) & ((unsigned)(ix0 + hx) < (unsigned)a.W) & rows_ok;
+          okoff[i] = ok ? (((sy - 1) * a.W + (hx - 1)) * a.csx + c4 * 4) * 4 : W36_MARKER;
+        }
+#pragma unroll
+        for (int i = 0; i < C::HIT64; ++i) {
+          int hv = slot_hyx64(tlq, i);
+          asm volatile("" : "+v"(hv));
+          const int hy = hv >> 16, hx = hv & 0xffff;
+          int sy;
+          const int iy = seam_row(hy, sy);
+          const bool rows_ok = (i * NTH + NTH - 1) / HW < HH ? true : hy < hrows;
+          const bool ok = ((unsigned)iy < (unsigned)hlim) & ((unsigned)(ix0 + hx) < (unsigned)a.W) & rows_ok;
+          okoff64[i] = ok ? (((sy - 1) * a.W + (hx - 1)) * a.csx + 64) * 4 : W36_MARKER;
+        }
       }
     }
   };
@@ -149,7 +203,13 @@
   const int tq = tid & (NTH - 1);
   const int wt_t = tq >> 4, ch_t = tq & 15;
   const int m_t = ((wt_t & 7) >> 1) * 4 + (wt_t >> 3) * 2 + (wt_t & 1);
-  const int trd = ((4 * (wt_t / TXT)) * HW + 4 * (wt_t % TXT)) * HROW + ch_t;
+  int trd = ((4 * (wt_t / TXT)) * HW + 4 * (wt_t % TXT)) * HROW + ch_t;
+  auto trd_tile = [&](const TilePos& q) {
+    int tl = tid & (NTH - 1);
+    asm volatile("" : "+v"(tl));
+    const int wt = tl >> 4, wr = wt / TXT;
+    return ((4 * wr + w36_seam_patch_shift(q.live >> 1, wr)) * HW + 4 * (wt % TXT)) * HROW + (tl & 15);
+  };
   const int twr = m_t * 16 + ((((ch_t >> 2) ^ (2 * ((m_t >> 3) & 1))) << 2) | (ch_t & 3));
   typedef float f32x2 __attribute__((ext_vector_type(2)));
   f32x2 tp[6][3];
@@ -219,6 +279,7 @@
   }
   FPC_LDS_BARRIER();
   if (hs == 0) {
+    if constexpr (SEAM) trd = trd_tile(pos_cur);
 #pragma unroll
     for (int i = 0; i < 6; ++i)
 #pragma unroll
@@ -230,6 +291,9 @@
       for (int j = 0; j < 6; ++j) t_write(twr + C::OFF_V0, i, j);
   }
   FPC_LDS_BARRIER();
+  if constexpr (DUST && SEAM) {
+    if (tid == 0) lds[C::D_SEAM] = __int_as_float(pos_cur.live >> 1);
+  }
 
   constexpr int C4 = N / 4, EIT = PX * C4 / C::NT, PPI = C::NT / C4;
   constexpr int RPI = PPI / TW > 0 ? PPI / TW : 1;
@@ -270,6 +334,9 @@
       const int c3 = c + 2;
       const bool nxt = c3 >= nchunk;
       const int l_base = (nxt ? base_next : base_cur) + (nxt ? c3 - nchunk : c3) * 64;
+      if constexpr (SEAM && role == 0 && par == 1) {
+        if (c + 1 == nchunk) trd = trd_tile(pos_next);
+      }
       int ao = aoff4 + VB_OFF / 4, trd_c = trd + HN_OFF, twr_c = twr + VN_OFF;
       asm volatile("" : "+v"(ao), "+v"(trd_c), "+v"(twr_c));
       [[maybe_unused]] int dva = d_va + VB_OFF / 4;
@@ -367,7 +434,8 @@
     if constexpr (DUST) {
       if (a.dust_in) {
         if (tid_t < 16) {
-          const int rd = C::D_H64 + ((4 * (tid_t / TXT)) * HW + 4 * (tid_t % TXT)) * 4;
+          const int wr_d = tid_t / TXT;
+          const int rd = C::D_H64 + ((4 * wr_d + (SEAM ? w36_seam_patch_shift(__float_as_int(lds[C::D_SEAM]), wr_d) : 0)) * HW + 4 * (tid_t % TXT)) * 4;
 #pragma unroll
           for (int i = 0; i < 6; ++i)
 #pragma unroll
@@ -410,6 +478,9 @@
       }
       FPC_LDS_BARRIER();
       if (hs == 1) load_halo64(base_next);
+      if constexpr (SEAM) {
+        if (tid_t == 0) lds[C::D_SEAM] = __int_as_float(pos_next.live >> 1);
+      }
     }
 
     int hw_base[4];
diff --git a/feature-point-cnn_amd/csrc/wblock_mfma.h b/feature-point-cnn_amd/csrc/wblock_mfma.h
--- a/feature-point-cnn_amd/csrc/wblock_mfma.h
+++ b/feature-point-cnn_amd/csrc/wblock_mfma.h
@@ -21,6 +21,7 @@
   int conv_only;
   const float* dust;
   int dust_in;
+  int frame_rows;
 #ifdef FPC_DIAG
   unsigned long long* stamps;
 #endif
diff --git a/include/fpc.h b/include/fpc.h
--- a/include/fpc.h
+++ b/include/fpc.h
@@ -68,6 +68,7 @@
   FPC_PLAN_W36_ONE_WAVE = 1 << 18,
   FPC_PLAN_STEM_ROUND3 = 1 << 20,
   FPC_PLAN_CONV_ROUND1 = 1 << 21,
+  FPC_PLAN_NO_STACKED_TILES = 1 << 22,
   FPC_PLAN_CONVT_PHASES = 1 << 19,
   FPC_PLAN_GUARD_ZONES = 1 << 15
 };
```

New measurement: 12140, median of 6. Within noise of the previous version (+0.7%).
